# dsilvestro/LiteRate

Hardware: AMD Instinct MI355X
Metric: RJMCMC iters/sec x lineages (lineage-log-lik evals/s, summed over chains) (higher is better)
Workload: dtype f64

## Files before the change

include/literate_hip.h:

```cpp
#ifndef LITERATE_HIP_H
#define LITERATE_HIP_H

#include <stdint.h>

#ifdef __cplusplus
extern "C" {
#endif

#define LR_OK 0
#define LR_ERR_NULL (-1)
#define LR_ERR_SIZE (-2)
#define LR_ERR_MODEL (-3)
#define LR_ERR_WORKSPACE (-4)
#define LR_ERR_T0 (-5)
#define LR_ERR_STATE (-6)
#define LR_ERR_ORDER (-7)

#define LR_KMAX 32
#define LR_ROW 64
#define LR_MAX_BINS 4094

#define LR_MODEL_BD 0
#define LR_MODEL_ID 1
#define LR_MODEL_KEIDING 2
// ... 48 lines not shown
                   double* birth_rates, double* death_rates, void* stream);

int lr_binned_keiding(const double* birth_rates, const double* death_rates, const int64_t* n_spec,
                      const int64_t* n_exti, const double* DT, int32_t n_bins, int32_t n_chains,
                      double* out_birth, double* out_death, void* stream);

int lr_simulate_bd(const double* lam_steps, const double* mu_steps, int32_t n_steps, int32_t mode,
                   double l0, double m0, double K, double scale, int64_t n_start, int64_t capacity,
                   uint64_t seed, double* ts, double* te, int64_t* counters ,
                   int64_t* alive_trace, void* workspace, int64_t workspace_bytes, void* stream);

#define LR_SIMBATCH_GROUPS 512
#define LR_SIMBATCH_LDS_SLOTS 16384
int64_t lr_simulate_bd_batch_workspace_bytes(int32_t n_reps, int32_t n_bins, int32_t steps_per_bin, int64_t capacity);
int lr_simulate_bd_batch(const double* lam_bins , const double* mu_bins ,
                         int32_t n_reps, int32_t n_bins, int32_t steps_per_bin,
                         const int64_t* n_start , int64_t capacity, uint64_t seed,
                         int64_t* counts , int64_t* totals ,
                         void* workspace, int64_t workspace_bytes, void* stream);

#define LR_FORMAT_CRLF 1
int64_t lr_format_rows(const double* vals, const int64_t* row_start, int64_t n_rows, uint64_t int_cols, int32_t flags,
                       char* out, int64_t cap);

int64_t lr_rtt_summary_workspace_bytes(int32_t n_samples, int32_t n_chains, double start_age, double end_age,
                                       double burnin, int32_t pooled);
int lr_rtt_summary(const double* trace, int32_t n_samples, int32_t n_chains, double start_age, double end_age,
                   double burnin, int32_t pooled, double* rates, double* shift_freq, int64_t* k_counts,
                   void* workspace, int64_t workspace_bytes, void* stream);

#define LR_ESS_LDS_ROWS 16384
int64_t lr_ess_summary_workspace_bytes(int32_t n_samples, int32_t n_chains, int32_t row_width, const int32_t* cols,
                                       int32_t n_cols, double burnin, int32_t max_lag);
int lr_ess_summary(const double* rows, int32_t n_samples, int32_t n_chains, int32_t row_width, const int32_t* cols,
                   int32_t n_cols, double burnin, int32_t max_lag, double* chain_stats, int32_t* stop_lag,
                   double* col_stats, void* workspace, int64_t workspace_bytes, void* stream);

int64_t lr_col_summary_workspace_bytes(int32_t n_samples, int32_t n_chains, int32_t row_width, const int32_t* cols,
                                       int32_t n_cols, double burnin, int32_t pooled, int32_t cols_per_pass);
int lr_col_summary(const double* rows, int32_t n_samples, int32_t n_chains, int32_t row_width, const int32_t* cols,
                   int32_t n_cols, double burnin, int32_t pooled, double* out, void* workspace, int64_t workspace_bytes,
                   void* stream);
int64_t lr_curve_summary_workspace_bytes(int32_t n_samples, int32_t n_chains, int32_t row_width, int32_t arg_col,
                                         int32_t sampler, int32_t n_bins, double burnin, int32_t pooled,
                                         int32_t bins_per_pass);
int lr_curve_summary(const double* rows, int32_t n_samples, int32_t n_chains, int32_t row_width, int32_t arg_col,
                     int32_t sampler, int32_t m_birth, int32_t m_death, const double* aux, int32_t n_bins, double burnin,
                     int32_t pooled, double* out, void* workspace, int64_t workspace_bytes, void* stream);

typedef struct lr_mcmc_config {
    int64_t n_lineages;
    int32_t n_bins;
    int32_t n_chains;
    int32_t model;
    int32_t const_rates;
    int32_t const_death_rate;
    int32_t use_rate_HP;
    int32_t s_freq;
    int32_t n_trace_slots;
    double poisson_HP;
    double update_fraction;
    double t0;
    double start_time;
    double end_time;
    uint64_t seed;
    int64_t chain_offset;
    int32_t unit_resolution;
    int32_t engine_mode;
    double frac_birth;
    double frac_death;
    int32_t sampler;
    int32_t m_birth;
    int32_t m_death;
    int32_t team_request;
    double dd_present;
    double dd_init_death;
} lr_mcmc_config;

typedef struct lr_mcmc_layout {
    int64_t state_f64;
    int64_t state_i32;
    int64_t bin_consts;
    int64_t lineage_idx;
    int64_t args_blob;
    int64_t tables;
    int64_t partials;
    int64_t trace;
    int64_t total_bytes;
    int32_t table_stride;
    int32_t tiles;
    int32_t chains_per_block;
    int32_t trace_width;
    int32_t n_parts;
    int32_t pipelined;
    int32_t persistent;
    int32_t reserved1;
    int64_t status;
    int64_t xchg;
    int32_t team_blocks;
    int32_t table_mode;
    int64_t lineage_frac;
    int64_t pack_tmp;
    int32_t spec_chains_per_team;
    int32_t streaming;
    int32_t packed_scan;
    int32_t reserved3;
} lr_mcmc_layout;

#define LR_ROW_L 0
#define LR_ROW_M 1
#define LR_ROW_TL 2
#define LR_ROW_TM 3
#define LR_ROW_PL 4
#define LR_ROW_PM 5
#define LR_ROW_PTL 6
#define LR_ROW_PTM 7
#define LR_ROW_SCALARS 8
#define LR_STATE_ROWS 9
#define LR_S_LIKA 0
#define LR_S_PRIORA 1
#define LR_S_PRIORPOIA 2
#define LR_S_GRATE_L 3
#define LR_S_GRATE_M 4
#define LR_S_POI 5
#define LR_S_HASTING 6
#define LR_S_PRIOR_P 7
#define LR_S_PRIORPOI_P 8
#define LR_S_CONST_P 9
#define LR_S_CONST_A 10
#define LR_S_LIK_P 11
#define LR_S_LOG_G0 12
#define LR_S_LOG_G1 13
#define LR_S_LOG_POI 14
#define LR_S_LOG_U 15
#define LR_IROW_EL 0
#define LR_IROW_EM 1
#define LR_IROW_PEL 2
#define LR_IROW_PEM 3
#define LR_IROW_SCALARS 4
#define LR_ISTATE_ROWS 5
#define LR_I_KL 0
#define LR_I_KM 1
#define LR_I_PKL 2
#define LR_I_PKM 3
#define LR_I_GIBBS 4
#define LR_I_INVALID 5
#define LR_I_IT_LO 6
#define LR_I_IT_HI 7
#define LR_I_ACCEPTED 8
#define LR_I_MOVE 9
#define LR_I_NEXT_LO 10
#define LR_I_NEXT_HI 11
#define LR_I_SLOT 12

#define LR_TRACE_HEAD 13
#define LR_TRACE_W (LR_TRACE_HEAD + 2 * (2 * LR_KMAX - 1))

typedef struct lr_engine lr_engine;

int lr_mcmc_query_layout(const lr_mcmc_config* cfg , lr_mcmc_layout* out );
int lr_mcmc_create(const lr_mcmc_config* cfg , const double* ts, const double* te,
                   const double* br_length ,
                   void* workspace, int64_t workspace_bytes, lr_engine** out );
int lr_mcmc_init(lr_engine* e, const double* L, const double* M, const double* tL,
                 const double* tM, const int32_t* KL, const int32_t* KM, int32_t kmax, void* stream);
int lr_mcmc_steps(lr_engine* e, int64_t n_iters, void* stream);
int lr_mcmc_restore(lr_engine* e, void* stream);
int lr_mcmc_time_scan(lr_engine* e, int32_t reps, float* avg_ms , void* stream);
int lr_mcmc_time_steps(lr_engine* e, int64_t n_iters, float* total_ms , void* stream);
int lr_mcmc_status(lr_engine* e, int32_t* status , void* stream);
#define LR_WARN_KCAP 2
int lr_mcmc_warnings(lr_engine* e, int32_t* warnings , void* stream);
int lr_mcmc_describe(const lr_engine* e, char* buf , int32_t n);
int lr_mcmc_destroy(lr_engine* e);

#ifdef __cplusplus
}
#endif
#endif
```

literate_amd/_hip.py:

```python
import ctypes as C
import os

from .build import LIB

c_i32, c_i64, c_f64, c_vp = C.c_int32, C.c_int64, C.c_double, C.c_void_p

LR_ERR_NULL, LR_ERR_SIZE, LR_ERR_MODEL, LR_ERR_WORKSPACE, LR_ERR_T0, LR_ERR_STATE, LR_ERR_ORDER = -1, -2, -3, -4, -5, -6, -7
ERRORS = {-1: "LR_ERR_NULL", -2: "LR_ERR_SIZE", -3: "LR_ERR_MODEL", -4: "LR_ERR_WORKSPACE", -5: "LR_ERR_T0",
          -6: "LR_ERR_STATE", -7: "LR_ERR_ORDER (lineages must be sorted by birth time for the persistent engines)"}

LR_KMAX, LR_ROW, LR_MAX_BINS = 32, 64, 4094
LR_WARN_KCAP = 2
LR_STATE_ROWS, LR_ISTATE_ROWS = 9, 5
LR_TRACE_HEAD = 13
LR_TRACE_W = LR_TRACE_HEAD + 2 * (2 * LR_KMAX - 1)
LR_SIMBATCH_GROUPS, LR_SIMBATCH_LDS_SLOTS = 512, 16384
LR_ESS_LDS_ROWS = 16384
ROW_L, ROW_M, ROW_TL, ROW_TM, ROW_PL, ROW_PM, ROW_PTL, ROW_PTM, ROW_SCALARS = range(9)
(S_LIKA, S_PRIORA, S_PRIORPOIA, S_GRATE_L, S_GRATE_M, S_POI, S_HASTING, S_PRIOR_P, S_PRIORPOI_P, S_CONST_P,
 S_CONST_A, S_LIK_P, S_LOG_G0, S_LOG_G1, S_LOG_POI) = range(15)
IROW_EL, IROW_EM, IROW_PEL, IROW_PEM, IROW_SCALARS = range(5)
(I_KL, I_KM, I_PKL, I_PKM, I_GIBBS, I_INVALID, I_IT_LO, I_IT_HI, I_ACCEPTED, I_MOVE, I_NEXT_LO, I_NEXT_HI,
 I_SLOT) = range(13)


class McmcConfig(C.Structure):
    _fields_ = [("n_lineages", c_i64), ("n_bins", c_i32), ("n_chains", c_i32), ("model", c_i32),
                ("const_rates", c_i32), ("const_death_rate", c_i32), ("use_rate_HP", c_i32), ("s_freq", c_i32),
                ("n_trace_slots", c_i32), ("poisson_HP", c_f64), ("update_fraction", c_f64), ("t0", c_f64),
                ("start_time", c_f64), ("end_time", c_f64), ("seed", C.c_uint64), ("chain_offset", c_i64),
                ("unit_resolution", c_i32), ("engine_mode", c_i32), ("frac_birth", c_f64), ("frac_death", c_f64),
                ("sampler", c_i32), ("m_birth", c_i32), ("m_death", c_i32), ("team_request", c_i32),
                ("dd_present", c_f64), ("dd_init_death", c_f64)]


class McmcLayout(C.Structure):
    _fields_ = [("state_f64", c_i64), ("state_i32", c_i64), ("bin_consts", c_i64), ("lineage_idx", c_i64), ("args_blob", c_i64), ("tables", c_i64),
                ("partials", c_i64), ("trace", c_i64), ("total_bytes", c_i64), ("table_stride", c_i32),
                ("tiles", c_i32), ("chains_per_block", c_i32), ("trace_width", c_i32), ("n_parts", c_i32),
                ("pipelined", c_i32), ("persistent", c_i32), ("reserved1", c_i32), ("status", c_i64), ("xchg", c_i64),
                ("team_blocks", c_i32), ("table_mode", c_i32), ("lineage_frac", c_i64), ("pack_tmp", c_i64),
                ("spec_chains_per_team", c_i32), ("streaming", c_i32), ("packed_scan", c_i32), ("reserved3", c_i32)]


SIGNATURES = {
    "lr_version": (c_i32, []),
    "lr_bin_events_workspace_bytes": (c_i64, [c_i64, c_i32]),
    "lr_bin_events": (c_i32, [c_vp, c_vp, c_i64, c_vp, c_vp, c_i32, c_vp, c_vp, c_vp, c_vp, c_i64, c_vp]),
    "lr_bin_unit_events_workspace_bytes": (c_i64, [c_i64, c_i32]),
    "lr_bin_unit_events": (c_i32, [c_vp, c_vp, c_i64, c_f64, c_i32, c_vp, c_vp, c_vp, c_vp, c_i64, c_vp]),
    "lr_expand_rates": (c_i32, [c_vp, c_vp, c_vp, c_i32, c_i32, c_i32, c_i32, c_vp, c_vp]),
    "lr_bd_loglik_workspace_bytes": (c_i64, [c_i64, c_i32, c_i32, c_i32]),
    "lr_bd_loglik_plan": (c_i32, [c_i64, c_i32, c_i32, c_i32, C.POINTER(c_i32)]),
    "lr_bd_loglik_batch": (c_i32, [c_vp, c_vp, c_i64, c_f64, c_i32, c_vp, c_vp, c_i32, c_i32, c_vp, c_f64, c_vp,
                                   c_vp, c_i64, c_vp]),
    "lr_rj_propose_score": (c_i32, [c_vp, c_vp, c_vp, c_i32, c_i32, c_vp, c_vp, c_vp, c_f64, c_vp, c_vp, c_vp, c_vp,
                                    c_vp]),
    "lr_log_priors": (c_i32, [c_vp, c_vp, c_i32, c_i32, c_f64, c_vp, c_vp, c_vp, c_vp]),
    "lr_dd_rates": (c_i32, [c_vp, c_vp, c_i32, c_i32, c_i32, c_i32, c_vp, c_vp, c_vp, c_vp, c_vp]),
    "lr_ddv2_rates": (c_i32, [c_vp, c_vp, c_i32, c_i32, c_i32, c_i32, c_vp, c_vp, c_vp, c_vp, c_vp]),
    "lr_binned_keiding": (c_i32, [c_vp, c_vp, c_vp, c_vp, c_vp, c_i32, c_i32, c_vp, c_vp, c_vp]),
    "lr_simulate_bd": (c_i32, [c_vp, c_vp, c_i32, c_i32, c_f64, c_f64, c_f64, c_f64, c_i64, c_i64, C.c_uint64, c_vp, c_vp,
                             c_vp, c_vp, c_vp, c_i64, c_vp]),
    "lr_simulate_bd_batch_workspace_bytes": (c_i64, [c_i32, c_i32, c_i32, c_i64]),
    "lr_simulate_bd_batch": (c_i32, [c_vp, c_vp, c_i32, c_i32, c_i32, c_vp, c_i64, C.c_uint64, c_vp, c_vp, c_vp, c_i64,
                                   c_vp]),
    "lr_trend_rates": (c_i32, [c_vp, c_vp, c_i32, c_i32, c_i32, c_i32, c_vp, c_vp, c_vp]),
    "lr_format_rows": (c_i64, [c_vp, c_vp, c_i64, C.c_uint64, c_i32, c_vp, c_i64]),
    "lr_rtt_summary_workspace_bytes": (c_i64, [c_i32, c_i32, c_f64, c_f64, c_f64, c_i32]),
    "lr_rtt_summary": (c_i32, [c_vp, c_i32, c_i32, c_f64, c_f64, c_f64, c_i32, c_vp, c_vp, c_vp, c_vp, c_i64, c_vp]),
    "lr_ess_summary_workspace_bytes": (c_i64, [c_i32, c_i32, c_i32, c_vp, c_i32, c_f64, c_i32]),
    "lr_ess_summary": (c_i32, [c_vp, c_i32, c_i32, c_i32, c_vp, c_i32, c_f64, c_i32, c_vp, c_vp, c_vp, c_vp, c_i64, c_vp]),
    "lr_col_summary_workspace_bytes": (c_i64, [c_i32, c_i32, c_i32, c_vp, c_i32, c_f64, c_i32, c_i32]),
    "lr_col_summary": (c_i32, [c_vp, c_i32, c_i32, c_i32, c_vp, c_i32, c_f64, c_i32, c_vp, c_vp, c_i64, c_vp]),
    "lr_curve_summary_workspace_bytes": (c_i64, [c_i32, c_i32, c_i32, c_i32, c_i32, c_i32, c_f64, c_i32, c_i32]),
    "lr_curve_summary": (c_i32, [c_vp, c_i32, c_i32, c_i32, c_i32, c_i32, c_i32, c_i32, c_vp, c_i32, c_f64, c_i32, c_vp,
                                 c_vp, c_i64, c_vp]),
    "lr_mcmc_query_layout": (c_i32, [C.POINTER(McmcConfig), C.POINTER(McmcLayout)]),
    "lr_mcmc_create": (c_i32, [C.POINTER(McmcConfig), c_vp, c_vp, c_vp, c_vp, c_i64, C.POINTER(c_vp)]),
    "lr_mcmc_init": (c_i32, [c_vp, c_vp, c_vp, c_vp, c_vp, c_vp, c_vp, c_i32, c_vp]),
    "lr_mcmc_steps": (c_i32, [c_vp, c_i64, c_vp]),
    "lr_mcmc_time_scan": (c_i32, [c_vp, c_i32, C.POINTER(C.c_float), c_vp]),
    "lr_mcmc_time_steps": (c_i32, [c_vp, c_i64, C.POINTER(C.c_float), c_vp]),
    "lr_mcmc_restore": (c_i32, [c_vp, c_vp]),
    "lr_mcmc_describe": (c_i32, [c_vp, C.c_char_p, c_i32]),
    "lr_mcmc_status": (c_i32, [c_vp, C.POINTER(c_i32), c_vp]),
    "lr_mcmc_warnings": (c_i32, [c_vp, C.POINTER(c_i32), c_vp]),
    "lr_mcmc_destroy": (c_i32, [c_vp]),
    "lr_debug_draws": (c_i32, [C.c_uint64, c_i64, c_vp, c_vp, c_vp, c_vp, c_vp, c_i32, c_vp, c_vp]),
    "lr_debug_stream2": (c_i32, [c_vp, c_vp, c_i64, c_vp, c_vp]),
}

_lib = None


class HipLibraryError(RuntimeError):
    pass


def load():
    global _lib
    if _lib is not None:
        return _lib
    if not os.path.exists(LIB):
        raise HipLibraryError("libliterate_hip.so not found at %s - run `python -m literate_amd.build` "
                              "(there is no CPU fallback)" % LIB)
    lib = C.CDLL(LIB)
    for name, (res, args) in SIGNATURES.items():
        fn = getattr(lib, name)
        fn.restype, fn.argtypes = res, args
    _lib = lib
    return lib


def check(rc, what):
    if rc == 0:
        return
    if rc < 0:
        raise ValueError("%s: %s" % (what, ERRORS.get(rc, rc)))
    raise HipLibraryError("%s: hipError_t %d" % (what, rc))


def require_gpu():
    import torch
    if not torch.cuda.is_available():
        raise HipLibraryError("no ROCm GPU visible: literate_amd has no CPU path")
    return torch


def ptr(t):
    return None if t is None else c_vp(t.data_ptr())


def stream_ptr(device=None):
    import torch
    return c_vp(torch.cuda.current_stream(device).cuda_stream)


def launch(fn, device, *args):
    import torch
    with torch.cuda.device(device):
        return fn(*args, stream_ptr(device))
```

literate_amd/csrc/lr_engine.h:

```cpp
#pragma once
#include "lr_internal.h"
#include "lr_scan.h"
#include "lr_step.h"

#define LR_MAX_PARTS 4
struct lr_part {
    int base, count, hA;
    bool pipelined;
    hipStream_t stream;
    hipEvent_t done;
    hipGraphExec_t graph_exec;
    int graph_units;
};

struct lr_p4_shares {
    int delta[16];
    int n_slots;
    int help_trips;
};

struct lr_engine {
    lr_mcmc_config cfg;
    lr_mcmc_layout lay;
    lr_scan_plan plan;
    const double* ts;
    const double* te;
    const double* br_length;
    char* ws;
    bool initialised;
    int n_parts;
    lr_part part[LR_MAX_PARTS];
    bool persistent;
    long long n8;
    long long n8_alloc;
    lr_p4_shares p4;
    bool p4_help;
    bool packed_scan;
    bool streaming;
    hipEvent_t fork;
    hipEvent_t ev0, ev1;
};


#define LR_P4_MAX_GIVE 64
#define LR_IDX_SPARE ((LR_P4_MAX_GIVE + 2) * 1024)
#define LR_MAX_RUNS (1ll << 20)

static inline long long lr_groups_alloc(long long n_lineages) {
    const long long runs = n_lineages < LR_MAX_RUNS ? n_lineages : LR_MAX_RUNS;
    return (n_lineages + LR_SLOTS - 1) / LR_SLOTS + runs + LR_IDX_SPARE;
}

#define LR_P4_CARRY_BYTES 512

#define LR_H_WIDE 520

#ifndef LR_SPEC_THREADS
#define LR_SPEC_THREADS 768
#endif
#ifndef LR_SPEC_THREADS_SINGLE
#define LR_SPEC_THREADS_SINGLE 768
#endif
#ifndef LR_SPEC_SCAN_UNROLL
#define LR_SPEC_SCAN_UNROLL 1
#endif
#ifndef LR_SPEC_SCAN_PRIO
#define LR_SPEC_SCAN_PRIO 2
#endif
#define LR_TEAM_MAX 8
#define LR_SPEC_GRANULES 16
#define LR_SPEC_TIMEOUT_TICKS 200000000ull

static inline bool lr_p4_help_choice(const lr_engine* e) {
    const char* env = getenv("LR_P4_HELP");
    if (e->lay.persistent != 2 || e->plan.unit == LR_TAB_PAIRGEN || e->cfg.sampler != 0 || e->plan.H > 264) return false;
    return env ? atoi(env) != 0 : true;
}

static inline int lr_spec_mode(const lr_engine* e) {
    if (e->lay.spec_chains_per_team != 1) return 0;
    if (e->lay.team_blocks > 1) return 1;
    const double trips = (double)e->n8 / 64.0 / 8.0;
    const char* env = getenv("LR_SPEC_PLANES_BY_SCANNERS");
    const bool by_scanners = env ? atoi(env) != 0 : trips <= 3.0;
    return by_scanners ? 2 : 3;
}

#define LR_STEP_WAVES_PER_BLOCK (LR_SCAN_THREADS / LR_WAVE)
#define LR_STREAM_COPIES 64
#define LR_STREAM_MAX_CHAINS 16
struct lr_stream_sync {
    unsigned long long arrived;
    unsigned long long pad0[15];
    unsigned long long word[LR_STREAM_COPIES][LR_STREAM_MAX_CHAINS];
};
#define LR_STREAM_SYNC_BYTES (128 + LR_STREAM_COPIES * 128 + 128)
static_assert(sizeof(lr_stream_sync) + 128 == LR_STREAM_SYNC_BYTES && LR_STREAM_SYNC_BYTES % 256 == 0, "counter line + a line per copy");
bool lr_stream_eligible(const lr_mcmc_config* cfg, const lr_scan_plan& p);
void lr_stream_plan(const lr_mcmc_config* cfg, lr_scan_plan* p, int cus);
int lr_launch_stream(lr_engine* e, const lr_step_args& a, int64_t n_iters, bool query, hipStream_t stream);

bool lr_packscan_eligible(const lr_mcmc_config* cfg, const lr_scan_plan& p);
void lr_packscan_plan(const lr_mcmc_config* cfg, lr_scan_plan* p, int cus);
int lr_packscan_pairs(const lr_scan_plan& p, int n_chains);
int lr_launch_packscan(const lr_engine* e, int base, int count, hipStream_t stream);

lr_step_args lr_make_args(const lr_engine* e);
int lr_pack_lineages(lr_engine* e, hipStream_t stream);
long long lr_pack_tmp_bytes(long long n_lineages);
int lr_launch_spec(lr_engine* e, const lr_step_args& a, const lr_packed_lineages& pk, int64_t n_iters, hipStream_t stream);
```

literate_amd/csrc/lr_mcmc.hip:

```cpp
#include <cmath>
#include <cstdio>
#include <cstdlib>
#include <new>

#include "lr_chain.h"
#include "lr_dd.h"
#include "lr_engine.h"
#include "lr_internal.h"
#include "lr_scan.h"
#include "lr_step.h"

__global__ __launch_bounds__(LR_WAVE) void lr_rj_propose_score_kernel(
    const double* __restrict__ rates, const double* __restrict__ times, const int* __restrict__ K, int kmax,
    const int* __restrict__ move, const int* __restrict__ index, const double* __restrict__ draws, double mult_d,
    double* __restrict__ out_rates, double* __restrict__ out_times, int* __restrict__ out_K,
    double* __restrict__ out_score) {
    const int c = blockIdx.x, lane = threadIdx.x;
    int k = K[c];
    double R = (lane < k) ? rates[(size_t)c * kmax + lane] : 0.0;
    double T = (lane <= k) ? times[(size_t)c * (kmax + 1) + lane] : 0.0;
    const double* dr = draws + (size_t)c * 2 * kmax;
    const int mv = move[c];
    double score = 0.0;
    if (mv == 0) {
// ... 3 lines not shown
    } else if (mv == 1) {
        score = lr_wave_add_shift(R, T, k, index[c], dr[0], dr[1], lane);
    } else if (mv == 2) {
        score = lr_wave_remove_shift(R, T, k, index[c], lane);
    }
    if (lane < kmax) out_rates[(size_t)c * kmax + lane] = (lane < k) ? R : 0.0;
    if (lane <= kmax) out_times[(size_t)c * (kmax + 1) + lane] = (lane <= k) ? T : 0.0;
    if (lane == 0) out_K[c] = k, out_score[c] = score;
}

extern "C" int lr_rj_propose_score(const double* rates, const double* times, const int32_t* K, int32_t kmax,
                                   int32_t n_chains, const int32_t* move, const int32_t* index, const double* draws,
                                   double mult_d, double* out_rates, double* out_times, int32_t* out_K,
                                   double* out_score, void* stream_) {
    if (!rates || !times || !K || !move || !index || !draws || !out_rates || !out_times || !out_K || !out_score)
        return LR_ERR_NULL;
    if (kmax < 2 || kmax > LR_WAVE - 1 || n_chains < 1) return LR_ERR_SIZE;
    hipLaunchKernelGGL(lr_rj_propose_score_kernel, dim3(n_chains), dim3(LR_WAVE), 0, (hipStream_t)stream_, rates, times,
                       K, kmax, move, index, draws, mult_d, out_rates, out_times, out_K, out_score);
    return (int)hipGetLastError();
}

__global__ __launch_bounds__(LR_WAVE) void lr_log_priors_kernel(const double* __restrict__ rates,
                                                                const int* __restrict__ K, int kmax, double shape,
                                                                const double* __restrict__ gamma_rate,
                                                                const double* __restrict__ poi_rate,
                                                                double* __restrict__ out) {
    const int c = blockIdx.x, lane = threadIdx.x;
    const int k = K[c];
    const double R = (lane < k) ? rates[(size_t)c * kmax + lane] : 1.0;
    double p = lr_wave_prior_gamma(R, k, shape, gamma_rate[c], lane);
    if (poi_rate) p += lr_wave_poisson_prior(k, poi_rate[c], lane);
    if (lane == 0) out[c] = p;
}

extern "C" int lr_log_priors(const double* rates, const int32_t* K, int32_t kmax, int32_t n_chains, double shape,
                             const double* gamma_rate, const double* poi_rate, double* out, void* stream_) {
    if (!rates || !K || !gamma_rate || !out) return LR_ERR_NULL;
    if (kmax < 1 || kmax > LR_WAVE - 1 || n_chains < 1) return LR_ERR_SIZE;
    hipLaunchKernelGGL(lr_log_priors_kernel, dim3(n_chains), dim3(LR_WAVE), 0, (hipStream_t)stream_, rates, K, kmax,
                       shape, gamma_rate, poi_rate, out);
    return (int)hipGetLastError();
}

__global__ void lr_debug_draws_kernel(uint32_t seed, uint32_t chain, const long long* it, const int* purpose,
                                      const int* idx, const int* kind, const double* shape, int n, double* out) {
    const int i = blockIdx.x * blockDim.x + threadIdx.x;
    if (i >= n) return;
    lr_stream s{seed, chain};
    const uint64_t t = (uint64_t)it[i];
    double v;
    switch (kind[i]) {
        case 0: v = lr_pair(s, t, purpose[i], idx[i]).a; break;
        case 1: v = lr_pair(s, t, purpose[i], idx[i]).b; break;
        case 2: v = lr_normal(s, t, purpose[i], idx[i]); break;
        default: v = lr_gamma(s, t, purpose[i], idx[i], shape[i]); break;
    }
    out[i] = v;
}

extern "C" int lr_debug_draws(uint64_t seed, int64_t chain, const int64_t* it, const int32_t* purpose,
                              const int32_t* idx, const int32_t* kind, const double* shape, int32_t n, double* out,
                              void* stream_) {
    if (!it || !purpose || !idx || !kind || !shape || !out) return LR_ERR_NULL;
    hipLaunchKernelGGL(lr_debug_draws_kernel, dim3((n + 63) / 64), dim3(64), 0, (hipStream_t)stream_, (uint32_t)seed,
                       (uint32_t)chain, (const long long*)it, purpose, idx, kind, shape, n, out);
    return (int)hipGetLastError();
}

#define LR_STEP_WAVES (LR_SCAN_THREADS / LR_WAVE)

__global__ __launch_bounds__(LR_SCAN_THREADS) void lr_chain_step_kernel(lr_step_args a, int mode, int chain_base,
                                                                        int n_sub) {
    __shared__ lr_seg_scratch scratch[LR_STEP_WAVES];
    const int wave = threadIdx.x / LR_WAVE, lane = threadIdx.x & (LR_WAVE - 1);
    const int j = blockIdx.x * LR_STEP_WAVES + wave;
    if (j < n_sub) lr_chain_step_body<32>(a, mode, chain_base + j, lane, &scratch[wave]);
}

struct lr_fused_args {
    const double* ts;
    const double* te;
    long long n, chunk;
    double t0;
    int n_bins, tiles;
    int scan_base, scan_n;
    int step_base, step_n;
    int step_blocks;
};

template <int CB, int H, bool UNIT>
__global__ __launch_bounds__(LR_SCAN_THREADS) void lr_fused_iter_kernel(lr_step_args a, lr_fused_args f) {
    extern __shared__ double2 lds[];
    lr_seg_scratch* scratch = reinterpret_cast<lr_seg_scratch*>(lds);
    const int bid = blockIdx.x;
    if (bid < f.step_blocks) {
        const int wave = threadIdx.x / LR_WAVE, lane = threadIdx.x & (LR_WAVE - 1);
        const int j = bid * LR_STEP_WAVES + wave;
        if (j < f.step_n) lr_chain_step_body(a, 0, f.step_base + j, lane, &scratch[wave]);
        return;
    }
    int group, tile;
    if ((f.step_blocks & 7) == 0) {
        lr_xcd_remap(bid - f.step_blocks, f.tiles, (f.scan_n + CB - 1) / CB, &group, &tile);
    } else {
        const int sb = bid - f.step_blocks;
        tile = sb % f.tiles, group = sb / f.tiles;
    }
    const double2* tables = a.tables + (size_t)f.scan_base * a.tab_stride;
    const int tile_stride = lr_tile_stride(a.tiles);
    double* partials = const_cast<double*>(a.partials) + (size_t)f.scan_base * tile_stride;
    if (UNIT)
        lr_scan_unit_body<CB, H>(lds, tile, group * CB, f.ts, f.te, f.n, f.t0, f.n_bins, tables, f.scan_n, f.chunk,
                                 partials, tile_stride);
    else
        lr_scan_fast_body<CB, H>(lds, tile, group * CB, f.ts, f.te, f.n, f.t0, f.n_bins, tables, f.scan_n, f.chunk,
                                 partials, tile_stride);
}

#ifndef LR_PERSIST_THREADS
#define LR_PERSIST_THREADS 512
#endif
#ifndef LR_PERSIST_MINWAVES
#define LR_PERSIST_MINWAVES 4
#endif

template <int H, bool GENERAL>
__global__ __launch_bounds__(256) void lr_pairscan_kernel(lr_packed_lineages pk, long long n8, const double2* __restrict__ tables,
                                                          int n_chains, int n_bins, int tiles, double* __restrict__ partials) {
    constexpr int ENT = GENERAL ? 2 : 1;
    __shared__ double2 tab[LR_UNIT_PLANES * H];
    __shared__ double red[4][2];
    const int tid = threadIdx.x, lane = tid & (LR_WAVE - 1), wave = tid / LR_WAVE;
    const int tile = blockIdx.x, pair = blockIdx.y;
    const double2* src = tables + (size_t)pair * (2 * H * ENT);
    for (int i = tid; i < 2 * H * ENT; i += 256) tab[GENERAL ? lr_pairgen_lds_entry(i, H) : i] = src[i];
    __syncthreads();
    if (GENERAL) lr_pair_planes_block_general(tab, H, n_bins, tid, 256);
    else lr_pair_planes_block(tab, H, n_bins, tid, 256);
    __syncthreads();
    const long long per = (n8 + tiles - 1) / tiles;
    const long long g0 = min((long long)tile * per, n8), g1 = min(g0 + per, n8);
    double acc0 = 0.0, acc1 = 0.0;
    lr_persist_scan<H, GENERAL>(reinterpret_cast<const char*>(tab), pk, g0, g1 - g0, tid, 256, &acc0, &acc1);
    const double s0 = lr_wave_sum(acc0), s1 = lr_wave_sum(acc1);
    if (lane == 0) red[wave][0] = s0, red[wave][1] = s1;
    __syncthreads();
    if (tid < 2 && 2 * pair + tid < n_chains)
        partials[(size_t)(2 * pair + tid) * lr_tile_stride(tiles) + tile] = ((red[0][tid] + red[1][tid]) + red[2][tid]) + red[3][tid];
}

typedef __attribute__((address_space(3))) double lr_lds_f64;
typedef __attribute__((address_space(3))) int lr_lds_i32;
template <int PB, int ES, bool PRE = false, int SAMPLER = -1, bool HAND = false>
__device__ __forceinline__ void lr_persist_step_body(const __attribute__((address_space(3))) lr_step_args* a3, int c, int lane,
                                                     __attribute__((address_space(3))) lr_seg_scratch* scratch3,
                                                     lr_lds_f64* st_f64, lr_lds_i32* st_i32, double lik, lr_lds_f64* table3,
                                                     lr_lds_f64* br3 ,
                                                     const lr_draw_slot* draws = nullptr ,
                                                     lr_table_hand* hand = nullptr, int hand_epoch = 0) {
    constexpr int table_es = ES;
    const lr_step_args& a = *(const lr_step_args*)a3;
    const double* br_lds = (const double*)br3;
    LR_SSTAMP(0);
    lr_chain_regs st;
    lr_chain_load(st, (double*)st_f64, (int*)st_i32, lane);
    if (SAMPLER == 1 || (SAMPLER == -1 && a.cfg.sampler != 0))
        lr_dd_step_core<true>(st, a, 0, c, lane, lik, reinterpret_cast<double2*>((double*)table3), table_es, br_lds);
    else if (PRE) {
        lr_rj_draws pre;
        lr_draws_load(draws, pre, lane);
        lr_chain_step_core<true, PB, HAND>(st, a, 0, c, lane, (lr_seg_scratch*)scratch3, lik, reinterpret_cast<double2*>((double*)table3),
                                           table_es, br_lds, br_lds + LR_H_WIDE, &pre, hand, hand_epoch);
    } else
        lr_chain_step_core<true, PB>(st, a, 0, c, lane, (lr_seg_scratch*)scratch3, lik, reinterpret_cast<double2*>((double*)table3),
                                     table_es, br_lds, br_lds + LR_H_WIDE);
    if (HAND) lr_chain_store_handed(st, (double*)st_f64, (int*)st_i32, lane);
    else lr_chain_store(st, (double*)st_f64, (int*)st_i32, lane);
    LR_SSTAMP(8);
}

template <int NA>
__device__ __forceinline__ void lr_p4_leave_sums(double2 (*part)[LR_WAVE], int* arrived, double* out, int slot, int lane,
                                                 int& scans_done, double s0, double s1) {
    part[slot][lane] = make_double2(s0, s1);
    int prev = 0;
    if (lane == 0) prev = __hip_atomic_fetch_add(arrived, 1, __ATOMIC_RELAXED, __HIP_MEMORY_SCOPE_WORKGROUP);
    prev = __builtin_amdgcn_readfirstlane(prev);
    if (prev == NA * (scans_done + 1) - 1) {
        asm volatile("" ::: "memory");
        double a0 = 0.0, a1 = 0.0;
#pragma unroll
        for (int w = 0; w < NA; ++w) {
            const double2 v = part[w][lane];
            a0 += v.x, a1 += v.y;
        }
        a0 = lr_wave_sum(a0), a1 = lr_wave_sum(a1);
        if (lane == 0) out[0] = a0, out[1] = a1;
    }
    ++scans_done;
}

template <int PB, int ES>
__device__ __attribute__((noinline)) void lr_persist_step(const __attribute__((address_space(3))) lr_step_args* a3, int c, int lane,
                                                          __attribute__((address_space(3))) lr_seg_scratch* scratch3,
                                                          lr_lds_f64* st_f64, lr_lds_i32* st_i32, double lik, lr_lds_f64* table3,
                                                          lr_lds_f64* br3) {
    lr_persist_step_body<PB, ES>(a3, c, lane, scratch3, st_f64, st_i32, lik, table3, br3);
}

template <int PB, int ES, int NW, int SAMPLER, bool HELP>
__device__ __attribute__((noinline)) void lr_persist4_steppers(const __attribute__((address_space(3))) lr_step_args* a3, int c0,
                                                               int n_chains, int wave, int lane,
                                                               __attribute__((address_space(3))) lr_seg_scratch* scratch3,
                                                               lr_lds_f64* st_f64, lr_lds_i32* st_i32, lr_lds_f64* red,
                                                               lr_lds_f64* tab, int tab_doubles, lr_lds_f64* br3, long long n_iters,
                                                               const lr_draw_slot* draws ,
                                                               lr_table_hand* hands ) {
    static_assert(!HELP || (ES == 2 && SAMPLER == 0), "helper waves: RJ sampler at unit resolution");
    for (long long iter = 0; iter < n_iters; ++iter) {
#pragma unroll 1
        for (int ph = 0; ph < 2; ++ph) {
#ifdef LR_DIAG
            const unsigned long long dq0 = wall_clock64();
#endif
            const int c = c0 + 2 * ph + wave;
            if (c < n_chains) {
                double lik = 0.0;
#pragma unroll
                for (int w2 = 2; w2 < (ES == 2  ? 3 : NW); ++w2) lik += red[(ph * NW + w2) * 2 + wave];
                lr_persist_step_body<PB, ES, ES == 2  && SAMPLER == 0, SAMPLER, HELP>(
                    a3, c, lane, scratch3, st_f64 + (2 * ph + wave) * (LR_STATE_ROWS * LR_ROW),
                    st_i32 + (2 * ph + wave) * (LR_ISTATE_ROWS * LR_ROW), lik, tab + ph * tab_doubles + wave, br3,
                    draws + (2 * ph + wave), HELP ? hands + wave : nullptr, (int)((2 * iter + ph + 1) & 0x3fffffff));
            }
#ifdef LR_DIAG
            const unsigned long long dq1 = wall_clock64();
#endif
            __syncthreads();
#ifdef LR_DIAG
            if (lane == 0 && blockIdx.x < 64) {
                atomicAdd(&lr_diag_step[16384 + (blockIdx.x * 16 + wave) * 4 + 0], dq1 - dq0);
                atomicAdd(&lr_diag_step[16384 + (blockIdx.x * 16 + wave) * 4 + 1], wall_clock64() - dq1);
            }
#endif
        }
    }
}

template <int H, int T, int PB>
__device__ __attribute__((noinline)) void lr_persist2_steppers(const __attribute__((address_space(3))) lr_step_args* a3, int c, int wave,
                                                               int lane, __attribute__((address_space(3))) lr_seg_scratch* scratch3,
                                                               lr_lds_f64* st_f64, lr_lds_i32* st_i32, lr_lds_f64* red ,
                                                               lr_lds_f64* tab, lr_lds_f64* br3, const uint4* __restrict__ idx8,
                                                               long long n8w, long long n_iters, int prio_shift, int grp) {
    const int tid = wave * LR_WAVE + lane;
    for (long long iter = 0; iter < n_iters; ++iter) {
        if (prio_shift > 0) {
            if (((wall_clock64() >> prio_shift) + grp) & 1) __builtin_amdgcn_s_setprio(1);
            else __builtin_amdgcn_s_setprio(0);
        }
        double acc0 = 0.0, acc1 = 0.0;
        lr_scan_tail tail;
        lr_persist_scan_pair<H, 1, true>((const char*)(const double*)tab, idx8, n8w, tid, T, &acc0, &acc1, nullptr, &tail);
        const double s0 = lr_wave_sum(acc0), s1 = lr_wave_sum(acc1);
        if (lane == 0) red[wave * 2 + 0] = s0, red[wave * 2 + 1] = s1;
        lr_scan_drain(tail);
        __syncthreads();
        double lik = 0.0;
#pragma unroll
        for (int w2 = 0; w2 < T / LR_WAVE; ++w2) lik += red[w2 * 2 + wave];
        lr_persist_step_body<PB, 2>(a3, c, lane, scratch3, st_f64, st_i32, lik, tab + wave, br3);
        __syncthreads();
    }
}

template <int H, int T>
__global__ __launch_bounds__(T, LR_PERSIST_MINWAVES) void lr_persist_kernel(
    const lr_step_args* __restrict__ ap ,
    const uint4* __restrict__ idx8, long long n8, lr_p4_shares sh, long long n_iters, int prio_shift) {
    const lr_step_args& a = *ap;
    __shared__ double2 tab[LR_UNIT_PLANES * H];
    __shared__ double red[T / LR_WAVE][2];
    __shared__ lr_seg_scratch scratch[2];
    __shared__ double st_f64[2][LR_STATE_ROWS * LR_ROW];
    __shared__ int st_i32[2][LR_ISTATE_ROWS * LR_ROW];
    __shared__ lr_step_args a_lds;
    __shared__ double br_lds[2][LR_H_WIDE];
    const int tid = threadIdx.x, lane = tid & (LR_WAVE - 1), wave = tid / LR_WAVE;
    if (tid < (int)(sizeof(lr_step_args) / 4)) reinterpret_cast<int*>(&a_lds)[tid] = reinterpret_cast<const int*>(ap)[tid];
    for (int b = tid; b < LR_H_WIDE; b += blockDim.x) {
        const bool in = b < ap->cfg.n_bins;
        br_lds[0][b] = (in && ap->br_length) ? ap->br_length[b] : 0.0;
        br_lds[1][b] = in ? ap->log_br[b] : 0.0;
    }
    const int c0 = blockIdx.x * 2;
    const int c = c0 + wave;
    const bool stepper = (wave < 2) && (c < a.cfg.n_chains);
    double2* gpair = lr_chain_table(a, c0);
    if (stepper) {
        const double* S = a.state_f64 + (size_t)c * LR_STATE_ROWS * LR_ROW;
        const int* I = a.state_i32 + (size_t)c * LR_ISTATE_ROWS * LR_ROW;
        for (int r = 0; r < LR_STATE_ROWS; ++r) st_f64[wave][r * LR_ROW + lane] = S[r * LR_ROW + lane];
        for (int r = 0; r < LR_ISTATE_ROWS; ++r) st_i32[wave][r * LR_ROW + lane] = I[r * LR_ROW + lane];
    }
    for (int i = tid; i < 2 * H; i += T) tab[i] = gpair[i];
    __syncthreads();
    lr_pair_planes_block(tab, H, a.cfg.n_bins, tid, T);
    __syncthreads();
    const char* lbase = reinterpret_cast<const char*>(tab);
    const long long n8w = sh.delta[0] != 0 ? ((n8 + T - 1) / T + sh.delta[wave]) * T : n8;
    const int grp = (blockIdx.x >> 8) & 1;
#ifdef LR_DIAG
    unsigned long long d_t0 = 0, d_t1 = 0, d_t2 = 0, d_scan = 0, d_red = 0, d_step = 0;
#endif
#ifndef LR_DIAG
    if (stepper) {
        lr_persist2_steppers<H, T, (H <= 264 ? lr_bins_per_lane(H) : 0)>(
            (const __attribute__((address_space(3))) lr_step_args*)&a_lds, c, wave, lane,
            (__attribute__((address_space(3))) lr_seg_scratch*)&scratch[wave], (lr_lds_f64*)st_f64[wave], (lr_lds_i32*)st_i32[wave],
            (lr_lds_f64*)&red[0][0], (lr_lds_f64*)reinterpret_cast<double*>(tab), (lr_lds_f64*)&br_lds[0][0], idx8, n8w, n_iters,
            prio_shift, grp);
    } else
#endif
    for (long long iter = 0; iter < n_iters; ++iter) {
        if (prio_shift > 0) {
            if (((wall_clock64() >> prio_shift) + grp) & 1) __builtin_amdgcn_s_setprio(1);
            else __builtin_amdgcn_s_setprio(0);
        }
#ifdef LR_DIAG
        d_t0 = wall_clock64();
#endif
        double acc0 = 0.0, acc1 = 0.0;
        lr_scan_tail tail;
        lr_persist_scan_pair<H, 1, true>(lbase, idx8, n8w, tid, T, &acc0, &acc1, nullptr, &tail);
#ifdef LR_DIAG
        if (lane == 0 && blockIdx.x < 512) atomicAdd(&lr_diag_step[20000 + blockIdx.x * 8 + wave], wall_clock64() - d_t0);
#endif
#ifdef LR_DIAG
        d_t1 = wall_clock64();
#endif
        const double s0 = lr_wave_sum(acc0), s1 = lr_wave_sum(acc1);
        if (lane == 0) red[wave][0] = s0, red[wave][1] = s1;
        lr_scan_drain(tail);
        __syncthreads();
#ifdef LR_DIAG
        d_t2 = wall_clock64();
#endif
        if (stepper) {
            double lik = 0.0;
#pragma unroll
            for (int w2 = 0; w2 < T / LR_WAVE; ++w2) lik += red[w2][wave];
            lr_persist_step<(H <= 264 ? lr_bins_per_lane(H) : 0), 2>(
                (const __attribute__((address_space(3))) lr_step_args*)&a_lds, c, lane,
                (__attribute__((address_space(3))) lr_seg_scratch*)&scratch[wave], (lr_lds_f64*)st_f64[wave],
                (lr_lds_i32*)st_i32[wave], lik, (lr_lds_f64*)(reinterpret_cast<double*>(tab) + wave), (lr_lds_f64*)&br_lds[0][0]);
        }
        __syncthreads();
#ifdef LR_DIAG
        d_scan += d_t1 - d_t0, d_red += d_t2 - d_t1, d_step += wall_clock64() - d_t2;
#endif
    }
#ifdef LR_DIAG
    if (lane == 0 && blockIdx.x < 512) {
        unsigned long long* o = lr_diag_step + 4096 * 12 - 4096 + (blockIdx.x * 8 + wave) % 4096;
        (void)o;
    }
    if (tid == 0 && blockIdx.x < 340) {
        lr_diag_step[blockIdx.x * 12 + 9] = d_scan, lr_diag_step[blockIdx.x * 12 + 10] = d_red;
        lr_diag_step[blockIdx.x * 12 + 11] = d_step;
    }
    if (tid == 0 && blockIdx.x < 1024) lr_diag_step[2048 * 12 + blockIdx.x * 2 + 1] = wall_clock64();
#endif
    if (stepper) {
        double* S = a.state_f64 + (size_t)c * LR_STATE_ROWS * LR_ROW;
        int* I = a.state_i32 + (size_t)c * LR_ISTATE_ROWS * LR_ROW;
        for (int r = 0; r < LR_STATE_ROWS; ++r) S[r * LR_ROW + lane] = st_f64[wave][r * LR_ROW + lane];
        for (int r = 0; r < LR_ISTATE_ROWS; ++r) I[r * LR_ROW + lane] = st_i32[wave][r * LR_ROW + lane];
    }
    for (int i = tid; i < 2 * H; i += T) gpair[i] = tab[i];
}

#ifndef LR_P4_THREADS
#define LR_P4_THREADS 1024
#endif
#ifdef LR_DIAG
#define LR_PSTAMP(k) if (threadIdx.x == 0 && blockIdx.x < 64) lr_diag_step[28672 + blockIdx.x * 8 + (k)] = wall_clock64()
#else
#define LR_PSTAMP(k)
#endif

template <int H, bool GENERAL, bool PARAM ,
          bool HELP = false>
__global__ __launch_bounds__(LR_P4_THREADS, LR_P4_THREADS / 256) void lr_persist4_kernel(const lr_step_args* __restrict__ ap ,
                                                                       lr_packed_lineages pk, long long n8,
                                                                       lr_p4_shares sh, long long n_iters, char* carry_all) {
    static_assert(!HELP || (!GENERAL && !PARAM), "helper waves: RJ sampler at unit resolution");
    const lr_step_args& a = *ap;
    LR_PSTAMP(0);
    constexpr int NW = LR_P4_THREADS / LR_WAVE;
    constexpr int W0 = HELP ? 4 : 2;
    constexpr int NS = NW - W0;
    constexpr int LR_P4_SCANNERS = NS * LR_WAVE;
    constexpr int ENT = GENERAL ? 2 : 1;
    constexpr int ES = GENERAL ? 6 * H : 2;
    __shared__ double2 tab[2][LR_UNIT_PLANES * H];
    __shared__ double red[2][NW][2];
    constexpr bool LAST_SUMS = !GENERAL;
    __shared__ double2 part[LAST_SUMS ? NW - 2 : 1][LR_WAVE];
    __shared__ int arrived;
    __shared__ lr_table_hand hands[2];
    __shared__ lr_seg_scratch scratch[2];
    __shared__ double st_f64[4][LR_STATE_ROWS * LR_ROW];
    __shared__ int st_i32[4][LR_ISTATE_ROWS * LR_ROW];
    __shared__ lr_step_args a_lds;
    __shared__ double br_lds[2][LR_H_WIDE];
    __shared__ lr_draw_slot draws_s[4];
    lr_draw_slot* const draws = draws_s;
    const int tid = threadIdx.x, lane = tid & (LR_WAVE - 1), wave = tid / LR_WAVE;
    if (tid < (int)(sizeof(lr_step_args) / 4)) reinterpret_cast<int*>(&a_lds)[tid] = reinterpret_cast<const int*>(ap)[tid];
    for (int b = tid; b < LR_H_WIDE; b += blockDim.x) {
        const bool in = b < ap->cfg.n_bins;
        br_lds[0][b] = (in && ap->br_length) ? ap->br_length[b] : 0.0;
        br_lds[1][b] = in ? ap->log_br[b] : 0.0;
    }
    constexpr bool draw_ahead = !GENERAL && !PARAM;
    auto draw_duty = [&](int pr) {
        const int q = wave - W0, k = q & 1, ch = 2 * pr + k;
        if (!draw_ahead || q < 0 || q >= (HELP ? 2 : 4) || (int)(blockIdx.x * 4) + ch >= ap->cfg.n_chains) return;
        const int* I = st_i32[ch] + LR_IROW_SCALARS * LR_ROW;
        const unsigned long long it = ((unsigned long long)(unsigned int)I[LR_I_IT_HI] << 32 | (unsigned int)I[LR_I_IT_LO]) + 1ull;
        lr_draw_slot* slot = &draws[ch];
        if (HELP) lr_spec_draw_both(a_lds, (int)(blockIdx.x * 4) + ch, lane, it, slot);
        else lr_spec_draw_part(a_lds, (int)(blockIdx.x * 4) + ch, lane, it, slot, q >> 1);
    };
    auto help_duty = [&](int ph, int epoch) {
        const int k = wave - 2;
        const int ch = 2 * ph + k;
        if ((int)(blockIdx.x * 4) + ch >= ap->cfg.n_chains) return;
        lr_table_hand* hand = &hands[k];
#ifdef LR_DIAG
        const unsigned long long dh0 = wall_clock64();
#endif
        while (__hip_atomic_load(&hand->epoch, __ATOMIC_RELAXED, __HIP_MEMORY_SCOPE_WORKGROUP) != epoch) __builtin_amdgcn_s_sleep(1);
        asm volatile("" ::: "memory");
#ifdef LR_DIAG
        if (lane == 0 && blockIdx.x < 64) atomicAdd(&lr_diag_step[16384 + (blockIdx.x * 16 + wave) * 4 + 2], wall_clock64() - dh0);
#endif
        const lr_seg_scratch* sc = &scratch[k];
        const int eL = lane <= LR_KMAX ? sc->edge[0][lane] : 0, eM = lane <= LR_KMAX ? sc->edge[1][lane] : 0;
        double* tabd = reinterpret_cast<double*>(tab[ph]) + k;
        const double constP = lr_build_tables_segments<(H <= 264 ? lr_bins_per_lane(H) : 1), 2>(
            sc, eL, eM, hand->KL, hand->KM, br_lds[0], br_lds[1], a_lds.cfg.model, a_lds.cfg.n_bins, a_lds.n_cls, a_lds.H,
            reinterpret_cast<double2*>(tabd), lane, LR_TAB_UNIT, a_lds.cfg.frac_birth, a_lds.cfg.frac_death, ES, nullptr);
        LR_WAVE_LDS_ORDER();
        lr_pair_planes_wave(tabd, H, a_lds.cfg.n_bins, lane, 0);
        if (lane == 0) st_f64[ch][LR_ROW_SCALARS * LR_ROW + LR_S_CONST_P] = constP;
    };
    if (tid == 0) arrived = 0;
    if (tid < 2) hands[tid].epoch = 0;
    for (int i = tid; i < 2 * NW * 2; i += LR_P4_THREADS) (&red[0][0][0])[i] = 0.0;
    int scans_done = 0;
    constexpr int NA = NS + (HELP ? 2 : 0);
    auto leave_sums = [&](int pr, double s0, double s1) {
        if (LAST_SUMS) {
            lr_p4_leave_sums<NA>(part, &arrived, &red[pr][2][0], wave >= W0 ? wave - W0 : NS + wave - 2, lane, scans_done, s0, s1);
        } else {
            s0 = lr_wave_sum(s0), s1 = lr_wave_sum(s1);
            if (lane == 0) red[pr][wave][0] = s0, red[pr][wave][1] = s1;
        }
    };
    const int c0 = blockIdx.x * 4;
    const int C = a.cfg.n_chains;
    if (wave < 4 && c0 + wave < C) {
        const int c = c0 + wave;
        const double* S = a.state_f64 + (size_t)c * LR_STATE_ROWS * LR_ROW;
        const int* I = a.state_i32 + (size_t)c * LR_ISTATE_ROWS * LR_ROW;
        for (int r = 0; r < LR_STATE_ROWS; ++r) st_f64[wave][r * LR_ROW + lane] = S[r * LR_ROW + lane];
        for (int r = 0; r < LR_ISTATE_ROWS; ++r) st_i32[wave][r * LR_ROW + lane] = I[r * LR_ROW + lane];
    }
    double2* g0 = lr_chain_table(a, c0);
    double2* g1 = lr_chain_table(a, c0 + 2);
    for (int i = tid; i < 2 * H * ENT; i += LR_P4_THREADS) {
        const int e = GENERAL ? lr_pairgen_lds_entry(i, H) : i;
        tab[0][e] = g0[i], tab[1][e] = g1[i];
    }
    __syncthreads();
    LR_PSTAMP(1);
    if (GENERAL) {
        lr_pair_planes_block_general(tab[0], H, a.cfg.n_bins, tid, LR_P4_THREADS);
        lr_pair_planes_block_general(tab[1], H, a.cfg.n_bins, tid, LR_P4_THREADS);
    } else {
        lr_pair_planes_block(tab[0], H, a.cfg.n_bins, tid, LR_P4_THREADS);
        lr_pair_planes_block(tab[1], H, a.cfg.n_bins, tid, LR_P4_THREADS);
    }
    __syncthreads();
    LR_PSTAMP(2);
    const bool scanner = wave >= W0;
    const bool helper = HELP && (wave == 2 || wave == 3);
    const int sid = tid - W0 * LR_WAVE;
    const long long nh_ = HELP ? (long long)sh.help_trips * (2 * LR_WAVE) : 0;
    const int k_tot = (int)((n8 - nh_ + LR_P4_SCANNERS - 1) / LR_P4_SCANNERS);
    const int k_mine = k_tot + (scanner ? sh.delta[wave - W0] : 0);
    bool any_shift = false;
#pragma unroll
    for (int q = 0; q < NS; ++q) any_shift |= sh.delta[q] != 0;
    const long long nh = HELP ? (long long)sh.help_trips * (2 * LR_WAVE) : 0;
    const long long n8w = any_shift ? (long long)k_mine * LR_P4_SCANNERS : n8 - nh;
    auto help_scan = [&](int pr) {
        double s0 = 0.0, s1 = 0.0;
        if (nh > 0) lr_persist_scan<H, GENERAL, 1, false, false>(reinterpret_cast<const char*>(tab[pr]), pk, 0, nh, tid - 2 * LR_WAVE, 2 * LR_WAVE, &s0, &s1);
        leave_sums(pr, s0, s1);
    };
    static_assert(2 * NW * 8 + 4 <= LR_P4_CARRY_BYTES, "");
    char* carry = carry_all ? carry_all + (size_t)blockIdx.x * LR_P4_CARRY_BYTES : nullptr;
    const bool carried = carry && *reinterpret_cast<const int*>(carry + 2 * NW * 8) == 1;
    auto prologue_draws = [&]() { draw_duty(0); };
    if (carried) {
        if (tid < 2 * NW) (&red[0][0][0])[tid] = reinterpret_cast<const double*>(carry)[tid];
        if (scanner) prologue_draws();
    } else if (scanner) {
        double s0 = 0.0, s1 = 0.0;
        lr_scan_tail tail;
        lr_persist_scan<H, GENERAL, 1, false, true>(reinterpret_cast<const char*>(tab[0]), pk, nh, n8w, sid, LR_P4_SCANNERS, &s0, &s1, nullptr, &tail);
        leave_sums(0, s0, s1);
        lr_scan_drain(tail);
        prologue_draws();
    }
    if (helper && !carried) help_scan(0);
    __syncthreads();
    LR_PSTAMP(3);
    if (helper) {
        for (long long iter = 0; iter < n_iters; ++iter) {
#pragma unroll 1
            for (int ph = 0; ph < 2; ++ph) {
#ifdef LR_DIAG
                const unsigned long long dq0 = wall_clock64();
#endif
                help_scan(1 - ph);
                help_duty(ph, (int)((2 * iter + ph + 1) & 0x3fffffff));
#ifdef LR_DIAG
                const unsigned long long dq1 = wall_clock64();
#endif
                __syncthreads();
#ifdef LR_DIAG
                if (lane == 0 && blockIdx.x < 64) {
                    atomicAdd(&lr_diag_step[16384 + (blockIdx.x * 16 + wave) * 4 + 0], dq1 - dq0);
                    atomicAdd(&lr_diag_step[16384 + (blockIdx.x * 16 + wave) * 4 + 1], wall_clock64() - dq1);
                }
#endif
            }
        }
    } else if (!scanner)
        lr_persist4_steppers<(H <= 264 ? lr_bins_per_lane(H) : 0), ES, NW, PARAM ? 1 : 0, HELP>(
            (const __attribute__((address_space(3))) lr_step_args*)&a_lds, c0, C, wave, lane,
            (__attribute__((address_space(3))) lr_seg_scratch*)&scratch[wave], (lr_lds_f64*)&st_f64[0][0], (lr_lds_i32*)&st_i32[0][0],
            (lr_lds_f64*)&red[0][0][0], (lr_lds_f64*)reinterpret_cast<double*>(tab[0]), 2 * LR_UNIT_PLANES * H,
            (lr_lds_f64*)&br_lds[0][0], n_iters, &draws[0], &hands[0]);
    else
    for (long long iter = 0; iter < n_iters; ++iter) {
#pragma unroll
        for (int ph = 0; ph < 2; ++ph) {
#ifdef LR_DIAG
            const unsigned long long dq0 = wall_clock64();
#endif
            {
                double s0 = 0.0, s1 = 0.0;
                lr_scan_tail tail;
                lr_persist_scan<H, GENERAL, 1, false, true>(reinterpret_cast<const char*>(tab[1 - ph]), pk, nh, n8w, sid, LR_P4_SCANNERS, &s0, &s1, nullptr, &tail);
                leave_sums(1 - ph, s0, s1);
                lr_scan_drain(tail);
                draw_duty(1 - ph);
            }
#ifdef LR_DIAG
            const unsigned long long dq1 = wall_clock64();
#endif
            __syncthreads();
#ifdef LR_DIAG
            if (lane == 0 && blockIdx.x < 64) {
                atomicAdd(&lr_diag_step[16384 + (blockIdx.x * 16 + wave) * 4 + 0], dq1 - dq0);
                atomicAdd(&lr_diag_step[16384 + (blockIdx.x * 16 + wave) * 4 + 1], wall_clock64() - dq1);
            }
#endif
        }
    }
    LR_PSTAMP(4);
    if (wave < 4 && c0 + wave < C) {
        const int c = c0 + wave;
        double* S = a.state_f64 + (size_t)c * LR_STATE_ROWS * LR_ROW;
        int* I = a.state_i32 + (size_t)c * LR_ISTATE_ROWS * LR_ROW;
        for (int r = 0; r < LR_STATE_ROWS; ++r) S[r * LR_ROW + lane] = st_f64[wave][r * LR_ROW + lane];
        for (int r = 0; r < LR_ISTATE_ROWS; ++r) I[r * LR_ROW + lane] = st_i32[wave][r * LR_ROW + lane];
    }
    for (int i = tid; i < 2 * H * ENT; i += LR_P4_THREADS) {
        const int e = GENERAL ? lr_pairgen_lds_entry(i, H) : i;
        g0[i] = tab[0][e], g1[i] = tab[1][e];
    }
    if (carry) {
        if (tid < 2 * NW) reinterpret_cast<double*>(carry)[tid] = (&red[0][0][0])[tid];
        if (tid == 0) *reinterpret_cast<int*>(carry + 2 * NW * 8) = 1;
    }
    LR_PSTAMP(5);
}

__global__ void lr_store_args_kernel(lr_step_args a, lr_step_args* dst) {
    if (threadIdx.x == 0 && blockIdx.x == 0) *dst = a;
}

__global__ void lr_log_br_kernel(const double* __restrict__ br, int n_bins, double* __restrict__ out) {
    const int b = blockIdx.x * blockDim.x + threadIdx.x;
    if (b < n_bins) out[b] = (br && br[b] > 0.0) ? lr_log(br[b]) : 0.0;
}

__global__ __launch_bounds__(LR_WAVE) void lr_chain_init_kernel(lr_step_args a, const double* L0, const double* M0,
                                                                const double* tL0, const double* tM0,
                                                                const int* KL0, const int* KM0, int kmax) {
    __shared__ lr_seg_scratch scratch;
    const lr_mcmc_config& cfg = a.cfg;
    const int c = blockIdx.x, lane = threadIdx.x, n_bins = cfg.n_bins;
    double* S = a.state_f64 + (size_t)c * LR_STATE_ROWS * LR_ROW;
    int* I = a.state_i32 + (size_t)c * LR_ISTATE_ROWS * LR_ROW;
    const lr_stream rng{(uint32_t)cfg.seed, (uint32_t)(cfg.chain_offset + c)};
    if (cfg.sampler != 0) {
        const bool trend = cfg.sampler == 2;
        const int npar = trend ? LR_TR_NPAR : LR_DD_NPAR;
        double A = 0.0;
        if (L0) {
            if (lane < npar) A = L0[(size_t)c * kmax + lane];
        } else if (trend) {
            const double init[LR_TR_NPAR] = {.1, .1, 0.0, 0.0, 1.0, 1.0};
            if (lane < npar) A = init[lane];
        } else {
            const double x0 = cfg.dd_present - (cfg.t0 + cfg.dd_present) / 2.0;
            const double init[LR_DD_NPAR] = {0.5, 1.5, x0, 10.0, 20000.0, cfg.dd_init_death, 1.0, 1.0};
            if (lane < npar) A = init[lane];
        }
        if (trend) {
            const lr_trend_params tp = lr_trend_unpack(A);
            const double* aux = a.br_length;
            lr_rates_build_tables_wave([&](int b, double* br, double* dr) { lr_trend_bin_rates(tp, aux[b], cfg.m_birth, cfg.m_death, br, dr); },
                                       n_bins, a.H, lr_chain_table(a, c), lane, a.unit, cfg.frac_birth, cfg.frac_death, lr_tab_es(a.unit, a.H));
        } else {
            const lr_dd_params pp = lr_dd_unpack(A);
            lr_dd_build_tables_wave(pp, a.br_length, cfg.m_birth, cfg.m_death, n_bins, a.H, lr_chain_table(a, c), lane,
                                    a.unit, cfg.frac_birth, cfg.frac_death, lr_tab_es(a.unit, a.H));
        }
        for (int r = 0; r < LR_STATE_ROWS; ++r) S[r * LR_ROW + lane] = 0.0;
        for (int r = 0; r < LR_ISTATE_ROWS; ++r) I[r * LR_ROW + lane] = 0;
        S[LR_ROW_L * LR_ROW + lane] = A, S[LR_ROW_PL * LR_ROW + lane] = A;
        int io = 0;
        if (lane == LR_I_KL || lane == LR_I_PKL || lane == LR_I_KM || lane == LR_I_PKM) io = npar;
        I[LR_IROW_SCALARS * LR_ROW + lane] = io;
        return;
    }
    double L = 0.0, M = 0.0, tL = 0.0, tM = 0.0;
    int KL = 1, KM = 1;
    if (L0) {
        KL = KL0[c], KM = KM0[c];
        if (lane < KL) L = L0[(size_t)c * kmax + lane];
        if (lane < KM) M = M0[(size_t)c * kmax + lane];
        if (lane <= KL) tL = tL0[(size_t)c * (kmax + 1) + lane];
        if (lane <= KM) tM = tM0[(size_t)c * (kmax + 1) + lane];
    } else {
        const double l0 = lr_gamma(rng, 0, LR_P_INIT, 0, 2.0) * 2.0;
        const double m0 = lr_gamma(rng, 0, LR_P_INIT, 64, 2.0) * 2.0;
        if (lane == 0) L = l0, M = m0, tL = tM = cfg.start_time;
        if (lane == 1) tL = tM = cfg.end_time;
    }
    const int eL = lr_wave_edges(tL, 1), eM = lr_wave_edges(tM, 1);
    double logL, logM;
    lr_stage_segments(&scratch, L, M, eL, eM, KL, KM, lane, &logL, &logM);
    const double constA = lr_build_tables_segments(&scratch, eL, eM, KL, KM, a.br_length, a.log_br, cfg.model, n_bins,
                                                   a.n_cls, a.H, lr_chain_table(a, c), lane,
                                                   a.unit, cfg.frac_birth, cfg.frac_death, lr_tab_es(a.unit, a.H));
    S[LR_ROW_L * LR_ROW + lane] = L, S[LR_ROW_M * LR_ROW + lane] = M;
    S[LR_ROW_TL * LR_ROW + lane] = tL, S[LR_ROW_TM * LR_ROW + lane] = tM;
    S[LR_ROW_PL * LR_ROW + lane] = L, S[LR_ROW_PM * LR_ROW + lane] = M;
    S[LR_ROW_PTL * LR_ROW + lane] = tL, S[LR_ROW_PTM * LR_ROW + lane] = tM;
    I[LR_IROW_EL * LR_ROW + lane] = eL, I[LR_IROW_EM * LR_ROW + lane] = eM;
    I[LR_IROW_PEL * LR_ROW + lane] = eL, I[LR_IROW_PEM * LR_ROW + lane] = eM;
    const double poi0 = (cfg.poisson_HP == 0.0) ? 1.0 : cfg.poisson_HP;
    double so = 0.0;
    if (lane == LR_S_GRATE_L || lane == LR_S_GRATE_M) so = 1.0;
    if (lane == LR_S_POI) so = poi0;
    if (lane == LR_S_LOG_POI) so = lr_log(poi0);
    if (lane == LR_S_CONST_A || lane == LR_S_CONST_P) so = constA;
    S[LR_ROW_SCALARS * LR_ROW + lane] = so;
    int io = 0;
    if (lane == LR_I_KL || lane == LR_I_PKL) io = KL;
    if (lane == LR_I_KM || lane == LR_I_PKM) io = KM;
    I[LR_IROW_SCALARS * LR_ROW + lane] = io;
}

static int lr_env_int(const char* name, int dflt) {
    const char* v = getenv(name);
    return v ? atoi(v) : dflt;
}
static int lr_pipeline_env() {
    static int env = lr_env_int("LR_PIPELINE", 1);
    return env;
}

static bool lr_packscan_planned(const lr_mcmc_config* cfg, const lr_scan_plan& p) {
    if (!lr_packscan_eligible(cfg, p)) return false;
    const bool general = p.unit == LR_TAB_PAIRGEN;
    const double evals = (double)cfg->n_lineages * (double)cfg->n_chains;
    return cfg->engine_mode == 7 || cfg->n_chains < (general ? 17 : 32) || evals >= (general ? 1.5e8 : 3.0e8);
}

static int lr_packed_mode(const lr_mcmc_config* cfg, const lr_scan_plan& p) {
    if (!lr_packscan_planned(cfg, p)) return 0;
    const char* env = getenv("LR_PACKED_PARTS");
    if (env && (atoi(env) == 1 || atoi(env) == 2)) return atoi(env);
    const double evals = (double)cfg->n_lineages * (double)cfg->n_chains;
    return evals >= (p.unit == LR_TAB_PAIRGEN ? 1.75e8 : 3.5e8) ? 2 : 1;
}

static int lr_partition(int n_chains, int cb, bool fused_ok, int base[LR_MAX_PARTS + 1], int hA[LR_MAX_PARTS],
                        bool pipelined[LR_MAX_PARTS], int packed = 0) {
    static const int want_parts = lr_env_int("LR_PARTS", 2);
    int parts = want_parts < 1 ? 1 : (want_parts > LR_MAX_PARTS ? LR_MAX_PARTS : want_parts);
    if (packed) fused_ok = false;
    if (packed == 1) parts = 1;
    const int groups = (n_chains + cb - 1) / cb;
    const bool pipe = lr_pipeline_env() && fused_ok;
    while (parts > 1 && groups < parts * (pipe ? 2 : 1)) --parts;
    base[0] = 0;
    for (int p = 0; p < parts; ++p) {
        const int g = groups / parts + (p < groups % parts ? 1 : 0);
        base[p + 1] = base[p] + g * cb < n_chains ? base[p] + g * cb : n_chains;
    }
    base[parts] = n_chains;
    for (int p = 0; p < parts; ++p) {
        const int count = base[p + 1] - base[p];
        pipelined[p] = pipe && count >= 2 * cb;
        hA[p] = pipelined[p] ? ((count / 2 + cb - 1) / cb) * cb : count;
    }
    return parts;
}

static int lr_persist_variant(const lr_mcmc_config* cfg, const lr_scan_plan& p, int* team_k, int* team_cpb);
static int lr_device_cus();
static int lr_plan_engine(const lr_mcmc_config* cfg, lr_scan_plan* p) {
    int rc = lr_plan_scan(cfg->n_lineages, cfg->n_chains, cfg->n_bins, cfg->model, cfg->unit_resolution, p,
                          (!cfg->unit_resolution && cfg->n_chains > 8 && cfg->n_chains <= 16 && lr_env_int("LR_ENGINE_WIDE", 1)) ? 1 : 0);
    if (rc) return rc;
    if (cfg->model == LR_MODEL_KEIDING_DEAD && cfg->n_bins <= 258) {
        static const int fast_H[] = {40, 72, 136, 264, LR_H_WIDE};
        lr_scan_plan q = *p;
        q.n_cls = 1, q.fast = 1, q.H = 0;
        for (int h : fast_H)
            if (2 * (cfg->n_bins + 2) <= h) {
                q.H = h;
// ... 149 lines not shown
    if (env == 0 || cfg->engine_mode == 1 || cfg->engine_mode == 6 || cfg->engine_mode == 7) return false;
    if (!p.unit || cfg->n_bins + 2 > LR_H_WIDE || p.cb < 2) return false;
    const bool general = p.unit == LR_TAB_PAIRGEN;
    if (cfg->n_lineages >= (1ll << 31) - 1 || lr_groups_alloc(cfg->n_lineages) * 16 >= (1ll << 32)) return false;
    if (p.H != 40 && p.H != 72 && p.H != 136 && p.H != 264 && p.H != LR_H_WIDE) return false;
    if (env == 1 || cfg->engine_mode >= 2) return true;
    const double n = (double)cfg->n_lineages, c = (double)cfg->n_chains;
    double t_persist = lr_model_four_chain(cfg, general);
    if (!general) t_persist = fmin(t_persist, lr_model_two_chain(cfg));
    int k = 0;
    const double t_spec = (p.H > (general ? 136 : 264)) ? 1e30 : lr_spec_model(cfg, &k, general);
    if (k > 0 && t_spec < t_persist) t_persist = t_spec;
    double t_launch = n * c / (general ? 3e12 : 7e12) * 1e6 + 15.5 + c / 1024.0;
    if (lr_packscan_planned(cfg, p)) t_launch = fmin(t_launch, 11.5 + 5.0 * c / 1024.0 + n * c / (general ? 1.5e13 : 3.1e13) * 1e6);
    return t_persist <= t_launch;
}

static int lr_persist_variant(const lr_mcmc_config* cfg, const lr_scan_plan& p, int* team_k, int* team_cpb = nullptr) {
    if (team_k) *team_k = 0;
    if (team_cpb) *team_cpb = 0;
    if (!lr_persist_eligible(cfg, p)) return 0;
    static const int p4_env = lr_env_int("LR_PERSIST4", -1);
    static const int spec_env = lr_env_int("LR_SPEC", -1);
    const bool general = p.unit == LR_TAB_PAIRGEN;
    int k = 0, cpb = 2;
    const double t_spec = (p.H > (general ? 136 : 264)) ? 1e30 : lr_spec_model(cfg, &k, general, &cpb);
    if (k > 0 && t_spec < 1e29 && cfg->engine_mode != 3 && cfg->engine_mode != 4 && spec_env != 0) {
        const double t_wide = general ? 1e30 : fmax(4.1, 4.41 + 0.236 * (double)((cfg->n_lineages + LR_GRP - 1) / LR_GRP) / 1024.0);
        if (cfg->engine_mode == 5 || spec_env == 1 || t_spec <= t_wide) {
            if (team_k) *team_k = k;
            if (team_cpb) *team_cpb = cpb;
            return 3;
        }
    }
    if (cfg->engine_mode == 5) return 0;
    if (general) return (p.cb >= 4 && cfg->engine_mode != 4) ? 2 : 0;
    if (p.cb < 4) return 1;
    if (cfg->engine_mode == 3) return 2;
    if (cfg->engine_mode == 4) return 1;
    if (p4_env >= 0) return p4_env ? 2 : 1;
    return lr_model_four_chain(cfg, false) < lr_model_two_chain(cfg) ? 2 : 1;
}

static int lr_check_cfg(const lr_mcmc_config* cfg) {
    if (!cfg) return LR_ERR_NULL;
    if (cfg->n_lineages < 1 || cfg->n_chains < 1 || cfg->s_freq < 1 || cfg->n_trace_slots < 0) return LR_ERR_SIZE;
    if (cfg->n_bins < 1 || cfg->n_bins > LR_MAX_BINS) return LR_ERR_SIZE;
    if (cfg->model < 0 || cfg->model > 3) return LR_ERR_MODEL;
    if (cfg->t0 != floor(cfg->t0)) return LR_ERR_T0;
    if (!(cfg->end_time > cfg->start_time)) return LR_ERR_SIZE;
    if (cfg->sampler < 0 || cfg->sampler > 2) return LR_ERR_MODEL;
    {
        const int k_req = cfg->team_request & 0xff, cpb_req = (cfg->team_request >> 8) & 0xff;
        if (cfg->team_request < 0 || cfg->team_request > 0xffff) return LR_ERR_SIZE;
        if (k_req != 0 && k_req != 1 && k_req != 2 && k_req != 4 && k_req != 8) return LR_ERR_SIZE;
        if (cpb_req > 2) return LR_ERR_SIZE;
    }
    if (cfg->sampler != 0) {
        if (cfg->model != LR_MODEL_KEIDING) return LR_ERR_MODEL;
        if (cfg->n_bins > LR_DD_MAXP * LR_WAVE) return LR_ERR_SIZE;
    }
    if (cfg->sampler == 1) {
        if (cfg->m_birth < 0 || cfg->m_birth > 2 || cfg->m_death < -2 || cfg->m_death > 2) return LR_ERR_MODEL;
        if (!(cfg->dd_present > cfg->t0)) return LR_ERR_SIZE;
    }
    return LR_OK;
}

extern "C" int lr_mcmc_query_layout(const lr_mcmc_config* cfg, lr_mcmc_layout* out) {
    int rc = lr_check_cfg(cfg);
    if (rc) return rc;
    if (!out) return LR_ERR_NULL;
    lr_scan_plan p;
    rc = lr_plan_engine(cfg, &p);
    if (rc) return rc;
    const long long C = cfg->n_chains;
    long long o = 0;
    out->state_f64 = o, o += lr_align_up64(C * LR_STATE_ROWS * LR_ROW * 8, 256);
    out->state_i32 = o, o += lr_align_up64(C * LR_ISTATE_ROWS * LR_ROW * 4, 256);
    out->bin_consts = o, o += lr_align_up64((long long)(cfg->n_bins + 2) * 8, 256);
    const long long n_alloc = lr_groups_alloc(cfg->n_lineages);
    out->lineage_idx = o, o += lr_align_up64(n_alloc * 16, 256);
    out->lineage_frac = o;
    if (p.unit == LR_TAB_PAIRGEN) o += lr_align_up64(n_alloc * 16 * LR_FRAC_ARRAYS, 256);
    out->pack_tmp = o, o += lr_align_up64(lr_pack_tmp_bytes(cfg->n_lineages), 256);
    out->args_blob = o, o += 1024;
    out->tables = o, o += lr_align_up64((long long)lr_align_up64(C, p.cb < 2 ? 2 : p.cb) * p.tab_stride * 16, 256);
    out->partials = o, o += lr_align_up64((long long)lr_tile_stride(p.tiles) * C * 8, 256);
    out->trace = o, o += lr_align_up64((long long)cfg->n_trace_slots * C * LR_TRACE_W * 8, 256);
    int team_k = 0, team_cpb = 0;
    out->persistent = lr_persist_variant(cfg, p, &team_k, &team_cpb);
    out->spec_chains_per_team = team_cpb;
    {
        int base[LR_MAX_PARTS + 1], hA[LR_MAX_PARTS];
        bool pipelined[LR_MAX_PARTS];
        const bool packed = lr_packscan_planned(cfg, p);
        const int parts = lr_partition(cfg->n_chains, p.cb, lr_fused_supported(p), base, hA, pipelined, lr_packed_mode(cfg, p));
        out->packed_scan = (out->persistent == 0 && packed) ? 1 : 0;
        out->streaming = (out->persistent == 0 && !out->packed_scan && parts == 1 && !pipelined[0] && lr_stream_eligible(cfg, p)) ? 1 : 0;
        out->reserved3 = 0;
    }
    if (p.unit == LR_TAB_PAIRGEN && out->persistent == 0 && !lr_packscan_planned(cfg, p)) return LR_ERR_STATE;
    out->team_blocks = team_k;
    out->table_mode = p.unit;
    out->status = o, o += 256;
    out->xchg = o, o += (team_k > 1) ? lr_align_up64(2ll * C * LR_TEAM_MAX * LR_SPEC_GRANULES * 8, 256)
                                     : (out->persistent == 2 ? lr_align_up64((C + 3) / 4 * LR_P4_CARRY_BYTES, 256)
                                        : (out->streaming ? LR_STREAM_SYNC_BYTES + lr_align_up64((long long)lr_align_up64(C, p.cb < 2 ? 2 : p.cb) * p.tab_stride * 16, 256) : 0));
    out->total_bytes = o;
    out->table_stride = p.tab_stride;
    out->tiles = p.tiles;
    out->chains_per_block = p.cb;
    out->trace_width = LR_TRACE_W;
    {
        int base[LR_MAX_PARTS + 1], hA[LR_MAX_PARTS];
        bool pipelined[LR_MAX_PARTS];
        out->n_parts = lr_partition(cfg->n_chains, p.cb, lr_fused_supported(p), base, hA, pipelined, lr_packed_mode(cfg, p));
        out->pipelined = pipelined[0] ? 1 : 0;
    }
    {
        static const int wide_env = lr_env_int("LR_PERSIST_WIDE", -1);
        const bool wide = wide_env >= 0 ? wide_env != 0 : ((cfg->n_chains + 1) / 2 <= 256 && cfg->n_lineages >= 20000);
        out->reserved1 = out->persistent == 3 ? (team_cpb == 1 ? LR_SPEC_THREADS_SINGLE : LR_SPEC_THREADS) : (out->persistent == 2 ? 1024 : (out->persistent == 1 ? (wide ? 1024 : 512) : 0));
    }
    return LR_OK;
}

extern "C" int lr_mcmc_create(const lr_mcmc_config* cfg, const double* ts, const double* te, const double* br_length,
                              void* workspace, int64_t workspace_bytes, lr_engine** out) {
    if (!ts || !te || !workspace || !out) return LR_ERR_NULL;
    lr_mcmc_layout lay;
    int rc = lr_mcmc_query_layout(cfg, &lay);
    if (rc) return rc;
    if ((cfg->model == LR_MODEL_BD || cfg->model == LR_MODEL_ID || cfg->sampler != 0) && !br_length) return LR_ERR_MODEL;
    if (lay.total_bytes > workspace_bytes) return LR_ERR_WORKSPACE;
    lr_engine* e = new (std::nothrow) lr_engine();
    if (!e) return (int)hipErrorOutOfMemory;
    e->cfg = *cfg;
    e->lay = lay;
    lr_plan_engine(cfg, &e->plan);
    e->ts = ts, e->te = te, e->br_length = br_length;
    e->ws = (char*)workspace;
    e->initialised = false;
    int base[LR_MAX_PARTS + 1], hA[LR_MAX_PARTS];
    bool pipelined[LR_MAX_PARTS];
    e->n_parts = lr_partition(cfg->n_chains, e->plan.cb, lr_fused_supported(e->plan), base, hA, pipelined,
                              lay.packed_scan ? lr_packed_mode(cfg, e->plan) : 0);
    e->persistent = lay.persistent != 0;
    e->n8 = 0;
    e->n8_alloc = lr_groups_alloc(cfg->n_lineages);
    for (int j = 0; j < 16; ++j) e->p4.delta[j] = 0;
    e->p4.n_slots = 8;
    e->p4_help = lr_p4_help_choice(e);
    e->streaming = false;
    e->packed_scan = lay.packed_scan != 0;
    e->fork = nullptr;
    e->ev0 = e->ev1 = nullptr;
    for (int p = 0; p < e->n_parts; ++p) {
        lr_part& q = e->part[p];
        q.base = base[p], q.count = base[p + 1] - base[p], q.hA = hA[p], q.pipelined = pipelined[p];
        q.stream = nullptr, q.done = nullptr, q.graph_exec = nullptr, q.graph_units = 0;
    }
    {
        hipError_t he = hipEventCreate(&e->ev0);
        if (he == hipSuccess) he = hipEventCreate(&e->ev1);
        if (he != hipSuccess) {
            lr_mcmc_destroy(e);
            return (int)he;
        }
    }
    if (e->n_parts > 1) {
        hipError_t he = hipEventCreateWithFlags(&e->fork, hipEventDisableTiming);
        for (int p = 0; p < e->n_parts && he == hipSuccess; ++p) {
            he = hipStreamCreateWithFlags(&e->part[p].stream, hipStreamNonBlocking);
            if (he == hipSuccess) he = hipEventCreateWithFlags(&e->part[p].done, hipEventDisableTiming);
        }
        if (he != hipSuccess) {
            lr_mcmc_destroy(e);
            return (int)he;
        }
    }
    if (lay.streaming) {
        const int rcq = lr_launch_stream(e, lr_make_args(e), 0, true, nullptr);
        if (rcq != LR_OK && rcq != LR_ERR_STATE) {
            lr_mcmc_destroy(e);
            return rcq;
        }
        e->streaming = rcq == LR_OK;
    }
    *out = e;
    return LR_OK;
}

lr_step_args lr_make_args(const lr_engine* e) {
    lr_step_args a;
    a.cfg = e->cfg;
    a.state_f64 = (double*)(e->ws + e->lay.state_f64);
    a.state_i32 = (int*)(e->ws + e->lay.state_i32);
    a.log_br = (const double*)(e->ws + e->lay.bin_consts);
    a.dd_consts = a.log_br + e->cfg.n_bins;
    a.log_T = log(e->cfg.end_time - e->cfg.start_time);
    a.mult_l = 2.0 * log(LR_MULT_D);
    a.tables = (double2*)(e->ws + e->lay.tables);
    a.partials = (const double*)(e->ws + e->lay.partials);
    a.trace = (double*)(e->ws + e->lay.trace);
    a.br_length = e->br_length;
    a.tab_stride = e->plan.tab_stride;
    a.n_cls = e->plan.n_cls;
    a.tiles = e->plan.tiles;
    a.H = e->plan.H;
    a.unit = e->plan.unit;
    a.cb = e->plan.cb;
    a.warn = (unsigned int*)(e->ws + e->lay.status) + 1;
    return a;
}

template <int H>
static int lr_launch_pairscan(const lr_engine* e, hipStream_t stream) {
    lr_packed_lineages pk;
    pk.idx8 = (const uint4*)(e->ws + e->lay.lineage_idx), pk.frac = (const uint4*)(e->ws + e->lay.lineage_frac);
    pk.fstride = e->n8_alloc;
    const dim3 grid(e->plan.tiles, (e->cfg.n_chains + 1) / 2);
    if (e->plan.unit == LR_TAB_PAIRGEN)
        hipLaunchKernelGGL((lr_pairscan_kernel<H, true>), grid, dim3(256), 0, stream, pk, e->n8,
                           (const double2*)(e->ws + e->lay.tables), e->cfg.n_chains, e->cfg.n_bins, e->plan.tiles, (double*)(e->ws + e->lay.partials));
    else
        hipLaunchKernelGGL((lr_pairscan_kernel<H, false>), grid, dim3(256), 0, stream, pk, e->n8,
                           (const double2*)(e->ws + e->lay.tables), e->cfg.n_chains, e->cfg.n_bins, e->plan.tiles, (double*)(e->ws + e->lay.partials));
    return (int)hipGetLastError();
}

static int lr_enqueue_scan_range(const lr_engine* e, int base, int count, hipStream_t stream) {
    if (e->packed_scan) return lr_launch_packscan(e, base, count, stream);
    if (e->plan.unit == LR_TAB_PAIRGEN || (e->persistent && (e->cfg.model == LR_MODEL_KEIDING_DEAD || e->plan.H == LR_H_WIDE))) {
        if (base != 0 || count != e->cfg.n_chains) return LR_ERR_STATE;
        switch (e->plan.H) {
            case 40: return lr_launch_pairscan<40>(e, stream);
            case 72: return lr_launch_pairscan<72>(e, stream);
            case 136: return lr_launch_pairscan<136>(e, stream);
            case 264: return lr_launch_pairscan<264>(e, stream);
            default: return lr_launch_pairscan<LR_H_WIDE>(e, stream);
        }
    }
    return lr_launch_scan(e->plan, e->ts, e->te, e->cfg.n_lineages, e->cfg.t0, e->cfg.n_bins, e->cfg.end_time,
                          (const double2*)(e->ws + e->lay.tables) + (size_t)base * e->plan.tab_stride, count,
                          (double*)(e->ws + e->lay.partials) + (size_t)base * lr_tile_stride(e->plan.tiles), lr_tile_stride(e->plan.tiles), stream);
}
static int lr_enqueue_scan(const lr_engine* e, hipStream_t stream) {
    return lr_enqueue_scan_range(e, 0, e->cfg.n_chains, stream);
}
static int lr_enqueue_step_range(const lr_engine* e, const lr_step_args& a, int mode, int base, int count,
                                 hipStream_t stream) {
    hipLaunchKernelGGL(lr_chain_step_kernel, dim3((count + LR_STEP_WAVES - 1) / LR_STEP_WAVES), dim3(LR_SCAN_THREADS),
                       0, stream, a, mode, base, count);
    return (int)hipGetLastError();
}

__global__ void lr_dd_consts_kernel(const double* __restrict__ DT, int n_bins, double* __restrict__ out) {
    const int lane = threadIdx.x;
    double m = -INFINITY;
    for (int b = lane; b < n_bins; b += LR_WAVE) m = fmax(m, DT[b]);
    m = -lr_wave_min(-m);
    if (lane == 0) out[0] = m, out[1] = lr_log(m);
}

static void lr_prepare_constants(const lr_engine* e, const lr_step_args& a, hipStream_t stream, bool restored) {
    if (restored) {
        (void)hipMemsetAsync(e->ws + e->lay.status, 0, 4, stream);
        (void)hipMemsetAsync(e->ws + e->lay.status + 8, 0, 248, stream);
    } else {
        (void)hipMemsetAsync(e->ws + e->lay.status, 0, 256, stream);
    }
    if (e->lay.persistent == 2) (void)hipMemsetAsync(e->ws + e->lay.xchg, 0, (size_t)((e->cfg.n_chains + 3) / 4) * LR_P4_CARRY_BYTES, stream);
    hipLaunchKernelGGL(lr_log_br_kernel, dim3((e->cfg.n_bins + 127) / 128), dim3(128), 0, stream, e->br_length,
                       e->cfg.n_bins, (double*)(e->ws + e->lay.bin_consts));
    if (e->cfg.sampler == 1)
        hipLaunchKernelGGL(lr_dd_consts_kernel, dim3(1), dim3(LR_WAVE), 0, stream, e->br_length, e->cfg.n_bins,
                           (double*)(e->ws + e->lay.bin_consts) + e->cfg.n_bins);
    if (e->persistent) {
        static_assert(sizeof(lr_step_args) <= 1024, "args blob too small");
        hipLaunchKernelGGL(lr_store_args_kernel, dim3(1), dim3(64), 0, stream, a, (lr_step_args*)(e->ws + e->lay.args_blob));
    }
}

static int lr_pack_for_scan(lr_engine* e, hipStream_t stream) {
    if (!e->lay.packed_scan) return LR_OK;
    const int rc = lr_pack_lineages(e, stream);
    e->packed_scan = rc == LR_OK;
    return (rc != LR_OK && (e->plan.unit == LR_TAB_PAIRGEN || e->cfg.model == LR_MODEL_KEIDING_DEAD || e->plan.H == LR_H_WIDE)) ? rc : LR_OK;
}

extern "C" int lr_mcmc_restore(lr_engine* e, void* stream_) {
    if (!e) return LR_ERR_NULL;
    hipStream_t stream = (hipStream_t)stream_;
    const lr_step_args a = lr_make_args(e);
    lr_prepare_constants(e, a, stream, true);
    int rc = (int)hipGetLastError();
    if (rc) return rc;
    if (e->persistent) rc = lr_pack_lineages(e, stream);
    if (rc) return rc;
    rc = lr_pack_for_scan(e, stream);
    if (rc) return rc;
    e->initialised = true;
    return LR_OK;
}

// ... 9 lines not shown
    if (e->persistent) {
        const int rcp = lr_pack_lineages(e, stream);
        if (rcp) return rcp;
    }
    {
        const int rcp = lr_pack_for_scan(e, stream);
        if (rcp) return rcp;
    }
    hipLaunchKernelGGL(lr_chain_init_kernel, dim3(e->cfg.n_chains), dim3(LR_WAVE), 0, stream, a, L, M, tL, tM, KL, KM,
                       kmax);
    int rc = (int)hipGetLastError();
    if (rc) return rc;
    rc = lr_enqueue_scan(e, stream);
    if (rc) return rc;
    rc = lr_enqueue_step_range(e, a, 1, 0, e->cfg.n_chains, stream);
    if (rc) return rc;
    e->initialised = true;
    return LR_OK;
}

static int lr_graph_iters() {
    static int v = -1;
    if (v < 0) {
        const char* e = getenv("LR_GRAPH_ITERS");
        v = e ? atoi(e) : 32;
        if (v < 0) v = 0;
        if (v > 4096) v = 4096;
    }
    return v;
}

template <int CB, int H, bool UNIT>
static int lr_launch_fused(const lr_engine* e, const lr_step_args& a, const lr_fused_args& f, hipStream_t stream) {
    const int groups = (f.scan_n + CB - 1) / CB;
    const int blocks = f.step_blocks + groups * f.tiles;
    const size_t lds_bytes = e->plan.lds_bytes > (int)(LR_STEP_WAVES * sizeof(lr_seg_scratch)) ? (size_t)e->plan.lds_bytes : LR_STEP_WAVES * sizeof(lr_seg_scratch);
    hipLaunchKernelGGL((lr_fused_iter_kernel<CB, H, UNIT>), dim3(blocks), dim3(LR_SCAN_THREADS), lds_bytes,
                       stream, a, f);
    return (int)hipGetLastError();
}

template <int H>
static int lr_launch_fused_h(const lr_engine* e, const lr_step_args& a, const lr_fused_args& f, hipStream_t stream) {
    if (e->plan.unit) {
        switch (e->plan.cb) {
            case 16: return lr_launch_fused<16, H, true>(e, a, f, stream);
            case 8: return lr_launch_fused<8, H, true>(e, a, f, stream);
            default: return LR_ERR_SIZE;
        }
    }
    switch (e->plan.cb) {
        case 8: return lr_launch_fused<8, H, false>(e, a, f, stream);
        case 4: return lr_launch_fused<4, H, false>(e, a, f, stream);
        default: return LR_ERR_SIZE;
    }
}

static int lr_enqueue_fused(const lr_engine* e, const lr_step_args& a, int scan_base, int scan_n, int step_base,
                            int step_n, hipStream_t stream) {
    lr_fused_args f;
    f.ts = e->ts, f.te = e->te, f.n = e->cfg.n_lineages, f.chunk = e->plan.chunk, f.t0 = e->cfg.t0;
    f.n_bins = e->cfg.n_bins, f.tiles = e->plan.tiles;
    f.scan_base = scan_base, f.scan_n = scan_n, f.step_base = step_base, f.step_n = step_n;
    f.step_blocks = (step_n + LR_STEP_WAVES - 1) / LR_STEP_WAVES;
    switch (e->plan.H) {
        case 40: return lr_launch_fused_h<40>(e, a, f, stream);
        case 72: return lr_launch_fused_h<72>(e, a, f, stream);
        case 136: return lr_launch_fused_h<136>(e, a, f, stream);
        case 264: return lr_launch_fused_h<264>(e, a, f, stream);
        default: return LR_ERR_SIZE;
    }
}

static int lr_enqueue_unit(const lr_engine* e, const lr_step_args& a, const lr_part& q, hipStream_t stream) {
    if (!q.pipelined) {
        int rc = lr_enqueue_scan_range(e, q.base, q.count, stream);
        if (rc) return rc;
        return lr_enqueue_step_range(e, a, 0, q.base, q.count, stream);
    }
    int rc = lr_enqueue_fused(e, a, q.base + q.hA, q.count - q.hA, q.base, q.hA, stream);
    if (rc) return rc;
    return lr_enqueue_fused(e, a, q.base, q.hA, q.base + q.hA, q.count - q.hA, stream);
}

static int lr_run_units(lr_engine* e, const lr_step_args& a, lr_part& q, int64_t units, hipStream_t stream) {
    int64_t done = 0;
    const int G = lr_graph_iters();
    if (G > 0 && units >= G) {
        if (!q.graph_exec) {
            hipStream_t cs = nullptr;
            hipGraph_t graph = nullptr;
            hipError_t he = hipStreamCreateWithFlags(&cs, hipStreamNonBlocking);
            if (he != hipSuccess) return (int)he;
            int rc = LR_OK;
            he = hipStreamBeginCapture(cs, hipStreamCaptureModeThreadLocal);
            if (he == hipSuccess) {
                for (int i = 0; i < G && rc == LR_OK; ++i) rc = lr_enqueue_unit(e, a, q, cs);
                he = hipStreamEndCapture(cs, &graph);
            }
            if (he == hipSuccess && rc == LR_OK) he = hipGraphInstantiate(&q.graph_exec, graph, nullptr, nullptr, 0);
            if (graph) (void)hipGraphDestroy(graph);
            (void)hipStreamDestroy(cs);
            if (rc) return rc;
            if (he != hipSuccess) return (int)he;
            q.graph_units = G;
        }
        while (units - done >= q.graph_units) {
            hipError_t he = hipGraphLaunch(q.graph_exec, stream);
            if (he != hipSuccess) return (int)he;
            done += q.graph_units;
        }
    }
    for (; done < units; ++done) {
        const int rc = lr_enqueue_unit(e, a, q, stream);
        if (rc) return rc;
    }
    return LR_OK;
}

static int lr_run_part(lr_engine* e, const lr_step_args& a, lr_part& q, int64_t n_iters, hipStream_t stream) {
    if (!q.pipelined) return lr_run_units(e, a, q, n_iters, stream);
    int rc = lr_enqueue_fused(e, a, q.base, q.hA, q.base, 0, stream);
    if (rc) return rc;
    rc = lr_run_units(e, a, q, n_iters - 1, stream);
    if (rc) return rc;
    rc = lr_enqueue_fused(e, a, q.base + q.hA, q.count - q.hA, q.base, q.hA, stream);
    if (rc) return rc;
    return lr_enqueue_step_range(e, a, 0, q.base + q.hA, q.count - q.hA, stream);
}

extern "C" int lr_mcmc_steps(lr_engine* e, int64_t n_iters, void* stream_) {
    if (!e) return LR_ERR_NULL;
    if (!e->initialised) return LR_ERR_STATE;
    if (n_iters < 0) return LR_ERR_SIZE;
    if (n_iters == 0) return LR_OK;
    hipStream_t stream = (hipStream_t)stream_;
    const lr_step_args a = lr_make_args(e);
    if (e->persistent) {
        const uint4* idx8 = (const uint4*)(e->ws + e->lay.lineage_idx);
        const bool general = e->plan.unit == LR_TAB_PAIRGEN;
        lr_packed_lineages pk;
        pk.idx8 = idx8, pk.frac = general ? (const uint4*)(e->ws + e->lay.lineage_frac) : nullptr, pk.fstride = e->n8_alloc;
        if (e->n8 <= 0) return LR_ERR_STATE;
        const lr_step_args* ap = (const lr_step_args*)(e->ws + e->lay.args_blob);
        const int blocks = (e->cfg.n_chains + 1) / 2;
        const bool p4 = e->lay.persistent == 2;
        const bool param = e->cfg.sampler != 0;
        static const int prio = lr_env_int("LR_PERSIST_PRIO", 12);
        const bool wide = e->lay.reserved1 == 1024;
        if (e->lay.persistent == 3) return lr_launch_spec(e, a, pk, n_iters, stream);
        for (int64_t done = 0; done < n_iters;) {
            const int64_t n = (n_iters - done > 4096) ? 4096 : n_iters - done;
        static const int carry_env = lr_env_int("LR_P4_CARRY", 1);
        char* p4_carry = (p4 && carry_env) ? e->ws + e->lay.xchg : nullptr;
#define LR_P_LAUNCH(HH)                                                                                                       \
    if (p4) {                                                                                                                 \
        const dim3 g4((e->cfg.n_chains + 3) / 4), b4(LR_P4_THREADS);                                                          \
        if (general && param) hipLaunchKernelGGL((lr_persist4_kernel<HH, true, true>), g4, b4, 0, stream, ap, pk, e->n8, e->p4, (long long)n, p4_carry);   \
        else if (general) hipLaunchKernelGGL((lr_persist4_kernel<HH, true, false>), g4, b4, 0, stream, ap, pk, e->n8, e->p4, (long long)n, p4_carry);      \
        else if (param) hipLaunchKernelGGL((lr_persist4_kernel<HH, false, true>), g4, b4, 0, stream, ap, pk, e->n8, e->p4, (long long)n, p4_carry);        \
        else if (e->p4_help)                                                 \
            hipLaunchKernelGGL((lr_persist4_kernel<(HH <= 264 ? HH : 264), false, false, true>), g4, b4, 0, stream, ap, pk, e->n8, e->p4, (long long)n, p4_carry); \
        else hipLaunchKernelGGL((lr_persist4_kernel<HH, false, false>), g4, b4, 0, stream, ap, pk, e->n8, e->p4, (long long)n, p4_carry);                  \
    } else if (wide) {                                                                                                        \
        hipLaunchKernelGGL((lr_persist_kernel<HH, 1024>), dim3(blocks), dim3(1024), 0, stream, ap, idx8, e->n8, e->p4, (long long)n, 0); \
    } else {                                                                                                                  \
        hipLaunchKernelGGL((lr_persist_kernel<HH, 512>), dim3(blocks), dim3(512), 0, stream, ap, idx8, e->n8, e->p4, (long long)n, prio); \
    }
            switch (e->plan.H) {
                case 40: LR_P_LAUNCH(40); break;
                case 72: LR_P_LAUNCH(72); break;
                case 136: LR_P_LAUNCH(136); break;
                case 264: LR_P_LAUNCH(264); break;
                default: LR_P_LAUNCH(LR_H_WIDE); break;
            }
#undef LR_P_LAUNCH
            const int rc = (int)hipGetLastError();
            if (rc) return rc;
            done += n;
        }
        return LR_OK;
    }
    if (e->streaming) return lr_launch_stream(e, a, n_iters, false, stream);
    if (e->n_parts == 1) return lr_run_part(e, a, e->part[0], n_iters, stream);
    hipError_t he = hipEventRecord(e->fork, stream);
    if (he != hipSuccess) return (int)he;
    for (int p = 0; p < e->n_parts; ++p) {
        lr_part& q = e->part[p];
        he = hipStreamWaitEvent(q.stream, e->fork, 0);
        if (he != hipSuccess) return (int)he;
        const int rc = lr_run_part(e, a, q, n_iters, q.stream);
        if (rc) return rc;
        he = hipEventRecord(q.done, q.stream);
        if (he != hipSuccess) return (int)he;
        he = hipStreamWaitEvent(stream, q.done, 0);
        if (he != hipSuccess) return (int)he;
    }
    return LR_OK;
}

extern "C" int lr_mcmc_time_steps(lr_engine* e, int64_t n_iters, float* total_ms, void* stream_) {
    if (!e || !total_ms) return LR_ERR_NULL;
    hipStream_t stream = (hipStream_t)stream_;
    int rc = (int)hipEventRecord(e->ev0, stream);
    if (rc == LR_OK) rc = lr_mcmc_steps(e, n_iters, stream_);
    if (rc == LR_OK) rc = (int)hipEventRecord(e->ev1, stream);
    if (rc == LR_OK) rc = (int)hipEventSynchronize(e->ev1);
    float ms = 0.f;
    if (rc == LR_OK) rc = (int)hipEventElapsedTime(&ms, e->ev0, e->ev1);
    *total_ms = ms;
    return rc;
}

extern "C" int lr_mcmc_time_scan(lr_engine* e, int32_t reps, float* avg_ms, void* stream_) {
    if (!e || !avg_ms) return LR_ERR_NULL;
    if (!e->initialised) return LR_ERR_STATE;
    if (reps < 1) return LR_ERR_SIZE;
    hipStream_t stream = (hipStream_t)stream_;
    int rc = lr_enqueue_scan(e, stream);
    if (rc == LR_OK) rc = (int)hipEventRecord(e->ev0, stream);
    for (int i = 0; i < reps && rc == LR_OK; ++i) rc = lr_enqueue_scan(e, stream);
    if (rc == LR_OK) rc = (int)hipEventRecord(e->ev1, stream);
    if (rc == LR_OK) rc = (int)hipEventSynchronize(e->ev1);
    float ms = 0.f;
    if (rc == LR_OK) rc = (int)hipEventElapsedTime(&ms, e->ev0, e->ev1);
    *avg_ms = ms / reps;
    return rc;
}

extern "C" int lr_mcmc_status(lr_engine* e, int32_t* status, void* stream_) {
    if (!e || !status) return LR_ERR_NULL;
    unsigned int v = 0;
    hipError_t he = hipMemcpyAsync(&v, e->ws + e->lay.status, sizeof(v), hipMemcpyDeviceToHost, (hipStream_t)stream_);
    if (he == hipSuccess) he = hipStreamSynchronize((hipStream_t)stream_);
    *status = (int32_t)v;
    return (int)he;
}

extern "C" int lr_mcmc_warnings(lr_engine* e, int32_t* warnings, void* stream_) {
    if (!e || !warnings) return LR_ERR_NULL;
    unsigned int v = 0;
    hipError_t he = hipMemcpyAsync(&v, e->ws + e->lay.status + 4, sizeof(v), hipMemcpyDeviceToHost, (hipStream_t)stream_);
    if (he == hipSuccess) he = hipStreamSynchronize((hipStream_t)stream_);
    *warnings = (int32_t)v;
    return (int)he;
}

extern "C" int lr_mcmc_describe(const lr_engine* e, char* buf, int32_t n) {
    if (!e || !buf) return LR_ERR_NULL;
    if (n < 64) return LR_ERR_SIZE;
    if (e->persistent) {
        const char* gen = e->plan.unit == LR_TAB_PAIRGEN ? "true" : "false";
        if (e->lay.persistent == 3)
            snprintf(buf, (size_t)n, "lr_spec_kernel<%d, %d, %s, %s, %d>", e->plan.H, e->lay.reserved1, e->cfg.sampler == 0 ? "true" : "false", gen,
                     lr_spec_mode(e));
        else if (e->lay.persistent == 2)
            snprintf(buf, (size_t)n, "lr_persist4_kernel<%d, %s, %s, %s>", e->plan.H, gen, e->cfg.sampler != 0 ? "true" : "false",
                     e->p4_help ? "true" : "false");
        else snprintf(buf, (size_t)n, "lr_persist_kernel<%d, %d>", e->plan.H, e->lay.reserved1);
    } else if (e->packed_scan) {
        snprintf(buf, (size_t)n, "lr_packscan_kernel<%d, %d, %s>", lr_packscan_pairs(e->plan, e->cfg.n_chains), e->plan.H,
                 e->plan.unit == LR_TAB_PAIRGEN ? "true" : "false");
    } else if (e->streaming) {
        snprintf(buf, (size_t)n, "lr_stream_kernel<%d, %d, %s>", e->plan.cb, e->plan.H, e->plan.unit ? "true" : "false");
    } else if (e->part[0].pipelined) {
        snprintf(buf, (size_t)n, "lr_fused_iter_kernel<%d, %d, %s>", e->plan.cb, e->plan.H, e->plan.unit ? "true" : "false");
    } else if (e->plan.fast && !e->plan.unit && e->plan.cb == 16) {
        snprintf(buf, (size_t)n, "lr_scan_wide_kernel<%d>", e->plan.H);
    } else if (e->plan.fast) {
        snprintf(buf, (size_t)n, "%s<%d, %d>", e->plan.unit ? "lr_scan_unit_kernel" : "lr_scan_fast_kernel", e->plan.cb, e->plan.H);
    } else {
        snprintf(buf, (size_t)n, "lr_scan_kernel<%d>", e->plan.cb);
    }
    return LR_OK;
}

extern "C" int lr_mcmc_destroy(lr_engine* e) {
    if (!e) return LR_ERR_NULL;
    for (int p = 0; p < e->n_parts; ++p) {
        lr_part& q = e->part[p];
        if (q.graph_exec) (void)hipGraphExecDestroy(q.graph_exec);
        if (q.done) (void)hipEventDestroy(q.done);
        if (q.stream) (void)hipStreamDestroy(q.stream);
    }
    if (e->fork) (void)hipEventDestroy(e->fork);
    if (e->ev0) (void)hipEventDestroy(e->ev0);
    if (e->ev1) (void)hipEventDestroy(e->ev1);
    delete e;
    return LR_OK;
}

#ifdef LR_DIAG
extern "C" int lr_diag_dump_step(unsigned long long* host_out, int n_words) {
    return (int)hipMemcpyFromSymbol(host_out, HIP_SYMBOL(lr_diag_step), (size_t)n_words * 8);
}
extern "C" int lr_diag_dump_seg(unsigned long long* host_out, int n_words, int reset) {
    int rc = (int)hipMemcpyFromSymbol(host_out, HIP_SYMBOL(lr_diag_seg), (size_t)n_words * 8);
    if (reset) {
        static unsigned long long zeros[64 * 16];
        rc = (int)hipMemcpyToSymbol(HIP_SYMBOL(lr_diag_seg), zeros, sizeof(zeros));
    }
    return rc;
}
#endif
```

literate_amd/csrc/lr_pack.hip:

```cpp
#include <cmath>
#include <cstdio>
#include <cstdlib>
#include <cstring>

#include <rocprim/rocprim.hpp>

#include "lr_engine.h"

static int lr_env_int_pack(const char* name, int dflt) {
    const char* v = getenv(name);
    return v ? atoi(v) : dflt;
}

__device__ __forceinline__ int lr_birth_index(double s, double t0, int n_bins) {
    return min(max(__double2int_rz(floor(s) - t0), -1), n_bins) + 1;
}
__device__ __forceinline__ int lr_death_index(double e, double t0, int n_bins) {
    return min(max(__double2int_rz(ceil(e) - t0), 0), n_bins + 1);
}

__global__ void lr_pack_runs_kernel(const double* __restrict__ ts, long long n, double t0, int n_bins,
                                    int* __restrict__ start_cand) {
    const long long i = (long long)blockIdx.x * blockDim.x + threadIdx.x;
    if (i >= n) return;
    const int a = lr_birth_index(ts[i], t0, n_bins);
    const int ap = i > 0 ? lr_birth_index(ts[i - 1], t0, n_bins) : -1;
    start_cand[i] = (a != ap) ? (int)i : 0;
}

__device__ __forceinline__ long long lr_share_permute(long long g, int k_tot, const lr_p4_shares& sh) {
    const int stride = sh.n_slots * 64;
    const int slot = (int)(g % stride) / 64, trip = (int)(g / stride), lane = (int)(g % 64);
    if (sh.delta[slot] < 0 && trip >= k_tot + sh.delta[slot]) {
        int r = trip - (k_tot + sh.delta[slot]);
        for (int q = 0; q < slot; ++q) r += sh.delta[q] < 0 ? -sh.delta[q] : 0;
        int to = 0;
        for (; to < sh.n_slots; ++to) {
            const int extra = sh.delta[to] > 0 ? sh.delta[to] : 0;
            if (r < extra) break;
            r -= extra;
        }
        g = (long long)(k_tot + r) * stride + to * 64 + lane;
    }
    return g;
}

__device__ __forceinline__ int lr_pack_death_entry(const double* __restrict__ ts, const double* __restrict__ te, long long i,
                                                   double t0, int n_bins, int extant_block, double end_time, bool* extant) {
    const double e = te[i];
    *extant = extant_block && e >= end_time;
    return *extant ? n_bins + 2 + lr_birth_index(ts[i], t0, n_bins) : lr_death_index(e, t0, n_bins);
}
__device__ __forceinline__ bool lr_pack_pairable(const double* __restrict__ ts, const double* __restrict__ te, long long i,
                                                 const int* __restrict__ run_start, double t0, int n_bins, int extant_block,
                                                 double end_time, int dmax) {
    if (i == 0 || run_start[i] == (int)i) return false;
    bool x0, x1;
    const int d0 = lr_pack_death_entry(ts, te, i - 1, t0, n_bins, extant_block, end_time, &x0);
    const int d1 = lr_pack_death_entry(ts, te, i, t0, n_bins, extant_block, end_time, &x1);
    return !x0 && !x1 && d1 >= d0 && d1 - d0 <= dmax;
}
__global__ void lr_pack_stretch_kernel(const double* __restrict__ ts, const double* __restrict__ te, long long n, double t0,
                                       int n_bins, const int* __restrict__ run_start, int extant_block, double end_time,
                                       int dmax, int* __restrict__ cand) {
    const long long i = (long long)blockIdx.x * blockDim.x + threadIdx.x;
    if (i >= n) return;
    cand[i] = lr_pack_pairable(ts, te, i, run_start, t0, n_bins, extant_block, end_time, dmax) ? 0 : (int)i;
}
__global__ void lr_pack_heads_kernel(const int* __restrict__ stretch_start, long long n, int* __restrict__ head) {
    const long long i = (long long)blockIdx.x * blockDim.x + threadIdx.x;
    if (i >= n) return;
    head[i] = (((int)i - stretch_start[i]) & 1) ? 0 : 1;
}
__global__ void lr_pack_slot_flags_kernel(const int* __restrict__ run_start, const int* __restrict__ stretch_start,
                                          const int* __restrict__ head_incl, long long n, int* __restrict__ flag) {
    const long long i = (long long)blockIdx.x * blockDim.x + threadIdx.x;
    if (i >= n) return;
    const bool head = !(((int)i - stretch_start[i]) & 1);
    const int slot = head_incl[i] - head_incl[run_start[i]];
    flag[i] = (head && slot % LR_SLOTS == 0) ? 1 : 0;
}
__global__ void lr_pack_slots_kernel(const double* __restrict__ ts, const double* __restrict__ te, long long n, double t0,
                                     int n_bins, int H, const int* __restrict__ run_start, const int* __restrict__ stretch_start,
                                     const int* __restrict__ head_incl, const int* __restrict__ group_incl, int permute,
                                     int k_tot, long long share_base, lr_p4_shares sh, unsigned short* __restrict__ out, int extant_block,
                                     double end_time, unsigned int* __restrict__ frac, long long fstride) {
    const long long i = (long long)blockIdx.x * blockDim.x + threadIdx.x;
    if (i >= n) return;
    if (((int)i - stretch_start[i]) & 1) return;
    const int rs = run_start[i];
    const int slot_in_run = head_incl[i] - head_incl[rs];
    const int slot = slot_in_run % LR_SLOTS;
    long long g = group_incl[i] - 1;
    if (permute && g >= share_base) g = share_base + lr_share_permute(g - share_base, k_tot, sh);
    unsigned short* grp = out + g * 8;
    bool x0;
    const int d0 = lr_pack_death_entry(ts, te, i, t0, n_bins, extant_block, end_time, &x0);
    const bool pair = i + 1 < n && stretch_start[i + 1] == stretch_start[i];
    int entry = H + d0;
    if (pair) {
        bool x1;
        const int d1 = lr_pack_death_entry(ts, te, i + 1, t0, n_bins, extant_block, end_time, &x1);
        entry = (2 + (d1 - d0)) * H + d0;
    }
    grp[1 + slot] = (unsigned short)(entry << 4);
    auto fix = [](double f) { return fmin(rint(f * 4294967296.0), 4294967295.0); };
    if (frac) {
        const double s0 = ts[i], e0 = te[i];
        double fe = x0 ? fix(s0 - floor(s0)) : fix(ceil(e0) - e0);
        if (pair) {
            const double e1 = te[i + 1];
            fe = fmin(rint((fe + fix(ceil(e1) - e1)) * 0.5), 4294967295.0);
        }
        frac[((size_t)(slot >> 2) * fstride + g) * 4 + (slot & 3)] = (unsigned int)fe;
    }
    if (slot == 0) {
        const int a = lr_birth_index(ts[i], t0, n_bins);
        int cnt = 0, slots = 0;
        long long k = i;
        while (slots < LR_SLOTS && k < n && run_start[k] == rs) {
            const bool pr = k + 1 < n && stretch_start[k + 1] == stretch_start[k];
            cnt += pr ? 2 : 1, k += pr ? 2 : 1, ++slots;
        }
        grp[0] = (unsigned short)((a << 4) | cnt);
        for (int q = slots; q < LR_SLOTS; ++q) grp[1 + q] = (unsigned short)(H << 4);
        if (frac) {
            double sum = 0.0;
            for (long long m = i; m < k; ++m) {
                const double sm = ts[m];
                sum += fix(sm - floor(sm));
            }
            unsigned int* q = frac + ((size_t)2 * fstride + g) * 4;
            q[0] = (unsigned int)__double2loint(sum), q[1] = (unsigned int)__double2hiint(sum);
        }
    }
}

struct lr_max_op {
    __host__ __device__ int operator()(int a, int b) const { return a > b ? a : b; }
};

static size_t lr_scan_tmp_bytes(long long n) {
    size_t b1 = 0, b2 = 0;
    (void)rocprim::inclusive_scan(nullptr, b1, (const int*)nullptr, (int*)nullptr, (size_t)n, lr_max_op());
    (void)rocprim::inclusive_scan(nullptr, b2, (const int*)nullptr, (int*)nullptr, (size_t)n, rocprim::plus<int>());
    return (b1 > b2 ? b1 : b2) + 256;
}

long long lr_pack_tmp_bytes(long long n) {
    return (long long)(4 * lr_align_up64(n * 4, 256) + (long long)lr_scan_tmp_bytes(n) + 256);
}

static void lr_set_shares(lr_engine* e) {
    static const char* env = getenv("LR_P4_SHARES");
    static const int env2 = lr_env_int_pack("LR_P2_SHARE", 0);
    for (int j = 0; j < 16; ++j) e->p4.delta[j] = 0;
    e->p4.help_trips = 0;
    e->p4_help = lr_p4_help_choice(e);
    if (e->lay.persistent == 2 && e->p4_help) {
        static const int env_t = lr_env_int_pack("LR_P4_HELP_TRIPS", -1);
        const double t = ((double)e->n8 + 512.0) / 896.0;
        int h = (int)lrint(t - 3.5);
        h = h < 0 ? 0 : (h > 5 ? 5 : h);
        e->p4.help_trips = env_t >= 0 ? env_t : h;
        if (e->p4.help_trips < 0) e->p4.help_trips = 0;
        if ((long long)e->p4.help_trips * 128 > e->n8) e->p4.help_trips = 0;
    }
    if (e->lay.persistent == 0 || e->lay.persistent == 3) {
        e->p4.n_slots = 8;
    } else if (e->lay.persistent == 2) {
        e->p4.n_slots = e->p4_help ? 12 : 14;
        int base[7] = {0, 0, 0, 0, 0, 0, 0};
        if (env && e->p4.n_slots == 14) sscanf(env, "%d,%d,%d,%d,%d,%d,%d", &base[0], &base[1], &base[2], &base[3], &base[4], &base[5], &base[6]);
        const long long behind = e->p4_help ? (long long)e->p4.help_trips * 128 : 0;
        const int per = e->p4.n_slots * 64;
        const int k_tot = (int)((e->n8 - behind + per - 1) / per);
        int sum = 0;
        for (int j = 0; j < 7; ++j) {
            int d = (k_tot >= 6) ? (int)lrint((double)base[j] * k_tot / 14.0) : 0;
            if (d < -(k_tot - 1)) d = -(k_tot - 1);
            if (d > LR_P4_MAX_GIVE) d = LR_P4_MAX_GIVE;
            e->p4.delta[2 * j] = e->p4.delta[2 * j + 1] = d;
            sum += d;
        }
        for (int guard = 0; sum != 0 && guard < 64; ++guard) {
            int pick = 0;
            for (int j = 1; j < 7; ++j)
                if (sum > 0 ? e->p4.delta[2 * j] > e->p4.delta[2 * pick] : e->p4.delta[2 * j] < e->p4.delta[2 * pick]) pick = j;
            const int step = sum > 0 ? -1 : 1;
            e->p4.delta[2 * pick] += step, e->p4.delta[2 * pick + 1] += step;
            sum += step;
        }
        if (sum != 0) for (int j = 0; j < 14; ++j) e->p4.delta[j] = 0;
    } else {
        const bool wide2 = e->lay.reserved1 == 1024;
        e->p4.n_slots = wide2 ? 16 : 8;
        const int k_tot = (int)((e->n8 + e->p4.n_slots * 64 - 1) / (e->p4.n_slots * 64));
        int d = (k_tot >= 12) ? (int)lrint((double)env2 * k_tot / 24.0) : 0;
        if (d > LR_P4_MAX_GIVE) d = LR_P4_MAX_GIVE;
        if (e->p4.n_slots == 8)
            for (int j = 0; j < 4; ++j) e->p4.delta[j] = d, e->p4.delta[4 + j] = -d;
        if (e->p4.n_slots == 16 && k_tot >= 6) {
            static const char* envw = getenv("LR_P2W_SHARES");
            int a = 5, b = 2;
            if (envw) sscanf(envw, "%d,%d", &a, &b);
            int da = (int)lrint((double)a * k_tot / 12.0), db = (int)lrint((double)b * k_tot / 12.0);
            if (da > LR_P4_MAX_GIVE) da = LR_P4_MAX_GIVE;
            if (db > LR_P4_MAX_GIVE) db = LR_P4_MAX_GIVE;
            if (da > k_tot - 1) da = k_tot - 1;
            if (db > k_tot - 1) db = k_tot - 1;
            for (int j = 0; j < 4; ++j) e->p4.delta[j] = da, e->p4.delta[4 + j] = db, e->p4.delta[8 + j] = -db, e->p4.delta[12 + j] = -da;
        }
    }
    const long long stride = (long long)e->p4.n_slots * 64;
    const long long k_tot = (e->n8 + stride - 1) / stride;
    int dmax = 0;
    for (int j = 0; j < 16; ++j) dmax = e->p4.delta[j] > dmax ? e->p4.delta[j] : dmax;
    if ((k_tot + dmax + 1) * stride + (e->p4_help ? (long long)e->p4.help_trips * 128 : 0) > e->n8_alloc)
        for (int j = 0; j < 16; ++j) e->p4.delta[j] = 0;
}

int lr_pack_lineages(lr_engine* e, hipStream_t stream) {
    const long long n = e->cfg.n_lineages;
    if (n >= (1ll << 31)) return LR_ERR_SIZE;
    const bool general = e->plan.unit == LR_TAB_PAIRGEN;
    const int extant_block = e->cfg.model == LR_MODEL_KEIDING_DEAD ? 1 : 0;
    char* tmp = e->ws + e->lay.pack_tmp;
    const long long arr = lr_align_up64(n * 4, 256);
    int* run_start = (int*)tmp;
    int* group_incl = (int*)(tmp + arr);
    int* stretch_start = (int*)(tmp + 2 * arr);
    int* head_incl = (int*)(tmp + 3 * arr);
    char* scan_tmp = tmp + 4 * arr;
    size_t scan_bytes = lr_scan_tmp_bytes(n);
    const dim3 grid((unsigned)((n + 255) / 256)), blk(256);
    hipLaunchKernelGGL(lr_pack_runs_kernel, grid, blk, 0, stream, e->ts, n, e->cfg.t0, e->cfg.n_bins, group_incl);
    hipError_t he = rocprim::inclusive_scan(scan_tmp, scan_bytes, (const int*)group_incl, run_start, (size_t)n, lr_max_op(), stream);
    if (he != hipSuccess) return (int)he;
    {
        hipLaunchKernelGGL(lr_pack_stretch_kernel, grid, blk, 0, stream, e->ts, e->te, n, e->cfg.t0, e->cfg.n_bins,
                           (const int*)run_start, extant_block, e->cfg.end_time, general ? 0 : LR_PAIR_DMAX, group_incl);
        scan_bytes = lr_scan_tmp_bytes(n);
        he = rocprim::inclusive_scan(scan_tmp, scan_bytes, (const int*)group_incl, stretch_start, (size_t)n, lr_max_op(), stream);
        if (he != hipSuccess) return (int)he;
        hipLaunchKernelGGL(lr_pack_heads_kernel, grid, blk, 0, stream, (const int*)stretch_start, n, group_incl);
        scan_bytes = lr_scan_tmp_bytes(n);
        he = rocprim::inclusive_scan(scan_tmp, scan_bytes, (const int*)group_incl, head_incl, (size_t)n, rocprim::plus<int>(), stream);
        if (he != hipSuccess) return (int)he;
        hipLaunchKernelGGL(lr_pack_slot_flags_kernel, grid, blk, 0, stream, (const int*)run_start, (const int*)stretch_start,
                           (const int*)head_incl, n, group_incl);
    }
    scan_bytes = lr_scan_tmp_bytes(n);
    he = rocprim::inclusive_scan(scan_tmp, scan_bytes, (const int*)group_incl, group_incl, (size_t)n, rocprim::plus<int>(), stream);
    if (he != hipSuccess) return (int)he;
    int n_groups = 0;
    he = hipMemcpyAsync(&n_groups, group_incl + (n - 1), sizeof(int), hipMemcpyDeviceToHost, stream);
    if (he == hipSuccess) he = hipStreamSynchronize(stream);
    if (he != hipSuccess) return (int)he;
    if (n_groups < 1 || (long long)n_groups + LR_IDX_SPARE > e->n8_alloc) return LR_ERR_ORDER;
    e->n8 = n_groups;
    lr_set_shares(e);
    he = hipMemsetAsync(e->ws + e->lay.lineage_idx, 0, (size_t)e->n8_alloc * 16, stream);
    if (he == hipSuccess && general) he = hipMemsetAsync(e->ws + e->lay.lineage_frac, 0, (size_t)e->n8_alloc * 16 * LR_FRAC_ARRAYS, stream);
    if (he != hipSuccess) return (int)he;
    bool any = false;
    for (int j = 0; j < 16; ++j) any |= e->p4.delta[j] != 0;
    const long long share_base = (e->lay.persistent == 2 && e->p4_help) ? (long long)e->p4.help_trips * 128 : 0;
    const int k_tot = (int)((e->n8 - share_base + e->p4.n_slots * 64 - 1) / (e->p4.n_slots * 64));
    hipLaunchKernelGGL(lr_pack_slots_kernel, grid, blk, 0, stream, e->ts, e->te, n, e->cfg.t0, e->cfg.n_bins, e->plan.H,
                       (const int*)run_start, (const int*)stretch_start, (const int*)head_incl, (const int*)group_incl,
                       any ? 1 : 0, k_tot, share_base, e->p4, (unsigned short*)(e->ws + e->lay.lineage_idx), extant_block, e->cfg.end_time,
                       general ? (unsigned int*)(e->ws + e->lay.lineage_frac) : nullptr, (long long)e->n8_alloc);
    return (int)hipGetLastError();
}
```

literate_amd/csrc/lr_step.h:

```cpp
#pragma once
#include "lr_chain.h"
#include "lr_dd.h"
#include "lr_internal.h"
#include "lr_scan.h"

struct lr_step_args {
    lr_mcmc_config cfg;
    double* state_f64;
    int* state_i32;
    const double* log_br;
    double2* tables;
    const double* partials;
    double* trace;
    const double* br_length;
    double log_T;
    double mult_l;
    const double* dd_consts;
    int tab_stride, n_cls, tiles, H, unit, cb;
    unsigned int* warn;
};

__device__ __forceinline__ double2* lr_chain_table(const lr_step_args& a, int c) {
    if (!a.unit) return a.tables + (size_t)c * a.tab_stride;
    if (a.unit == LR_TAB_PAIRGEN)
// ... 368 lines not shown
        case 11: h = s.g1; break;
        case 12: h = s.poi; break;
    }
    if (lane < LR_TRACE_HEAD) row[lane] = h;
    const double nan = __longlong_as_double(0x7ff8000000000000LL);
    double* rl = row + LR_TRACE_HEAD;
    double* rm = rl + (2 * LR_KMAX - 1);
    if (lane < LR_KMAX) rl[lane] = lane < s.KL ? s.L : nan, rm[lane] = lane < s.KM ? s.M : nan;
    if (lane >= 1 && lane < LR_KMAX) {
        rl[LR_KMAX + lane - 1] = lane < s.KL ? s.tL : nan;
        rm[LR_KMAX + lane - 1] = lane < s.KM ? s.tM : nan;
    }
}

struct lr_rj_draws {
    double log_u;
    double r_a, r_b, q_a, q_b, q2_a, q2_b;
    double beta;
    double x, m, da;
};

__device__ __forceinline__ void lr_make_rj_draws(const lr_step_args& a, int c, int lane, uint64_t it, lr_rj_draws& d) {
    const lr_mcmc_config& cfg = a.cfg;
    const lr_stream rng{(uint32_t)cfg.seed, (uint32_t)(cfg.chain_offset + c)};
    const uint32_t purpose = (lane == 0) ? LR_P_ACCEPT : (lane == 1 ? LR_P_MOVE : LR_P_RJ);
    const lr_u2 ud = lr_pair(rng, it, purpose, lane == 3 ? 1u : 0u);
    const double lu = lr_log(lane == 0 ? ud.a : 1.0);
    d.log_u = lr_bcast(lu, 0);
    d.r_a = lr_bcast(ud.a, 1), d.r_b = lr_bcast(ud.b, 1);
    d.q_a = lr_bcast(ud.a, 2), d.q_b = lr_bcast(ud.b, 2);
    d.q2_a = lr_bcast(ud.a, 3), d.q2_b = lr_bcast(ud.b, 3);
    d.x = 0.0, d.m = 1.0, d.da = 1.0, d.beta = 0.0;
    if (d.r_a < 0.8) {
        const lr_u2 u = lr_pair(rng, it, LR_P_MULT, lane);
        d.da = u.a;
        d.x = a.mult_l * (u.b - .5);
        d.m = exp(d.x);
    } else if (d.r_a < 0.999 && cfg.const_rates == 0 && d.q_b > 0.5) {
        double ga, gb;
        lr_wave_gamma2(rng, it, LR_P_BETA_A, LR_SHAPE_BETA_RJ, LR_P_BETA_B, LR_SHAPE_BETA_RJ, lane, &ga, &gb);
        d.beta = ga / (ga + gb);
    }
}

struct lr_draw_slot {
    double sc[8];
    double x[LR_ROW], m[LR_ROW], da[LR_ROW];
};

__device__ __forceinline__ void lr_draws_store(lr_draw_slot* q, const lr_rj_draws& d, int lane) {
    double so = d.log_u;
    so = (lane == 1) ? d.r_a : so;
    so = (lane == 2) ? d.r_b : so;
    so = (lane == 3) ? d.q_a : so;
    so = (lane == 4) ? d.q_b : so;
    so = (lane == 5) ? d.q2_a : so;
    so = (lane == 6) ? d.q2_b : so;
    so = (lane == 7) ? d.beta : so;
    if (lane < 8) q->sc[lane] = so;
    q->x[lane] = d.x, q->m[lane] = d.m, q->da[lane] = d.da;
}

__device__ __forceinline__ void lr_draws_load(const lr_draw_slot* q, lr_rj_draws& d, int lane) {
    const double v = q->sc[lane & 7];
    d.log_u = lr_bcast(v, 0), d.r_a = lr_bcast(v, 1), d.r_b = lr_bcast(v, 2), d.q_a = lr_bcast(v, 3);
    d.q_b = lr_bcast(v, 4), d.q2_a = lr_bcast(v, 5), d.q2_b = lr_bcast(v, 6), d.beta = lr_bcast(v, 7);
    d.x = q->x[lane], d.m = q->m[lane], d.da = q->da[lane];
}

__device__ __forceinline__ void lr_spec_draw(const lr_step_args& a, int c, int lane, unsigned long long it,
                                             lr_draw_slot* out) {
    lr_rj_draws d;
    lr_make_rj_draws(a, c, lane, it, d);
    lr_draws_store(out, d, lane);
}

__device__ __forceinline__ void lr_spec_draw_part(const lr_step_args& a, int c, int lane, unsigned long long it,
                                                  lr_draw_slot* out, int part) {
    const lr_mcmc_config& cfg = a.cfg;
    const lr_stream rng{(uint32_t)cfg.seed, (uint32_t)(cfg.chain_offset + c)};
    if (part) {
        const lr_u2 u = lr_pair(rng, it, LR_P_MULT, lane);
        const double x = a.mult_l * (u.b - .5);
        out->x[lane] = x, out->m[lane] = exp(x), out->da[lane] = u.a;
    } else {
        const uint32_t purpose = (lane == 0) ? LR_P_ACCEPT : (lane == 1 ? LR_P_MOVE : LR_P_RJ);
        const lr_u2 ud = lr_pair(rng, it, purpose, lane == 3 ? 1u : 0u);
        const double lu = lr_log(lane == 0 ? ud.a : 1.0);
        const double r_a = lr_bcast(ud.a, 1), q_b = lr_bcast(ud.b, 2);
        double beta = 0.0;
        if (!(r_a < 0.8) && r_a < 0.999 && cfg.const_rates == 0 && q_b > 0.5) {
            double ga, gb;
            lr_wave_gamma2(rng, it, LR_P_BETA_A, LR_SHAPE_BETA_RJ, LR_P_BETA_B, LR_SHAPE_BETA_RJ, lane, &ga, &gb);
            beta = ga / (ga + gb);
        }
        double so = lu;
        so = (lane == 1) ? r_a : so;
        so = (lane == 2) ? lr_bcast(ud.b, 1) : so;
        so = (lane == 3) ? lr_bcast(ud.a, 2) : so;
        so = (lane == 4) ? q_b : so;
        so = (lane == 5) ? lr_bcast(ud.a, 3) : so;
        so = (lane == 6) ? lr_bcast(ud.b, 3) : so;
        so = (lane == 7) ? beta : so;
        if (lane < 8) out->sc[lane] = so;
    }
}

#define LR_UD_LANE 32
static_assert(LR_KMAX <= LR_UD_LANE && LR_UD_LANE + 4 <= LR_WAVE, "one lane per rate below the wave-uniform draws");

__device__ __forceinline__ double lr_wave_multiplier_pre(double& R, int K, bool ff, double x, double m, int lane) {
    const bool active = (lane < K) && ff;
    if (active) R = R * m;
    return lr_wave_sum(active ? x : 0.0);
}

__device__ __forceinline__ void lr_spec_draw_both(const lr_step_args& a, int c, int lane, unsigned long long it, lr_draw_slot* out) {
    const lr_mcmc_config& cfg = a.cfg;
    const lr_stream rng{(uint32_t)cfg.seed, (uint32_t)(cfg.chain_offset + c)};
    const int ul = lane - LR_UD_LANE;
    const uint32_t purpose = (ul < 0) ? LR_P_MULT : ((ul == 0) ? LR_P_ACCEPT : (ul == 1 ? LR_P_MOVE : LR_P_RJ));
    const lr_u2 u = lr_pair(rng, it, purpose, ul < 0 ? (uint32_t)lane : (ul == 3 ? 1u : 0u));
    const double x = a.mult_l * (u.b - .5);
    out->x[lane] = x, out->m[lane] = exp(x), out->da[lane] = u.a;
    const double lu = lr_log(ul == 0 ? u.a : 1.0);
    const double r_a = lr_bcast(u.a, LR_UD_LANE + 1), q_b = lr_bcast(u.b, LR_UD_LANE + 2);
    double beta = 0.0;
    if (!(r_a < 0.8) && r_a < 0.999 && cfg.const_rates == 0 && q_b > 0.5) {
        double ga, gb;
        lr_wave_gamma2(rng, it, LR_P_BETA_A, LR_SHAPE_BETA_RJ, LR_P_BETA_B, LR_SHAPE_BETA_RJ, lane, &ga, &gb);
        beta = ga / (ga + gb);
    }
    double so = lr_bcast(lu, LR_UD_LANE);
    so = (lane == 1) ? r_a : so;
    so = (lane == 2) ? lr_bcast(u.b, LR_UD_LANE + 1) : so;
    so = (lane == 3) ? lr_bcast(u.a, LR_UD_LANE + 2) : so;
    so = (lane == 4) ? q_b : so;
    so = (lane == 5) ? lr_bcast(u.a, LR_UD_LANE + 3) : so;
    so = (lane == 6) ? lr_bcast(u.b, LR_UD_LANE + 3) : so;
    so = (lane == 7) ? beta : so;
    if (lane < 8) out->sc[lane] = so;
}

struct lr_table_hand {
    int epoch;
    int KL, KM;
    int reuse;
    int noop;
    int out_idx, base_idx;
    int pad_;
    double par[8];
};

template <bool LDS_CONSTS = false, int PB = 0, int CS = 2, bool PAIR_PLANES = true, bool HAND = false>
__device__ __forceinline__ void lr_propose_rj(const lr_step_args& a, int c, int lane, lr_seg_scratch* scratch_p,
                                              uint64_t it, lr_rj_state& s, lr_rj_prop& p, double2* table,
                                              int table_es, const lr_rj_draws* pre = nullptr,
                                              const double* br_lds = nullptr, const double* logbr_lds = nullptr,
                                              const double* base_col = nullptr, int col_doubles = 0, double base_const = 0.0,
                                              lr_table_hand* hand = nullptr, int hand_epoch = 0) {
    static_assert(CS == 2 || (PB > 0 && !PAIR_PLANES), "a column of its own: one-pass builder, no pair planes");
    static_assert(!HAND || PB > 0, "a helper wave runs the one-pass builder");
    lr_seg_scratch& scratch = *scratch_p;
    const lr_mcmc_config& cfg = a.cfg;
    const int n_bins = cfg.n_bins;
    const lr_stream rng{(uint32_t)cfg.seed, (uint32_t)(cfg.chain_offset + c)};
    const double L = s.L, M = s.M, tL = s.tL, tM = s.tM;
    const int eL = s.eL, eM = s.eM, KL = s.KL, KM = s.KM;
    double g0 = s.g0, g1 = s.g1, poi = s.poi, lg0 = s.lg0, lg1 = s.lg1, lpoi = s.lpoi;
    const double priorPoiA = s.priorPoi;

    lr_u2 ud{0.0, 0.0};
    if (!pre) {
        const int ul = lane - LR_UD_LANE;
        const uint32_t purpose = (ul < 0) ? LR_P_MULT : ((ul == 0) ? LR_P_ACCEPT : (ul == 1 ? LR_P_MOVE : LR_P_RJ));
        ud = lr_pair(rng, it, purpose, ul < 0 ? (uint32_t)lane : (ul == 3 ? 1u : 0u));
    }
    const double u_next = pre ? 1.0 : lr_bcast(ud.a, LR_UD_LANE);
    LR_SSTAMP(2);

    double pL = L, pM = M, ptL = tL, ptM = tM;
    int peL = eL, peM = eM, PKL = KL, PKM = KM;
    double hasting = 0.0, priorPoi = 0.0;
    int gibbs = 0, invalid = 0, move_kind;
    const double sample_shift_mu = cfg.const_death_rate ? 0.0 : 0.5;
    const double b_freq = cfg.const_death_rate ? 0.7 : 0.4, d_freq = 0.8;
    const double fL = cfg.update_fraction, fM = cfg.const_death_rate ? 1.0 : cfg.update_fraction;
    const lr_u2 r = pre ? lr_u2{pre->r_a, pre->r_b} : lr_u2{lr_bcast(ud.a, LR_UD_LANE + 1), lr_bcast(ud.b, LR_UD_LANE + 1)};
    if (r.a < b_freq) {
        if (r.b < .5 || KL == 1) {
            if (pre) {
                hasting = lr_wave_multiplier_pre(pL, KL, pre->da < fL, pre->x, pre->m, lane);
            } else {
                hasting = lr_wave_multiplier(pL, KL, ud.a < fL, ud.b, a.mult_l, lane);
            }
            move_kind = 0;
        } else {
            peL = lr_wave_edges(tL, 0);
            move_kind = 1;
        }
    } else if (r.a < d_freq) {
        if (r.b < .5 || KM == 1) {
            if (pre) {
                hasting = lr_wave_multiplier_pre(pM, KM, pre->da < fM, pre->x, pre->m, lane);
            } else {
                hasting = lr_wave_multiplier(pM, KM, ud.a < fM, ud.b, a.mult_l, lane);
            }
            move_kind = 2;
        } else {
            peM = lr_wave_edges(tM, 0);
            move_kind = 3;
        }
    } else if (r.a < 0.999 && cfg.const_rates == 0) {
        move_kind = 4;
        const lr_u2 q = pre ? lr_u2{pre->q_a, pre->q_b} : lr_u2{lr_bcast(ud.a, LR_UD_LANE + 2), lr_bcast(ud.b, LR_UD_LANE + 2)};
        const bool sideL = q.a > sample_shift_mu;
        double R = sideL ? L : M, T = sideL ? tL : tM;
        int K = sideL ? KL : KM;
        double score = 0.0;
        const lr_u2 q2 = pre ? lr_u2{pre->q2_a, pre->q2_b} : lr_u2{lr_bcast(ud.a, LR_UD_LANE + 3), lr_bcast(ud.b, LR_UD_LANE + 3)};
        if (q.b > 0.5) {
            if (K >= LR_KMAX) {
                invalid = LR_INVALID_KCAP;
            } else {
                const int ind = min((int)(q2.a * K), K - 1);
                const double delta = q2.b * (lr_bcast(T, ind + 1) - lr_bcast(T, ind));
                double beta;
                if (pre) {
                    beta = pre->beta;
                } else {
                    double ga, gb;
                    lr_wave_gamma2(rng, it, LR_P_BETA_A, LR_SHAPE_BETA_RJ, LR_P_BETA_B, LR_SHAPE_BETA_RJ, lane, &ga, &gb);
                    beta = ga / (ga + gb);
                }
                score = lr_wave_add_shift(R, T, K, ind, delta, beta, lane);
            }
        } else if (K > 1) {
            const int idx = 1 + min((int)(q2.a * (K - 1)), K - 2);
            score = lr_wave_remove_shift(R, T, K, idx, lane);
        }
        hasting = score;
        const int E = lr_wave_edges(T, 0);
        if (sideL) pL = R, ptL = T, PKL = K, peL = E;
        else pM = R, ptM = T, PKM = K, peM = E;
        priorPoi = lr_poisson_prior(PKL, poi, lpoi) + lr_poisson_prior(PKM, poi, lpoi);
    } else {
        move_kind = 5;
        double gl = 0.0, gm = 0.0, gp = 0.0, dummy;
        if (cfg.use_rate_HP)
            lr_wave_gamma2(rng, it, LR_P_GIBBS_L, LR_HP_GAMMA_SHAPE + LR_GAMMA_SHAPE * KL, LR_P_GIBBS_M,
                           LR_HP_GAMMA_SHAPE + LR_GAMMA_SHAPE * KM, lane, &gl, &gm);
        if (cfg.poisson_HP == 0.0)
            lr_wave_gamma2(rng, it, LR_P_GIBBS_POI, LR_RJHP_SHAPE + KL + KM, LR_P_GIBBS_POI, LR_RJHP_SHAPE + KL + KM, lane,
                           &gp, &dummy);
        if (cfg.poisson_HP == 0.0) poi = gp * (1. / (LR_RJHP_RATE + 2));
        if (cfg.use_rate_HP) {
            const double sL = lr_wave_sum(lane < KL ? L : 0.0), sM = lr_wave_sum(lane < KM ? M : 0.0);
            g0 = gl * (1. / (LR_HP_GAMMA_RATE + sL));
            g1 = gm * (1. / (LR_HP_GAMMA_RATE + sM));
        }
        const double lx = lr_log(lane == 0 ? g0 : (lane == 1 ? g1 : (lane == 2 ? poi : 1.0)));
        lg0 = lr_bcast(lx, 0), lg1 = lr_bcast(lx, 1), lpoi = lr_bcast(lx, 2);
        gibbs = 1;
    }

    LR_SSTAMP(3);
    double logpL, logpM, log_u_next;
    lr_stage_segments(&scratch, pL, pM, peL, peM, PKL, PKM, lane, &logpL, &logpM, u_next, &log_u_next);
    if (pre) log_u_next = pre->log_u;

    lr_seg_cache sg{s.sgL, s.sgM, false};
    bool edges_same = false;
    if ((pre && s.sg_valid) || base_col) edges_same = PKL == KL && PKM == KM && __ballot(lane <= LR_KMAX && (peL != eL || peM != eM)) == 0ull;
    if (pre && s.sg_valid) sg.reuse = edges_same;
    const bool same_table = base_col && edges_same && (move_kind == 1 || move_kind == 3 || move_kind == 5);
    if (HAND) {
        if (lane == 0) hand->KL = PKL, hand->KM = PKM, hand->reuse = sg.reuse ? 1 : 0, hand->noop = same_table ? 1 : 0;
        LR_WAVE_LDS_ORDER();
        if (lane == 0) __hip_atomic_store(&hand->epoch, hand_epoch, __ATOMIC_RELAXED, __HIP_MEMORY_SCOPE_WORKGROUP);
    }

    LR_SSTAMP(4);
    double priorP = -INFINITY;
    {
        const double nL = lr_dpp_zero<0x130 , 0xf, 0xf>(ptL);
        const double nM = lr_dpp_zero<0x130, 0xf, 0xf>(ptM);
        const double dmin = fmin(lane < PKL ? fabs(nL - ptL) : 1e300, lane < PKM ? fabs(nM - ptM) : 1e300);
        if (__ballot(dmin <= LR_MIN_ALLOWED_T)) invalid |= LR_INVALID_GUARD;
    }
    if (!invalid) {
        const double vL = (lane < PKL) ? (logpL + lg0) - pL * g0 + lg0 : 0.0;
        const double vM = (lane < PKM) ? (logpM + lg1) - pM * g1 + lg1 : 0.0;
        priorP = lr_wave_sum(vL + vM);
        priorP += -a.log_T * (PKL - 1 + PKM - 1);
        if (priorPoi != 0.0) priorP += priorPoi;
        else priorP += priorPoiA, priorPoi = priorPoiA;
    }

    LR_SSTAMP(5);
    double constP = 0.0;
    p.table_by_helper = 0;
    if (same_table) {
        double* col = reinterpret_cast<double*>(table);
        for (int i = lane; i < col_doubles; i += LR_WAVE) col[CS * i] = base_col[CS * i];
        constP = base_const;
    } else if (HAND) {
        p.table_by_helper = 1;
    } else {
        constP = lr_build_tables_segments<PB, CS>(&scratch, peL, peM, PKL, PKM, LDS_CONSTS ? br_lds : a.br_length,
                                                  LDS_CONSTS ? logbr_lds : a.log_br, cfg.model,
                                                  n_bins, a.n_cls, a.H, table, lane,
                                                  lr_tab_mode<LDS_CONSTS>(a, table_es), cfg.frac_birth, cfg.frac_death,
                                                  table_es, pre ? &sg : nullptr);
        s.sgL = sg.packL, s.sgM = sg.packM, s.sg_valid = (pre && sg.packL != -1) ? 1 : 0;
    }
    if (LDS_CONSTS && PAIR_PLANES && !HAND && !same_table) {
        LR_WAVE_LDS_ORDER();
        if (lr_tab_mode<LDS_CONSTS>(a, table_es) == LR_TAB_UNIT) lr_pair_planes_wave(reinterpret_cast<double*>(table), a.H, n_bins, lane, 0);
        else lr_pair_planes_wave_general(reinterpret_cast<double*>(table), a.H, n_bins, lane, 0);
    }
    LR_SSTAMP(6);
    s.L = pL, s.M = pM, s.tL = ptL, s.tM = ptM, s.eL = peL, s.eM = peM, s.KL = PKL, s.KM = PKM;
    s.g0 = g0, s.g1 = g1, s.poi = poi, s.lg0 = lg0, s.lg1 = lg1, s.lpoi = lpoi, s.priorPoi = priorPoi;
    p.hasting = hasting, p.prior = priorP, p.constP = constP, p.log_u = log_u_next;
    p.gibbs = gibbs, p.invalid = invalid, p.move = move_kind;
}

template <bool LDS_CONSTS = false, int PB = 0, bool HAND = false>
__device__ __forceinline__ void lr_chain_step_core(lr_chain_regs& st, const lr_step_args& a, int mode, int c, int lane,
                                                   lr_seg_scratch* scratch_p, double lik_sum, double2* table,
                                                   int table_es = 2, const double* br_lds = nullptr,
                                                   const double* logbr_lds = nullptr, const lr_rj_draws* pre = nullptr,
                                                   lr_table_hand* hand = nullptr, int hand_epoch = 0) {
    const lr_mcmc_config& cfg = a.cfg;
    const double sc = st.sc;
    const int isc = st.isc;
    double lik_p = lr_bcast(sc, LR_S_LIK_P);
    double likA = lr_bcast(sc, LR_S_LIKA), priorA = lr_bcast(sc, LR_S_PRIORA);
    double constA = lr_bcast(sc, LR_S_CONST_A);
    lr_rj_state s;
    s.L = st.L, s.M = st.M, s.tL = st.tL, s.tM = st.tM, s.eL = st.eL, s.eM = st.eM;
    s.KL = lr_bcast_i(isc, LR_I_KL), s.KM = lr_bcast_i(isc, LR_I_KM);
    s.g0 = lr_bcast(sc, LR_S_GRATE_L), s.g1 = lr_bcast(sc, LR_S_GRATE_M), s.poi = lr_bcast(sc, LR_S_POI);
    s.lg0 = lr_bcast(sc, LR_S_LOG_G0), s.lg1 = lr_bcast(sc, LR_S_LOG_G1), s.lpoi = lr_bcast(sc, LR_S_LOG_POI);
    s.priorPoi = lr_bcast(sc, LR_S_PRIORPOIA);
    s.sgL = s.sgM = 0, s.sg_valid = 0;
    uint64_t it = (uint64_t)(uint32_t)lr_bcast_i(isc, LR_I_IT_LO) | ((uint64_t)(uint32_t)lr_bcast_i(isc, LR_I_IT_HI) << 32);
    int n_acc = lr_bcast_i(isc, LR_I_ACCEPTED);
    uint64_t next_sample = (uint64_t)(uint32_t)lr_bcast_i(isc, LR_I_NEXT_LO) | ((uint64_t)(uint32_t)lr_bcast_i(isc, LR_I_NEXT_HI) << 32);
    int trace_slot = lr_bcast_i(isc, LR_I_SLOT);
    LR_SSTAMP(1);

    if (mode == 1) {
        likA = lik_sum + constA;
        priorA = lr_wave_prior_gamma(s.L, s.KL, LR_GAMMA_SHAPE, 2.0, lane) + lr_wave_prior_gamma(s.M, s.KM, LR_GAMMA_SHAPE, 2.0, lane);
        priorA += -a.log_T * (s.KL - 1 + s.KM - 1);
        s.priorPoi = lr_poisson_prior(s.KL, s.poi, s.lpoi) + lr_poisson_prior(s.KM, s.poi, s.lpoi);
        priorA += s.priorPoi;
    } else {
        const int gibbs = lr_bcast_i(isc, LR_I_GIBBS), invalid = lr_bcast_i(isc, LR_I_INVALID);
        const double priorP = lr_bcast(sc, LR_S_PRIOR_P), constP = lr_bcast(sc, LR_S_CONST_P);
        double lik;
        const bool ok = lr_mh_accept(gibbs, invalid, lik_sum, constP, likA, priorP, priorA, lr_bcast(sc, LR_S_HASTING),
                                     lr_bcast(sc, LR_S_LOG_U), &lik) && mode != 2;
        lik_p = invalid ? -INFINITY : lik;
        lr_warn_kcap(a.warn, invalid, lane);
        if (ok) {
            s.L = st.pL, s.M = st.pM, s.tL = st.ptL, s.tM = st.ptM, s.eL = st.peL, s.eM = st.peM;
            s.KL = lr_bcast_i(isc, LR_I_PKL), s.KM = lr_bcast_i(isc, LR_I_PKM);
            likA = lik, priorA = priorP, s.priorPoi = lr_bcast(sc, LR_S_PRIORPOI_P), constA = constP;
            n_acc += 1;
        }
        if (it == next_sample) {
            const int slot = trace_slot;
            trace_slot += 1;
            next_sample += (uint64_t)cfg.s_freq;
            if (slot < cfg.n_trace_slots) lr_write_trace_row(a, c, lane, slot, it, likA, priorA, s);
        }
        it += 1;
    }
    const double priorPoiA = s.priorPoi;
    st.L = s.L, st.M = s.M, st.tL = s.tL, st.tM = s.tM, st.eL = s.eL, st.eM = s.eM;
    const int KL = s.KL, KM = s.KM;

    lr_rj_prop p;
    if (HAND) lr_propose_rj<LDS_CONSTS, (PB > 0 ? PB : 1), 2, true, HAND>(a, c, lane, scratch_p, it, s, p, table, table_es, pre, br_lds, logbr_lds, nullptr, 0, 0.0, hand, hand_epoch);
    else lr_propose_rj<LDS_CONSTS, PB>(a, c, lane, scratch_p, it, s, p, table, table_es, pre, br_lds, logbr_lds);

    st.pL = s.L, st.pM = s.M, st.ptL = s.tL, st.ptM = s.tM, st.peL = s.eL, st.peM = s.eM;
    {
        double so = 0.0;
        so = (lane == LR_S_LIKA) ? likA : so;
        so = (lane == LR_S_PRIORA) ? priorA : so;
        so = (lane == LR_S_PRIORPOIA) ? priorPoiA : so;
        so = (lane == LR_S_GRATE_L) ? s.g0 : so;
        so = (lane == LR_S_GRATE_M) ? s.g1 : so;
        so = (lane == LR_S_POI) ? s.poi : so;
        so = (lane == LR_S_HASTING) ? p.hasting : so;
        so = (lane == LR_S_PRIOR_P) ? p.prior : so;
        so = (lane == LR_S_PRIORPOI_P) ? s.priorPoi : so;
        so = (lane == LR_S_CONST_P) ? p.constP : so;
        so = (lane == LR_S_CONST_A) ? constA : so;
        so = (lane == LR_S_LIK_P) ? lik_p : so;
        so = (lane == LR_S_LOG_G0) ? s.lg0 : so;
        so = (lane == LR_S_LOG_G1) ? s.lg1 : so;
        so = (lane == LR_S_LOG_POI) ? s.lpoi : so;
        so = (lane == LR_S_LOG_U) ? p.log_u : so;
        st.sc = so;
        int io = 0;
        io = (lane == LR_I_KL) ? KL : io;
        io = (lane == LR_I_KM) ? KM : io;
        io = (lane == LR_I_PKL) ? s.KL : io;
        io = (lane == LR_I_PKM) ? s.KM : io;
        io = (lane == LR_I_GIBBS) ? p.gibbs : io;
        io = (lane == LR_I_INVALID) ? p.invalid : io;
        io = (lane == LR_I_IT_LO) ? (int)(uint32_t)it : io;
        io = (lane == LR_I_IT_HI) ? (int)(uint32_t)(it >> 32) : io;
        io = (lane == LR_I_ACCEPTED) ? n_acc : io;
        io = (lane == LR_I_MOVE) ? p.move : io;
        io = (lane == LR_I_NEXT_LO) ? (int)(uint32_t)next_sample : io;
        io = (lane == LR_I_NEXT_HI) ? (int)(uint32_t)(next_sample >> 32) : io;
        io = (lane == LR_I_SLOT) ? trace_slot : io;
        st.isc = io;
    }
    LR_SSTAMP(7);

}


struct lr_dd_prop {
    double hasting, prior, log_u;
    int move;
};
struct lr_dd_draws {
    double log_u, rr_a, rr_b, slide_u, z1;
    double da, x, m;
};
__device__ __forceinline__ void lr_make_dd_draws(const lr_step_args& a, int c, int lane, uint64_t it, lr_dd_draws& d) {
    const lr_mcmc_config& cfg = a.cfg;
    const bool trend = cfg.sampler == 2;
    const lr_stream rng{(uint32_t)cfg.seed, (uint32_t)(cfg.chain_offset + c)};
    const uint32_t purpose = trend ? (lane == 0 ? LR_P_TR_ACCEPT : LR_P_TR_MOVE)
                                   : (lane == 0 ? LR_P_DD_ACCEPT : (lane == 1 ? LR_P_DD_MOVE : LR_P_DD_SLIDE));
    const lr_u2 ud = lr_pair(rng, it, purpose, 0u);
    const double lu = lr_log(lane == 0 ? ud.a : 1.0);
    d.log_u = lr_bcast(lu, 0);
    d.rr_a = lr_bcast(ud.a, 1), d.rr_b = lr_bcast(ud.b, 1), d.slide_u = lr_bcast(ud.a, 2);
    d.z1 = 0.0, d.da = 1.0, d.x = 0.0, d.m = 1.0;
    if (trend) {
        const lr_u2 u = lr_pair(rng, it, LR_P_TR_MULT, lane);
        d.da = u.a;
        if (d.rr_a < .33) {
            d.x = lr_normal(rng, it, LR_P_TR_NORM, lane);
        } else {
            d.x = a.mult_l * (u.b - .5);
            d.m = exp(d.x);
        }
    } else if (d.rr_b < 0.1 && (cfg.m_birth == 2 || cfg.m_death == 2)) {
        if (cfg.m_death == -1) d.z1 = lr_normal(rng, it, LR_P_DD_SLIDE, 1);
    } else {
        const lr_u2 u = lr_pair(rng, it, LR_P_DD_MULT, lane);
        d.da = u.a;
        d.x = a.mult_l * (u.b - .5);
        d.m = exp(d.x);
    }
}

template <bool LDS_CONSTS, bool PAIR_PLANES, int CS>
__device__ __forceinline__ void lr_param_tables(const lr_step_args& a, double P, const double* aux, double2* table, int mode,
                                                int table_es, int lane) {
    const lr_mcmc_config& cfg = a.cfg;
    if (cfg.sampler == 2) {
        const lr_trend_params tp = lr_trend_unpack(P);
        lr_rates_build_tables_wave<CS>([&](int b, double* br, double* dr) { lr_trend_bin_rates(tp, aux[b], cfg.m_birth, cfg.m_death, br, dr); },
                                       cfg.n_bins, a.H, table, lane, mode, cfg.frac_birth, cfg.frac_death, table_es);
    } else {
        const lr_dd_params pp = lr_dd_unpack(P);
        lr_dd_build_tables_wave<CS>(pp, aux, cfg.m_birth, cfg.m_death, cfg.n_bins, a.H, table, lane, mode, cfg.frac_birth, cfg.frac_death,
                                    table_es);
    }
    if (LDS_CONSTS && PAIR_PLANES) {
        LR_WAVE_LDS_ORDER();
        if (mode == LR_TAB_UNIT) lr_pair_planes_wave(reinterpret_cast<double*>(table), a.H, cfg.n_bins, lane, 0);
        else lr_pair_planes_wave_general(reinterpret_cast<double*>(table), a.H, cfg.n_bins, lane, 0);
    }
}

template <bool LDS_CONSTS = false, bool PAIR_PLANES = true, int CS = 2, bool HAND = false>
__device__ __forceinline__ double lr_propose_dd(const lr_step_args& a, int c, int lane, uint64_t it, double A,
                                                lr_dd_prop& p, double2* table, int table_es,
                                                const double* aux_lds = nullptr, const lr_dd_draws* pre = nullptr,
                                                lr_table_hand* hand = nullptr, int hand_epoch = 0) {
    static_assert(CS == 2 || !PAIR_PLANES, "a column of its own carries no pair planes");
    const lr_mcmc_config& cfg = a.cfg;
    const bool trend = cfg.sampler == 2;
    const int npar = trend ? LR_TR_NPAR : LR_DD_NPAR;
    const lr_stream rng{(uint32_t)cfg.seed, (uint32_t)(cfg.chain_offset + c)};
    const double origin = cfg.t0, present = cfg.dd_present;
    const double k0 = a.dd_consts[0], log_k0 = a.dd_consts[1];
    const double* aux = LDS_CONSTS ? aux_lds : a.br_length;
    const uint32_t purpose = trend ? (lane == 0 ? LR_P_TR_ACCEPT : LR_P_TR_MOVE)
                                   : (lane == 0 ? LR_P_DD_ACCEPT : (lane == 1 ? LR_P_DD_MOVE : LR_P_DD_SLIDE));
    lr_u2 ud{0.0, 0.0};
    if (!pre) ud = lr_pair(rng, it, purpose, 0u);
    p.log_u = pre ? pre->log_u : lr_bcast(lr_log(lane == 0 ? ud.a : 1.0), 0);
    double P = A, hasting = 0.0;
    int move_kind;
    if (trend) {
        const double rr = pre ? pre->rr_a : lr_bcast(ud.a, 1);
        double f_mult, f_norm;
        lr_trend_update_freq(cfg.m_birth, cfg.m_death, lane, &f_mult, &f_norm);
        lr_u2 d{0.0, 0.0};
        if (!pre) d = lr_pair(rng, it, LR_P_TR_MULT, lane);
        const double da = pre ? pre->da : d.a;
        if (rr < .33) {
            const double z = pre ? pre->x : lr_normal(rng, it, LR_P_TR_NORM, lane);
            if (lane < npar && da < f_norm) P = A + z * .001;
            move_kind = 1;
        } else {
            hasting = pre ? lr_wave_multiplier_pre(P, npar, da < f_mult, pre->x, pre->m, lane)
                          : lr_wave_multiplier(P, npar, da < f_mult, d.b, a.mult_l, lane);
            move_kind = 0;
        }
    } else {
        const lr_u2 rr = pre ? lr_u2{pre->rr_a, pre->rr_b} : lr_u2{lr_bcast(ud.a, 1), lr_bcast(ud.b, 1)};
        if (rr.b < 0.1 && (cfg.m_birth == 2 || cfg.m_death == 2)) {
            double ii = lr_bcast(A, 2) + ((pre ? pre->slide_u : lr_bcast(ud.a, 2)) - .5) * 1.5;
            if (ii > present) ii = present - (ii - present);
            ii = fabs(ii);
            if (lane == 2) P = ii;
            if (cfg.m_death == -1) {
                const double z = pre ? pre->z1 : lr_normal(rng, it, LR_P_DD_SLIDE, 1);
                if (lane == 1) P = A + z * 0.2;
            }
            move_kind = 1;
        } else {
            const double f = lr_dd_update_freq(cfg.m_birth, cfg.m_death, lane);
            if (pre) {
                hasting = lr_wave_multiplier_pre(P, npar, pre->da < f, pre->x, pre->m, lane);
            } else {
                const lr_u2 d = lr_pair(rng, it, LR_P_DD_MULT, lane);
                hasting = lr_wave_multiplier(P, npar, d.a < f, d.b, a.mult_l, lane);
            }
            move_kind = 0;
        }
    }
    if (HAND) {
        if (lane < 8) hand->par[lane] = P;
        LR_WAVE_LDS_ORDER();
        if (lane == 0) __hip_atomic_store(&hand->epoch, hand_epoch, __ATOMIC_RELAXED, __HIP_MEMORY_SCOPE_WORKGROUP);
        p.prior = trend ? lr_trend_prior(P, lane) : lr_dd_prior(P, origin, present, k0, log_k0, lane);
    } else {
        if (trend) p.prior = lr_trend_prior(P, lane);
        else p.prior = lr_dd_prior(P, origin, present, k0, log_k0, lane);
        lr_param_tables<LDS_CONSTS, PAIR_PLANES, CS>(a, P, aux, table, lr_tab_mode<LDS_CONSTS>(a, table_es), table_es, lane);
    }
    p.hasting = hasting, p.move = move_kind;
    return P;
}

__device__ __forceinline__ bool lr_dd_accept(double lik, double likA, double priorP, double priorA, double hasting,
                                             double log_u, uint64_t it) {
    return ((lik - likA) + (priorP - priorA) + hasting > log_u) || it == 0;
}

__device__ __forceinline__ void lr_dd_write_trace_row(const lr_step_args& a, int c, int lane, int slot, uint64_t it,
                                                      double likA, double priorA, double A) {
    const int npar = a.cfg.sampler == 2 ? LR_TR_NPAR : LR_DD_NPAR;
    double* row = a.trace + ((size_t)slot * a.cfg.n_chains + c) * LR_TRACE_W;
    double h = __longlong_as_double(0x7ff8000000000000LL);
    if (lane == 0) h = (double)it;
    if (lane == 1) h = likA + priorA;
    if (lane == 2) h = likA;
    if (lane == 3) h = priorA;
    const double Aj = __shfl(A, (lane - 4) & (LR_WAVE - 1));
// ... 110 lines not shown
```

literate_amd/engine.py:

```python
import ctypes as C
import hashlib
import os
from collections import namedtuple

import numpy as np

from . import _hip, ops


class ChainEngine:
    def __init__(self, ts, te, n_chains, model=0, seed=1, const_rates=0, const_death_rate=0, use_rate_HP=1,
                 poisson_HP=0.0, update_fraction=0.75, s_freq=1000, n_trace_slots=0, chain_offset=0,
                 device=None, stats=None, sort_lineages=True, unit_resolution=None, engine="auto", dd=None, team=0,
                 chains_per_team=0):
        torch = _hip.require_gpu()
        self.lib = _hip.load()
        self.device = torch.device(device or "cuda")
        ts_d = ops._dev(ts, torch.float64, self.device)
        te_d = ops._dev(te, torch.float64, self.device)
        if sort_lineages:
            o1 = torch.sort(te_d, stable=True).indices
            o2 = torch.sort(torch.floor(ts_d[o1]), stable=True).indices
            order = o1[o2]
            ts_d, te_d = ts_d[order].contiguous(), te_d[order].contiguous()
# ... 26 lines not shown
            engine_mode={"auto": 0, "launch": 1, "persistent": 2, "persistent4": 3, "persistent2": 4, "spec": 5, "stream": 6, "packed": 7}[engine],
            frac_birth=fs0 if self.unit_resolution else 0.0, frac_death=fe0 if self.unit_resolution else 0.0,
            sampler=0 if dd is None else (2 if dd.get("kind") == "trend" else 1),
            m_birth=0 if dd is None else int(dd["m_birth"]), m_death=0 if dd is None else int(dd["m_death"]),
            team_request=(int(team) or (1 if os.environ.get("LR_SHARED_DEVICE", "0") == "1" else 0)) | (int(chains_per_team) << 8),
            dd_present=0.0 if dd is None else float(dd.get("present", 0.0)),
            dd_init_death=0.0 if dd is None else float(dd.get("init_death", 0.1)))
        self.dd = dd
        self.layout = _hip.McmcLayout()
        with torch.cuda.device(self.device):
            _hip.check(self.lib.lr_mcmc_query_layout(C.byref(self.cfg), C.byref(self.layout)), "lr_mcmc_query_layout")
        self.workspace = torch.zeros(self.layout.total_bytes, dtype=torch.uint8, device=self.device)
        handle = C.c_void_p()
        br_ptr = _hip.ptr(self.br_length) if (model in (0, 1) or dd is not None) else None
        with torch.cuda.device(self.device):
            _hip.check(self.lib.lr_mcmc_create(C.byref(self.cfg), _hip.ptr(self.ts), _hip.ptr(self.te), br_ptr,
                                               _hip.ptr(self.workspace), self.workspace.numel(), C.byref(handle)),
                       "lr_mcmc_create")
        self.handle = handle
        self.n_chains = int(n_chains)
        self.iterations = 0
        self._hash = None
        self._plan_args = dict(model=model, const_rates=const_rates, const_death_rate=const_death_rate, use_rate_HP=use_rate_HP,
                               poisson_HP=poisson_HP, update_fraction=update_fraction, unit_resolution=self.unit_resolution, dd=dd,
                               stats=(self.t0, self.n_bins, self.br_length))
        self.plan_report = None
        if engine == "auto" and os.environ.get("LR_PLAN_CHECK", "0") == "1" and not ChainEngine._in_plan_check:
            self.plan_report = self.plan_check()

    _in_plan_check = False

    def plan_check(self, n_iters=200, tolerance=0.10):
        import warnings
        torch = _hip.require_gpu()
        ChainEngine._in_plan_check = True
        times = {}
        try:
            for name in ("auto", "persistent4", "persistent2", "spec", "packed", "launch"):
                try:
                    e = ChainEngine(self.ts, self.te, self.n_chains, seed=int(self.cfg.seed), s_freq=1 << 30, n_trace_slots=2,
                                    chain_offset=int(self.cfg.chain_offset), device=self.device, sort_lineages=False,
                                    engine=name, **self._plan_args)
                except (ValueError, _hip.HipLibraryError):
                    times[name] = None
                    continue
                try:
                    e.init()
                    e.steps(n_iters)
                    torch.cuda.synchronize(self.device)
                    times[name] = e.timed_steps(n_iters) / n_iters * 1e3
                    if name == "auto":
                        auto_kernel = e.kernel_name()
                finally:
                    e.close()
        finally:
            ChainEngine._in_plan_check = False
        valid = {k: v for k, v in times.items() if v is not None and k != "auto"}
        best = min(valid, key=valid.get)
        ok = times["auto"] <= (1.0 + tolerance) * valid[best]
        if not ok:
            warnings.warn("LR_PLAN_CHECK: the planner chose %s (%.2f us per iteration) but engine=%r runs this configuration "
                          "in %.2f us on this device: pass engine=%r, and refit the planner's model (csrc/lr_mcmc.hip)"
                          % (auto_kernel, times["auto"], best, valid[best], best), RuntimeWarning)
        return dict(auto=auto_kernel, us_per_iter=times, best=best, ok=bool(ok))

    @property
    def _data_hash(self):
        if self._hash is None:
            h = hashlib.sha1(self.ts.cpu().numpy().tobytes())
            h.update(self.te.cpu().numpy().tobytes())
            self._hash = h.hexdigest()
        return self._hash

    def _view(self, off, dtype, shape):
        torch = _hip.require_gpu()
        n = int(np.prod(shape))
        item = torch.empty((), dtype=dtype).element_size()
        return self.workspace[off:off + n * item].view(dtype).view(*shape)

    @property
    def state_f64(self):
        import torch
        return self._view(self.layout.state_f64, torch.float64, (self.n_chains, _hip.LR_STATE_ROWS, _hip.LR_ROW))

    @property
    def state_i32(self):
        import torch
        return self._view(self.layout.state_i32, torch.int32, (self.n_chains, _hip.LR_ISTATE_ROWS, _hip.LR_ROW))

    @property
    def trace(self):
        import torch
        return self._view(self.layout.trace, torch.float64,
                          (self.cfg.n_trace_slots, self.n_chains, _hip.LR_TRACE_W))

    def init(self, L=None, M=None, tL=None, tM=None):
        import torch
        if L is None:
            rc = _hip.launch(self.lib.lr_mcmc_init, self.device, self.handle, None, None, None, None, None, None, 0)
        elif self.dd is not None:
            npar = 6 if self.dd.get("kind") == "trend" else 8
            args = np.zeros((self.n_chains, _hip.LR_KMAX))
            args[:, :npar] = np.asarray(L, dtype=float).reshape(self.n_chains, npar)
            self._init_keep = [ops._dev(args, torch.float64, self.device)]
            rc = _hip.launch(self.lib.lr_mcmc_init, self.device, self.handle, _hip.ptr(self._init_keep[0]), None, None, None,
                             None, None, _hip.LR_KMAX)
        else:
            kmax = _hip.LR_KMAX
            Ls = np.zeros((self.n_chains, kmax)); Ms = np.zeros((self.n_chains, kmax))
            tLs = np.zeros((self.n_chains, kmax + 1)); tMs = np.zeros((self.n_chains, kmax + 1))
            KL = np.zeros(self.n_chains, dtype=np.int32); KM = np.zeros(self.n_chains, dtype=np.int32)
            for c in range(self.n_chains):
                l, m = np.atleast_1d(L[c]), np.atleast_1d(M[c])
                KL[c], KM[c] = len(l), len(m)
                Ls[c, :len(l)], Ms[c, :len(m)] = l, m
                tLs[c, :len(l) + 1], tMs[c, :len(m) + 1] = tL[c], tM[c]
            dev = [ops._dev(x, torch.float64, self.device) for x in (Ls, Ms, tLs, tMs)]
            dk = [ops._dev(x, torch.int32, self.device) for x in (KL, KM)]
            self._init_keep = dev + dk
            rc = _hip.launch(self.lib.lr_mcmc_init, self.device, self.handle, *[_hip.ptr(x) for x in dev + dk], kmax)
        _hip.check(rc, "lr_mcmc_init")
        self.iterations = 0

    def _launch(self, fn, *args):
        import torch
        idx = self.device.index
        if idx is None or torch.cuda.current_device() == idx:
            return fn(*args, C.c_void_p(torch.cuda.current_stream().cuda_stream))
        return _hip.launch(fn, self.device, *args)

    def steps(self, n):
        _hip.check(self._launch(self.lib.lr_mcmc_steps, self.handle, int(n)), "lr_mcmc_steps")
        self.iterations += int(n)

    def time_scan(self, reps=20):
        ms = C.c_float(0.0)
        _hip.check(_hip.launch(self.lib.lr_mcmc_time_scan, self.device, self.handle, int(reps), C.byref(ms)),
                   "lr_mcmc_time_scan")
        return float(ms.value)

    def check_status(self):
        st = C.c_int32(0)
        _hip.check(_hip.launch(self.lib.lr_mcmc_status, self.device, self.handle, C.byref(st)), "lr_mcmc_status")
        if st.value != 0:
            raise _hip.HipLibraryError("engine status %d: a wait between blocks timed out (the kernel's blocks were not all "
                                       "resident: is the GPU shared? LR_SHARED_DEVICE=1 runs without teams, LR_STREAM=0 "
                                       "without the resident streaming kernel), the run is void" % st.value)

    def warnings(self):
        w = C.c_int32(0)
        _hip.check(_hip.launch(self.lib.lr_mcmc_warnings, self.device, self.handle, C.byref(w)), "lr_mcmc_warnings")
        return int(w.value)

    def warning_text(self):
        w = self.warnings()
        if w & _hip.LR_WARN_KCAP:
            return ("WARNING: an add-shift move was proposed from a state with %d rates and rejected: the device holds at "
                    "most %d rates per process (the reference has no cap, LiteRateForward.py:29-47); the posterior of "
                    "the number of shifts is truncated there" % (_hip.LR_KMAX, _hip.LR_KMAX))
        return ""

    def kernel_name(self):
        buf = C.create_string_buffer(128)
        _hip.check(self.lib.lr_mcmc_describe(self.handle, buf, 128), "lr_mcmc_describe")
        return buf.value.decode()

    def timed_steps(self, n):
        ms = C.c_float(0.0)
        _hip.check(self._launch(self.lib.lr_mcmc_time_steps, self.handle, int(n), C.byref(ms)), "lr_mcmc_time_steps")
        self.iterations += int(n)
        return float(ms.value)

    def prepared_timed_steps(self, n):
        import torch
        ms = C.c_float(0.0)
        fn, handle, n_c, ms_ref = self.lib.lr_mcmc_time_steps, self.handle, C.c_int64(int(n)), C.byref(ms)
        with torch.cuda.device(self.device):
            stream = C.c_void_p(torch.cuda.current_stream(self.device).cuda_stream)

        def call():
            rc = fn(handle, n_c, ms_ref, stream)
            if rc:
                _hip.check(rc, "lr_mcmc_time_steps")
            self.iterations += int(n)
            return float(ms.value)
        return call

    _CFG_KEYS = ("n_lineages", "n_bins", "n_chains", "model", "const_rates", "const_death_rate", "use_rate_HP",
                 "s_freq", "n_trace_slots", "poisson_HP", "update_fraction", "t0", "start_time", "end_time", "seed",
                 "chain_offset", "unit_resolution", "frac_birth", "frac_death", "sampler", "m_birth", "m_death",
                 "dd_present", "dd_init_death", "engine_mode")

    def _signature(self):
        sig = {k: repr(getattr(self.cfg, k)) for k in self._CFG_KEYS}
        sig.update({"layout_" + f: repr(getattr(self.layout, f)) for f, _ in self.layout._fields_})
        sig["data_sha1"] = self._data_hash
        sig["format"] = "2: state in .npz (head, tail), trace rows in .npz.trace"
        return sig

    def _trace_span(self):
        return int(self.layout.trace), int(self.layout.status)

    def checkpoint_begin(self):
        import torch
        t0, t1 = self._trace_span()
        with torch.cuda.device(self.device):
            head, tail = self.workspace[:t0].clone(), self.workspace[t1:].clone()
            ev = torch.cuda.Event()
            ev.record()
        return dict(head=head, tail=tail, ev=ev, iterations=int(self.iterations), samples=int(self.samples_done()))

    def checkpoint_write(self, ticket, path):
        import torch
        path = str(path)
        if not path.endswith(".npz"):
            path += ".npz"
        side = getattr(self, "_ckpt_stream", None)
        if side is None:
            side = self._ckpt_stream = torch.cuda.Stream(device=self.device)
        row_bytes = self.n_chains * _hip.LR_TRACE_W * 8
        s1 = ticket["samples"]
        sidecar = path + ".trace"
        saved = getattr(self, "_ckpt_saved", {}).get(path, 0)
        if saved > s1 or not os.path.exists(sidecar) or os.path.getsize(sidecar) < saved * row_bytes:
            saved = 0
        with torch.cuda.device(self.device), torch.cuda.stream(side):
            side.wait_event(ticket["ev"])
            head, tail = ticket["head"].cpu().numpy(), ticket["tail"].cpu().numpy()
            new_rows = self.trace[saved:s1].cpu().numpy() if s1 > saved else None
        side.synchronize()
        sig = self._signature()
        tmp = path + ".tmp.npz"
        np.savez(tmp, head=head, tail=tail, iterations=np.int64(ticket["iterations"]), n_trace_rows=np.int64(s1),
                 sig_keys=np.array(list(sig.keys())), sig_vals=np.array(list(sig.values())))
        if saved > 0:
            with open(sidecar, "r+b") as f:
                f.seek(saved * row_bytes)
                f.truncate()
                if new_rows is not None:
                    f.write(new_rows.tobytes())
                f.flush()
                os.fsync(f.fileno())
        else:
            with open(sidecar + ".tmp", "wb") as f:
                if new_rows is not None:
                    f.write(new_rows.tobytes())
                f.flush()
                os.fsync(f.fileno())
            os.replace(sidecar + ".tmp", sidecar)
        os.replace(tmp, path)
        if not hasattr(self, "_ckpt_saved"):
            self._ckpt_saved = {}
        self._ckpt_saved[path] = s1

    def save(self, path):
        ticket = self.checkpoint_begin()
        self.check_status()
        self.checkpoint_write(ticket, path)

    def load(self, path):
        import torch
        path = str(path)
        with np.load(path) as z:
            saved = dict(zip([str(k) for k in z["sig_keys"]], [str(v) for v in z["sig_vals"]]))
            mine = self._signature()
            bad = [k for k in mine if k not in saved or mine[k] != saved[k]]
            if bad or len(saved) != len(mine):
                raise ValueError("checkpoint was written by a different configuration: " + ", ".join(bad))
            t0, t1 = self._trace_span()
            head, tail = torch.from_numpy(z["head"]), torch.from_numpy(z["tail"])
            if head.numel() != t0 or tail.numel() != self.workspace.numel() - t1:
                raise ValueError("checkpoint workspace size differs")
            n_rows = int(z["n_trace_rows"])
            row_bytes = self.n_chains * _hip.LR_TRACE_W * 8
            if n_rows > 0:
                sidecar = path + ".trace"
                if not os.path.exists(sidecar) or os.path.getsize(sidecar) < n_rows * row_bytes:
                    raise ValueError("checkpoint trace file %s is missing or shorter than the %d rows the checkpoint holds" % (sidecar, n_rows))
                rows = np.fromfile(sidecar, dtype=np.uint8, count=n_rows * row_bytes)
                self.workspace[t0:t0 + n_rows * row_bytes].copy_(torch.from_numpy(rows).to(self.device))
            self.workspace[:t0].copy_(head.to(self.device))
            self.workspace[t1:].copy_(tail.to(self.device))
            self.iterations = int(z["iterations"])
        self._ckpt_saved = {path: n_rows}
        _hip.check(_hip.launch(self.lib.lr_mcmc_restore, self.device, self.handle), "lr_mcmc_restore")

    def close(self):
        if getattr(self, "handle", None) is not None:
            self.lib.lr_mcmc_destroy(self.handle)
            self.handle = None

    def __del__(self):
        try:
            self.close()
        except Exception:
            pass

    def snapshot(self):
        self.check_status()
        return self.snapshot_from(self.state_f64.cpu().numpy(), self.state_i32.cpu().numpy())

    def snapshot_from(self, S, I):
        KL, KM = I[:, _hip.IROW_SCALARS, _hip.I_KL], I[:, _hip.IROW_SCALARS, _hip.I_KM]
        sc = S[:, _hip.ROW_SCALARS]
        n = S.shape[0]
        return dict(
# ... 110 lines not shown
```

Measured before the change: 16160 billion.

## Skip lineage scans for invalid or no-op RJ proposals in helper persistent kernel

In the helper-wave persistent kernel, a stepper whose proposal is invalid or leaves the rate-shift edges unchanged from an accepted origin state now decides it locally, reusing the carried likelihood, and proposes again without waiting for a full lineage scan. Phases are driven by per-chain done/need status bytes in LDS, so scanners and helpers only scan when some chain needs a fresh table, and the loop ends when every chain reaches its iteration target. The intent is to remove lineage scans whose result is already known. In exchange it adds control-flow complexity, a new origin state field, uneven per-chain progress inside a launch, and new counters and an environment toggle (on by default).

```diff
diff --git a/include/literate_hip.h b/include/literate_hip.h
--- a/include/literate_hip.h
+++ b/include/literate_hip.h
@@ -224,6 +224,7 @@
 #define LR_I_NEXT_LO 10
 #define LR_I_NEXT_HI 11
 #define LR_I_SLOT 12
+#define LR_I_ORIGIN 13
 
 #define LR_TRACE_HEAD 13
 #define LR_TRACE_W (LR_TRACE_HEAD + 2 * (2 * LR_KMAX - 1))
@@ -243,6 +244,11 @@
 int lr_mcmc_status(lr_engine* e, int32_t* status , void* stream);
 #define LR_WARN_KCAP 2
 int lr_mcmc_warnings(lr_engine* e, int32_t* warnings , void* stream);
+#define LR_COUNTER_PHASES 0
+#define LR_COUNTER_SHORTCUTS 1
+#define LR_COUNTER_SCANS 2
+#define LR_COUNTERS_OFFSET 16
+int lr_mcmc_counters(lr_engine* e, int64_t* counters , void* stream);
 int lr_mcmc_describe(const lr_engine* e, char* buf , int32_t n);
 int lr_mcmc_destroy(lr_engine* e);
 
diff --git a/literate_amd/_hip.py b/literate_amd/_hip.py
--- a/literate_amd/_hip.py
+++ b/literate_amd/_hip.py
@@ -21,7 +21,7 @@
  S_CONST_A, S_LIK_P, S_LOG_G0, S_LOG_G1, S_LOG_POI) = range(15)
 IROW_EL, IROW_EM, IROW_PEL, IROW_PEM, IROW_SCALARS = range(5)
 (I_KL, I_KM, I_PKL, I_PKM, I_GIBBS, I_INVALID, I_IT_LO, I_IT_HI, I_ACCEPTED, I_MOVE, I_NEXT_LO, I_NEXT_HI,
- I_SLOT) = range(13)
+ I_SLOT, I_ORIGIN) = range(14)
 
 
 class McmcConfig(C.Structure):
@@ -86,6 +86,7 @@
     "lr_mcmc_describe": (c_i32, [c_vp, C.c_char_p, c_i32]),
     "lr_mcmc_status": (c_i32, [c_vp, C.POINTER(c_i32), c_vp]),
     "lr_mcmc_warnings": (c_i32, [c_vp, C.POINTER(c_i32), c_vp]),
+    "lr_mcmc_counters": (c_i32, [c_vp, C.POINTER(c_i64), c_vp]),
     "lr_mcmc_destroy": (c_i32, [c_vp]),
     "lr_debug_draws": (c_i32, [C.c_uint64, c_i64, c_vp, c_vp, c_vp, c_vp, c_vp, c_i32, c_vp, c_vp]),
     "lr_debug_stream2": (c_i32, [c_vp, c_vp, c_i64, c_vp, c_vp]),
diff --git a/literate_amd/csrc/lr_engine.h b/literate_amd/csrc/lr_engine.h
--- a/literate_amd/csrc/lr_engine.h
+++ b/literate_amd/csrc/lr_engine.h
@@ -35,6 +35,7 @@
     long long n8_alloc;
     lr_p4_shares p4;
     bool p4_help;
+    bool p4_shortcut;
     bool packed_scan;
     bool streaming;
     hipEvent_t fork;
@@ -77,6 +78,11 @@
     return env ? atoi(env) != 0 : true;
 }
 
+static inline bool lr_p4_shortcut_choice() {
+    const char* env = getenv("LR_P4_SHORTCUT");
+    return env ? atoi(env) != 0 : true;
+}
+
 static inline int lr_spec_mode(const lr_engine* e) {
     if (e->lay.spec_chains_per_team != 1) return 0;
     if (e->lay.team_blocks > 1) return 1;
diff --git a/literate_amd/csrc/lr_mcmc.hip b/literate_amd/csrc/lr_mcmc.hip
--- a/literate_amd/csrc/lr_mcmc.hip
+++ b/literate_amd/csrc/lr_mcmc.hip
@@ -179,13 +179,14 @@
 
 typedef __attribute__((address_space(3))) double lr_lds_f64;
 typedef __attribute__((address_space(3))) int lr_lds_i32;
-template <int PB, int ES, bool PRE = false, int SAMPLER = -1, bool HAND = false>
+template <int PB, int ES, bool PRE = false, int SAMPLER = -1, bool HAND = false, bool SKIP = false>
 __device__ __forceinline__ void lr_persist_step_body(const __attribute__((address_space(3))) lr_step_args* a3, int c, int lane,
                                                      __attribute__((address_space(3))) lr_seg_scratch* scratch3,
                                                      lr_lds_f64* st_f64, lr_lds_i32* st_i32, double lik, lr_lds_f64* table3,
                                                      lr_lds_f64* br3 ,
                                                      const lr_draw_slot* draws = nullptr ,
-                                                     lr_table_hand* hand = nullptr, int hand_epoch = 0) {
+                                                     lr_table_hand* hand = nullptr, int hand_epoch = 0,
+                                                     lr_skip_ctl* ctl = nullptr) {
     constexpr int table_es = ES;
     const lr_step_args& a = *(const lr_step_args*)a3;
     const double* br_lds = (const double*)br3;
@@ -197,8 +198,8 @@
     else if (PRE) {
         lr_rj_draws pre;
         lr_draws_load(draws, pre, lane);
-        lr_chain_step_core<true, PB, HAND>(st, a, 0, c, lane, (lr_seg_scratch*)scratch3, lik, reinterpret_cast<double2*>((double*)table3),
-                                           table_es, br_lds, br_lds + LR_H_WIDE, &pre, hand, hand_epoch);
+        lr_chain_step_core<true, PB, HAND, SKIP>(st, a, 0, c, lane, (lr_seg_scratch*)scratch3, lik, reinterpret_cast<double2*>((double*)table3),
+                                                 table_es, br_lds, br_lds + LR_H_WIDE, &pre, hand, hand_epoch, ctl);
     } else
         lr_chain_step_core<true, PB>(st, a, 0, c, lane, (lr_seg_scratch*)scratch3, lik, reinterpret_cast<double2*>((double*)table3),
                                      table_es, br_lds, br_lds + LR_H_WIDE);
@@ -236,6 +237,9 @@
     lr_persist_step_body<PB, ES>(a3, c, lane, scratch3, st_f64, st_i32, lik, table3, br3);
 }
 
+#define LR_P4_DONE 1u
+#define LR_P4_NEED 2u
+#define LR_P4_ALL_DONE 0x01010101u
 template <int PB, int ES, int NW, int SAMPLER, bool HELP>
 __device__ __attribute__((noinline)) void lr_persist4_steppers(const __attribute__((address_space(3))) lr_step_args* a3, int c0,
                                                                int n_chains, int wave, int lane,
@@ -243,8 +247,71 @@
                                                                lr_lds_f64* st_f64, lr_lds_i32* st_i32, lr_lds_f64* red,
                                                                lr_lds_f64* tab, int tab_doubles, lr_lds_f64* br3, long long n_iters,
                                                                const lr_draw_slot* draws ,
-                                                               lr_table_hand* hands ) {
+                                                               lr_table_hand* hands , lr_lds_i32* p4ctl = nullptr,
+                                                               int shortcut = 0) {
     static_assert(!HELP || (ES == 2 && SAMPLER == 0), "helper waves: RJ sampler at unit resolution");
+    if constexpr (HELP) {
+        c0 = __builtin_amdgcn_readfirstlane(c0), n_chains = __builtin_amdgcn_readfirstlane(n_chains), wave = __builtin_amdgcn_readfirstlane(wave);
+        tab_doubles = __builtin_amdgcn_readfirstlane(tab_doubles), shortcut = __builtin_amdgcn_readfirstlane(shortcut);
+        draws = (const lr_draw_slot*)lr_uniform_ptr(draws), hands = (lr_table_hand*)lr_uniform_ptr(hands);
+        uint64_t it_end[2];
+#pragma unroll
+        for (int k = 0; k < 2; ++k) {
+            const lr_lds_i32* I = st_i32 + (2 * k + wave) * (LR_ISTATE_ROWS * LR_ROW) + LR_IROW_SCALARS * LR_ROW;
+            const uint32_t lo = (uint32_t)__builtin_amdgcn_readfirstlane(I[LR_I_IT_LO]), hi = (uint32_t)__builtin_amdgcn_readfirstlane(I[LR_I_IT_HI]);
+            it_end[k] = ((uint64_t)hi << 32 | lo) + (uint64_t)n_iters;
+        }
+        unsigned int W = (unsigned int)__builtin_amdgcn_readfirstlane(p4ctl[1]);
+#pragma unroll 1
+        for (int p = 0;; ++p) {
+            const int ph = p & 1, mine = 2 * ph + wave, other = 2 * (1 - ph) + wave;
+#ifdef LR_DIAG
+            const unsigned long long dq0 = wall_clock64();
+#endif
+            unsigned int b = (W >> (8 * mine)) & 0xffu, o = (W >> (8 * other)) & 0xffu;
+            const int c = c0 + mine;
+            const int epoch = (p + 1) & 0x3fffffff;
+            if (c < n_chains) {
+                if (!(b & LR_P4_DONE)) {
+                    const double lik = red[(ph * NW + 2) * 2 + wave];
+                    lr_skip_ctl ctl{ph ? it_end[1] : it_end[0], shortcut, 0, 0, 0, 0};
+                    int decided = 0;
+#pragma unroll 1
+                    do {
+                        ctl.carried = ctl.skipped;
+                        lr_persist_step_body<PB, ES, true, SAMPLER, true, true>(
+                            a3, c, lane, scratch3, st_f64 + mine * (LR_STATE_ROWS * LR_ROW), st_i32 + mine * (LR_ISTATE_ROWS * LR_ROW), lik,
+                            tab + ph * tab_doubles + wave, br3, draws + mine, hands + wave, epoch, &ctl);
+                        decided += ctl.decided;
+                    } while (ctl.skipped);
+                    b = ctl.done ? (LR_P4_DONE | LR_P4_NEED) : LR_P4_NEED;
+                    if (lane == 0 && decided) p4ctl[2 + wave] += decided;
+                } else if (lane == 0) {
+                    hands[wave].noop = 1;
+                    LR_WAVE_LDS_ORDER();
+                    __hip_atomic_store(&hands[wave].epoch, epoch, __ATOMIC_RELAXED, __HIP_MEMORY_SCOPE_WORKGROUP);
+                }
+            }
+            if (o & LR_P4_DONE) o = LR_P4_DONE;
+            if (lane == 0) {
+                __attribute__((address_space(3))) unsigned char* wb = (__attribute__((address_space(3))) unsigned char*)(p4ctl + ph);
+                wb[mine] = (unsigned char)b, wb[other] = (unsigned char)o;
+            }
+#ifdef LR_DIAG
+            const unsigned long long dq1 = wall_clock64();
+#endif
+            __syncthreads();
+#ifdef LR_DIAG
+            if (lane == 0 && blockIdx.x < 64) {
+                atomicAdd(&lr_diag_step[16384 + (blockIdx.x * 16 + wave) * 4 + 0], dq1 - dq0);
+                atomicAdd(&lr_diag_step[16384 + (blockIdx.x * 16 + wave) * 4 + 1], wall_clock64() - dq1);
+            }
+#endif
+            W = (unsigned int)__builtin_amdgcn_readfirstlane(p4ctl[ph]);
+            if ((W & LR_P4_ALL_DONE) == LR_P4_ALL_DONE) break;
+        }
+        return;
+    }
     for (long long iter = 0; iter < n_iters; ++iter) {
 #pragma unroll 1
         for (int ph = 0; ph < 2; ++ph) {
@@ -421,7 +488,8 @@
           bool HELP = false>
 __global__ __launch_bounds__(LR_P4_THREADS, LR_P4_THREADS / 256) void lr_persist4_kernel(const lr_step_args* __restrict__ ap ,
                                                                        lr_packed_lineages pk, long long n8,
-                                                                       lr_p4_shares sh, long long n_iters, char* carry_all) {
+                                                                       lr_p4_shares sh, long long n_iters, char* carry_all,
+                                                                       int shortcut ) {
     static_assert(!HELP || (!GENERAL && !PARAM), "helper waves: RJ sampler at unit resolution");
     const lr_step_args& a = *ap;
     LR_PSTAMP(0);
@@ -444,6 +512,7 @@
     __shared__ double br_lds[2][LR_H_WIDE];
     __shared__ lr_draw_slot draws_s[4];
     lr_draw_slot* const draws = draws_s;
+    __shared__ int p4ctl[4];
     const int tid = threadIdx.x, lane = tid & (LR_WAVE - 1), wave = tid / LR_WAVE;
     if (tid < (int)(sizeof(lr_step_args) / 4)) reinterpret_cast<int*>(&a_lds)[tid] = reinterpret_cast<const int*>(ap)[tid];
     for (int b = tid; b < LR_H_WIDE; b += blockDim.x) {
@@ -452,9 +521,10 @@
         br_lds[1][b] = in ? ap->log_br[b] : 0.0;
     }
     constexpr bool draw_ahead = !GENERAL && !PARAM;
-    auto draw_duty = [&](int pr) {
+    auto draw_duty = [&](int pr, unsigned int status = 0u ) {
         const int q = wave - W0, k = q & 1, ch = 2 * pr + k;
         if (!draw_ahead || q < 0 || q >= (HELP ? 2 : 4) || (int)(blockIdx.x * 4) + ch >= ap->cfg.n_chains) return;
+        if ((status >> (8 * ch)) & LR_P4_DONE) return;
         const int* I = st_i32[ch] + LR_IROW_SCALARS * LR_ROW;
         const unsigned long long it = ((unsigned long long)(unsigned int)I[LR_I_IT_HI] << 32 | (unsigned int)I[LR_I_IT_LO]) + 1ull;
         lr_draw_slot* slot = &draws[ch];
@@ -474,6 +544,7 @@
 #ifdef LR_DIAG
         if (lane == 0 && blockIdx.x < 64) atomicAdd(&lr_diag_step[16384 + (blockIdx.x * 16 + wave) * 4 + 2], wall_clock64() - dh0);
 #endif
+        if (hand->noop) return;
         const lr_seg_scratch* sc = &scratch[k];
         const int eL = lane <= LR_KMAX ? sc->edge[0][lane] : 0, eM = lane <= LR_KMAX ? sc->edge[1][lane] : 0;
         double* tabd = reinterpret_cast<double*>(tab[ph]) + k;
@@ -486,6 +557,11 @@
     };
     if (tid == 0) arrived = 0;
     if (tid < 2) hands[tid].epoch = 0;
+    if (HELP && tid == 0) {
+        unsigned int w = 0u;
+        for (int ch = 0; ch < 4; ++ch) w |= ((int)(blockIdx.x * 4) + ch < ap->cfg.n_chains ? LR_P4_NEED : LR_P4_DONE) << (8 * ch);
+        p4ctl[0] = 0, p4ctl[1] = (int)w, p4ctl[2] = p4ctl[3] = 0;
+    }
     for (int i = tid; i < 2 * NW * 2; i += LR_P4_THREADS) (&red[0][0][0])[i] = 0.0;
     int scans_done = 0;
     constexpr int NA = NS + (HELP ? 2 : 0);
@@ -557,7 +633,56 @@
     if (helper && !carried) help_scan(0);
     __syncthreads();
     LR_PSTAMP(3);
-    if (helper) {
+    bool carry_ok = true;
+    if (HELP && (helper || scanner)) {
+        unsigned int W = (unsigned int)__builtin_amdgcn_readfirstlane(p4ctl[1]);
+        int n_phases = 0, n_scans = carried ? 0 : 1;
+        bool all_done = false;
+#pragma unroll 1
+        for (int p = 0; !all_done; p += 2) {
+#pragma unroll
+        for (int ph = 0; ph < 2 && !all_done; ++ph) {
+            const bool scan = ((W >> (16 * (1 - ph))) & (LR_P4_NEED | LR_P4_NEED << 8)) != 0u;
+            if (ph == 0 && (W & 0x0101u) != 0x0101u) carry_ok = false;
+            if (ph == 1 && scan) carry_ok = true;
+            ++n_phases, n_scans += scan ? 1 : 0;
+#ifdef LR_DIAG
+            const unsigned long long dq0 = wall_clock64();
+#endif
+            if (helper) {
+                if (scan) help_scan(1 - ph);
+                help_duty(ph, (p + ph + 1) & 0x3fffffff);
+            } else {
+                if (scan) {
+                    double s0 = 0.0, s1 = 0.0;
+                    lr_scan_tail tail;
+                    lr_persist_scan<H, GENERAL, 1, false, true>(reinterpret_cast<const char*>(tab[1 - ph]), pk, nh, n8w, sid, LR_P4_SCANNERS, &s0, &s1, nullptr, &tail);
+                    leave_sums(1 - ph, s0, s1);
+                    lr_scan_drain(tail);
+                }
+                draw_duty(1 - ph, W);
+            }
+#ifdef LR_DIAG
+            const unsigned long long dq1 = wall_clock64();
+#endif
+            __syncthreads();
+#ifdef LR_DIAG
+            if (lane == 0 && blockIdx.x < 64) {
+                atomicAdd(&lr_diag_step[16384 + (blockIdx.x * 16 + wave) * 4 + 0], dq1 - dq0);
+                atomicAdd(&lr_diag_step[16384 + (blockIdx.x * 16 + wave) * 4 + 1], wall_clock64() - dq1);
+            }
+#endif
+            W = (unsigned int)__builtin_amdgcn_readfirstlane(p4ctl[ph]);
+            all_done = (W & LR_P4_ALL_DONE) == LR_P4_ALL_DONE;
+        }
+        }
+        if (tid == W0 * LR_WAVE) {
+            unsigned long long* cnt = reinterpret_cast<unsigned long long*>(reinterpret_cast<char*>(a.warn - 1) + LR_COUNTERS_OFFSET);
+            atomicAdd(cnt + LR_COUNTER_PHASES, (unsigned long long)n_phases);
+            atomicAdd(cnt + LR_COUNTER_SHORTCUTS, (unsigned long long)(p4ctl[2] + p4ctl[3]));
+            atomicAdd(cnt + LR_COUNTER_SCANS, (unsigned long long)n_scans);
+        }
+    } else if (helper) {
         for (long long iter = 0; iter < n_iters; ++iter) {
 #pragma unroll 1
             for (int ph = 0; ph < 2; ++ph) {
@@ -583,7 +708,7 @@
             (const __attribute__((address_space(3))) lr_step_args*)&a_lds, c0, C, wave, lane,
             (__attribute__((address_space(3))) lr_seg_scratch*)&scratch[wave], (lr_lds_f64*)&st_f64[0][0], (lr_lds_i32*)&st_i32[0][0],
             (lr_lds_f64*)&red[0][0][0], (lr_lds_f64*)reinterpret_cast<double*>(tab[0]), 2 * LR_UNIT_PLANES * H,
-            (lr_lds_f64*)&br_lds[0][0], n_iters, &draws[0], &hands[0]);
+            (lr_lds_f64*)&br_lds[0][0], n_iters, &draws[0], &hands[0], (lr_lds_i32*)&p4ctl[0], shortcut);
     else
     for (long long iter = 0; iter < n_iters; ++iter) {
 #pragma unroll
@@ -624,8 +749,9 @@
         g0[i] = tab[0][e], g1[i] = tab[1][e];
     }
     if (carry) {
-        if (tid < 2 * NW) reinterpret_cast<double*>(carry)[tid] = (&red[0][0][0])[tid];
-        if (tid == 0) *reinterpret_cast<int*>(carry + 2 * NW * 8) = 1;
+        const int ct = HELP ? sid : tid;
+        if (ct >= 0 && ct < 2 * NW && carry_ok) reinterpret_cast<double*>(carry)[ct] = (&red[0][0][0])[ct];
+        if (ct == 0) *reinterpret_cast<int*>(carry + 2 * NW * 8) = carry_ok ? 1 : 0;
     }
     LR_PSTAMP(5);
 }
@@ -1081,6 +1207,7 @@
     for (int j = 0; j < 16; ++j) e->p4.delta[j] = 0;
     e->p4.n_slots = 8;
     e->p4_help = lr_p4_help_choice(e);
+    e->p4_shortcut = lr_p4_shortcut_choice();
     e->streaming = false;
     e->packed_scan = lay.packed_scan != 0;
     e->fork = nullptr;
@@ -1396,16 +1523,17 @@
         for (int64_t done = 0; done < n_iters;) {
             const int64_t n = (n_iters - done > 4096) ? 4096 : n_iters - done;
         static const int carry_env = lr_env_int("LR_P4_CARRY", 1);
+        const int shortcut_env = e->p4_shortcut ? 1 : 0;
         char* p4_carry = (p4 && carry_env) ? e->ws + e->lay.xchg : nullptr;
 #define LR_P_LAUNCH(HH)                                                                                                       \
     if (p4) {                                                                                                                 \
         const dim3 g4((e->cfg.n_chains + 3) / 4), b4(LR_P4_THREADS);                                                          \
-        if (general && param) hipLaunchKernelGGL((lr_persist4_kernel<HH, true, true>), g4, b4, 0, stream, ap, pk, e->n8, e->p4, (long long)n, p4_carry);   \
-        else if (general) hipLaunchKernelGGL((lr_persist4_kernel<HH, true, false>), g4, b4, 0, stream, ap, pk, e->n8, e->p4, (long long)n, p4_carry);      \
-        else if (param) hipLaunchKernelGGL((lr_persist4_kernel<HH, false, true>), g4, b4, 0, stream, ap, pk, e->n8, e->p4, (long long)n, p4_carry);        \
+        if (general && param) hipLaunchKernelGGL((lr_persist4_kernel<HH, true, true>), g4, b4, 0, stream, ap, pk, e->n8, e->p4, (long long)n, p4_carry, shortcut_env);   \
+        else if (general) hipLaunchKernelGGL((lr_persist4_kernel<HH, true, false>), g4, b4, 0, stream, ap, pk, e->n8, e->p4, (long long)n, p4_carry, shortcut_env);      \
+        else if (param) hipLaunchKernelGGL((lr_persist4_kernel<HH, false, true>), g4, b4, 0, stream, ap, pk, e->n8, e->p4, (long long)n, p4_carry, shortcut_env);        \
         else if (e->p4_help)                                                 \
-            hipLaunchKernelGGL((lr_persist4_kernel<(HH <= 264 ? HH : 264), false, false, true>), g4, b4, 0, stream, ap, pk, e->n8, e->p4, (long long)n, p4_carry); \
-        else hipLaunchKernelGGL((lr_persist4_kernel<HH, false, false>), g4, b4, 0, stream, ap, pk, e->n8, e->p4, (long long)n, p4_carry);                  \
+            hipLaunchKernelGGL((lr_persist4_kernel<(HH <= 264 ? HH : 264), false, false, true>), g4, b4, 0, stream, ap, pk, e->n8, e->p4, (long long)n, p4_carry, shortcut_env); \
+        else hipLaunchKernelGGL((lr_persist4_kernel<HH, false, false>), g4, b4, 0, stream, ap, pk, e->n8, e->p4, (long long)n, p4_carry, shortcut_env);                  \
     } else if (wide) {                                                                                                        \
         hipLaunchKernelGGL((lr_persist_kernel<HH, 1024>), dim3(blocks), dim3(1024), 0, stream, ap, idx8, e->n8, e->p4, (long long)n, 0); \
     } else {                                                                                                                  \
@@ -1487,6 +1615,15 @@
     hipError_t he = hipMemcpyAsync(&v, e->ws + e->lay.status + 4, sizeof(v), hipMemcpyDeviceToHost, (hipStream_t)stream_);
     if (he == hipSuccess) he = hipStreamSynchronize((hipStream_t)stream_);
     *warnings = (int32_t)v;
+    return (int)he;
+}
+
+extern "C" int lr_mcmc_counters(lr_engine* e, int64_t* counters, void* stream_) {
+    if (!e || !counters) return LR_ERR_NULL;
+    unsigned long long v[3] = {0, 0, 0};
+    hipError_t he = hipMemcpyAsync(v, e->ws + e->lay.status + LR_COUNTERS_OFFSET, sizeof(v), hipMemcpyDeviceToHost, (hipStream_t)stream_);
+    if (he == hipSuccess) he = hipStreamSynchronize((hipStream_t)stream_);
+    for (int i = 0; i < 3; ++i) counters[i] = (int64_t)v[i];
     return (int)he;
 }
 
diff --git a/literate_amd/csrc/lr_pack.hip b/literate_amd/csrc/lr_pack.hip
--- a/literate_amd/csrc/lr_pack.hip
+++ b/literate_amd/csrc/lr_pack.hip
@@ -157,6 +157,7 @@
     for (int j = 0; j < 16; ++j) e->p4.delta[j] = 0;
     e->p4.help_trips = 0;
     e->p4_help = lr_p4_help_choice(e);
+    e->p4_shortcut = lr_p4_shortcut_choice();
     if (e->lay.persistent == 2 && e->p4_help) {
         static const int env_t = lr_env_int_pack("LR_P4_HELP_TRIPS", -1);
         const double t = ((double)e->n8 + 512.0) / 896.0;
diff --git a/literate_amd/csrc/lr_step.h b/literate_amd/csrc/lr_step.h
--- a/literate_amd/csrc/lr_step.h
+++ b/literate_amd/csrc/lr_step.h
@@ -544,16 +544,20 @@
     double par[8];
 };
 
-template <bool LDS_CONSTS = false, int PB = 0, int CS = 2, bool PAIR_PLANES = true, bool HAND = false>
+template <bool LDS_CONSTS = false, int PB = 0, int CS = 2, bool PAIR_PLANES = true, bool HAND = false, bool SKIP = false>
 __device__ __forceinline__ void lr_propose_rj(const lr_step_args& a, int c, int lane, lr_seg_scratch* scratch_p,
                                               uint64_t it, lr_rj_state& s, lr_rj_prop& p, double2* table,
                                               int table_es, const lr_rj_draws* pre = nullptr,
                                               const double* br_lds = nullptr, const double* logbr_lds = nullptr,
                                               const double* base_col = nullptr, int col_doubles = 0, double base_const = 0.0,
-                                              lr_table_hand* hand = nullptr, int hand_epoch = 0) {
+                                              lr_table_hand* hand = nullptr, int hand_epoch = 0, bool may_skip = false,
+                                              int origin = 0, bool* skipped = nullptr,
+                                              bool pre_on = true ) {
     static_assert(CS == 2 || (PB > 0 && !PAIR_PLANES), "a column of its own: one-pass builder, no pair planes");
+    static_assert(!SKIP || HAND, "proposals are skipped where a helper wave builds the tables");
     static_assert(!HAND || PB > 0, "a helper wave runs the one-pass builder");
     lr_seg_scratch& scratch = *scratch_p;
+    const bool has_pre = pre != nullptr && pre_on;
     const lr_mcmc_config& cfg = a.cfg;
     const int n_bins = cfg.n_bins;
     const lr_stream rng{(uint32_t)cfg.seed, (uint32_t)(cfg.chain_offset + c)};
@@ -563,12 +567,12 @@
     const double priorPoiA = s.priorPoi;
 
     lr_u2 ud{0.0, 0.0};
-    if (!pre) {
+    if (!has_pre) {
         const int ul = lane - LR_UD_LANE;
         const uint32_t purpose = (ul < 0) ? LR_P_MULT : ((ul == 0) ? LR_P_ACCEPT : (ul == 1 ? LR_P_MOVE : LR_P_RJ));
         ud = lr_pair(rng, it, purpose, ul < 0 ? (uint32_t)lane : (ul == 3 ? 1u : 0u));
     }
-    const double u_next = pre ? 1.0 : lr_bcast(ud.a, LR_UD_LANE);
+    const double u_next = has_pre ? 1.0 : lr_bcast(ud.a, LR_UD_LANE);
     LR_SSTAMP(2);
 
     double pL = L, pM = M, ptL = tL, ptM = tM;
@@ -578,10 +582,10 @@
     const double sample_shift_mu = cfg.const_death_rate ? 0.0 : 0.5;
     const double b_freq = cfg.const_death_rate ? 0.7 : 0.4, d_freq = 0.8;
     const double fL = cfg.update_fraction, fM = cfg.const_death_rate ? 1.0 : cfg.update_fraction;
-    const lr_u2 r = pre ? lr_u2{pre->r_a, pre->r_b} : lr_u2{lr_bcast(ud.a, LR_UD_LANE + 1), lr_bcast(ud.b, LR_UD_LANE + 1)};
+    const lr_u2 r = has_pre ? lr_u2{pre->r_a, pre->r_b} : lr_u2{lr_bcast(ud.a, LR_UD_LANE + 1), lr_bcast(ud.b, LR_UD_LANE + 1)};
     if (r.a < b_freq) {
         if (r.b < .5 || KL == 1) {
-            if (pre) {
+            if (has_pre) {
                 hasting = lr_wave_multiplier_pre(pL, KL, pre->da < fL, pre->x, pre->m, lane);
             } else {
                 hasting = lr_wave_multiplier(pL, KL, ud.a < fL, ud.b, a.mult_l, lane);
@@ -593,7 +597,7 @@
         }
     } else if (r.a < d_freq) {
         if (r.b < .5 || KM == 1) {
-            if (pre) {
+            if (has_pre) {
                 hasting = lr_wave_multiplier_pre(pM, KM, pre->da < fM, pre->x, pre->m, lane);
             } else {
                 hasting = lr_wave_multiplier(pM, KM, ud.a < fM, ud.b, a.mult_l, lane);
@@ -605,12 +609,12 @@
         }
     } else if (r.a < 0.999 && cfg.const_rates == 0) {
         move_kind = 4;
-        const lr_u2 q = pre ? lr_u2{pre->q_a, pre->q_b} : lr_u2{lr_bcast(ud.a, LR_UD_LANE + 2), lr_bcast(ud.b, LR_UD_LANE + 2)};
+        const lr_u2 q = has_pre ? lr_u2{pre->q_a, pre->q_b} : lr_u2{lr_bcast(ud.a, LR_UD_LANE + 2), lr_bcast(ud.b, LR_UD_LANE + 2)};
         const bool sideL = q.a > sample_shift_mu;
         double R = sideL ? L : M, T = sideL ? tL : tM;
         int K = sideL ? KL : KM;
         double score = 0.0;
-        const lr_u2 q2 = pre ? lr_u2{pre->q2_a, pre->q2_b} : lr_u2{lr_bcast(ud.a, LR_UD_LANE + 3), lr_bcast(ud.b, LR_UD_LANE + 3)};
+        const lr_u2 q2 = has_pre ? lr_u2{pre->q2_a, pre->q2_b} : lr_u2{lr_bcast(ud.a, LR_UD_LANE + 3), lr_bcast(ud.b, LR_UD_LANE + 3)};
         if (q.b > 0.5) {
             if (K >= LR_KMAX) {
                 invalid = LR_INVALID_KCAP;
@@ -618,7 +622,7 @@
                 const int ind = min((int)(q2.a * K), K - 1);
                 const double delta = q2.b * (lr_bcast(T, ind + 1) - lr_bcast(T, ind));
                 double beta;
-                if (pre) {
+                if (has_pre) {
                     beta = pre->beta;
                 } else {
                     double ga, gb;
@@ -657,16 +661,27 @@
     }
 
     LR_SSTAMP(3);
+    bool skip = false;
+    if (SKIP) {
+        const double nL = lr_dpp_zero<0x130 , 0xf, 0xf>(ptL);
+        const double nM = lr_dpp_zero<0x130, 0xf, 0xf>(ptM);
+        const double dmin = fmin(lane < PKL ? fabs(nL - ptL) : 1e300, lane < PKM ? fabs(nM - ptM) : 1e300);
+        if (__ballot(dmin <= LR_MIN_ALLOWED_T)) invalid |= LR_INVALID_GUARD;
+        bool noop = gibbs != 0;
+        if (move_kind == 1 || move_kind == 3) noop = __ballot(lane <= LR_KMAX && (peL != eL || peM != eM)) == 0ull;
+        skip = may_skip && (invalid != 0 || (origin != 0 && noop));
+        *skipped = skip;
+    }
     double logpL, logpM, log_u_next;
     lr_stage_segments(&scratch, pL, pM, peL, peM, PKL, PKM, lane, &logpL, &logpM, u_next, &log_u_next);
-    if (pre) log_u_next = pre->log_u;
+    if (has_pre) log_u_next = pre->log_u;
 
     lr_seg_cache sg{s.sgL, s.sgM, false};
     bool edges_same = false;
-    if ((pre && s.sg_valid) || base_col) edges_same = PKL == KL && PKM == KM && __ballot(lane <= LR_KMAX && (peL != eL || peM != eM)) == 0ull;
-    if (pre && s.sg_valid) sg.reuse = edges_same;
+    if ((has_pre && s.sg_valid) || base_col) edges_same = PKL == KL && PKM == KM && __ballot(lane <= LR_KMAX && (peL != eL || peM != eM)) == 0ull;
+    if (has_pre && s.sg_valid) sg.reuse = edges_same;
     const bool same_table = base_col && edges_same && (move_kind == 1 || move_kind == 3 || move_kind == 5);
-    if (HAND) {
+    if (HAND && !skip) {
         if (lane == 0) hand->KL = PKL, hand->KM = PKM, hand->reuse = sg.reuse ? 1 : 0, hand->noop = same_table ? 1 : 0;
         LR_WAVE_LDS_ORDER();
         if (lane == 0) __hip_atomic_store(&hand->epoch, hand_epoch, __ATOMIC_RELAXED, __HIP_MEMORY_SCOPE_WORKGROUP);
@@ -674,7 +689,7 @@
 
     LR_SSTAMP(4);
     double priorP = -INFINITY;
-    {
+    if (!SKIP) {
         const double nL = lr_dpp_zero<0x130 , 0xf, 0xf>(ptL);
         const double nM = lr_dpp_zero<0x130, 0xf, 0xf>(ptM);
         const double dmin = fmin(lane < PKL ? fabs(nL - ptL) : 1e300, lane < PKM ? fabs(nM - ptM) : 1e300);
@@ -697,14 +712,14 @@
         for (int i = lane; i < col_doubles; i += LR_WAVE) col[CS * i] = base_col[CS * i];
         constP = base_const;
     } else if (HAND) {
-        p.table_by_helper = 1;
+        p.table_by_helper = skip ? 0 : 1;
     } else {
         constP = lr_build_tables_segments<PB, CS>(&scratch, peL, peM, PKL, PKM, LDS_CONSTS ? br_lds : a.br_length,
                                                   LDS_CONSTS ? logbr_lds : a.log_br, cfg.model,
                                                   n_bins, a.n_cls, a.H, table, lane,
                                                   lr_tab_mode<LDS_CONSTS>(a, table_es), cfg.frac_birth, cfg.frac_death,
-                                                  table_es, pre ? &sg : nullptr);
-        s.sgL = sg.packL, s.sgM = sg.packM, s.sg_valid = (pre && sg.packL != -1) ? 1 : 0;
+                                                  table_es, has_pre ? &sg : nullptr);
+        s.sgL = sg.packL, s.sgM = sg.packM, s.sg_valid = (has_pre && sg.packL != -1) ? 1 : 0;
     }
     if (LDS_CONSTS && PAIR_PLANES && !HAND && !same_table) {
         LR_WAVE_LDS_ORDER();
@@ -718,12 +733,22 @@
     p.gibbs = gibbs, p.invalid = invalid, p.move = move_kind;
 }
 
-template <bool LDS_CONSTS = false, int PB = 0, bool HAND = false>
+struct lr_skip_ctl {
+    uint64_t it_end;
+    int on;
+    int carried;
+    int skipped;
+    int decided;
+    int done;
+};
+template <bool LDS_CONSTS = false, int PB = 0, bool HAND = false, bool SKIP = false>
 __device__ __forceinline__ void lr_chain_step_core(lr_chain_regs& st, const lr_step_args& a, int mode, int c, int lane,
                                                    lr_seg_scratch* scratch_p, double lik_sum, double2* table,
                                                    int table_es = 2, const double* br_lds = nullptr,
                                                    const double* logbr_lds = nullptr, const lr_rj_draws* pre = nullptr,
-                                                   lr_table_hand* hand = nullptr, int hand_epoch = 0) {
+                                                   lr_table_hand* hand = nullptr, int hand_epoch = 0,
+                                                   lr_skip_ctl* ctl = nullptr) {
+    static_assert(!SKIP || HAND, "");
     const lr_mcmc_config& cfg = a.cfg;
     const double sc = st.sc;
     const int isc = st.isc;
@@ -741,6 +766,8 @@
     int n_acc = lr_bcast_i(isc, LR_I_ACCEPTED);
     uint64_t next_sample = (uint64_t)(uint32_t)lr_bcast_i(isc, LR_I_NEXT_LO) | ((uint64_t)(uint32_t)lr_bcast_i(isc, LR_I_NEXT_HI) << 32);
     int trace_slot = lr_bcast_i(isc, LR_I_SLOT);
+    int origin = SKIP ? lr_bcast_i(isc, LR_I_ORIGIN) : 0;
+    const bool carried = SKIP && ctl->carried != 0;
     LR_SSTAMP(1);
 
     if (mode == 1) {
@@ -753,15 +780,18 @@
         const int gibbs = lr_bcast_i(isc, LR_I_GIBBS), invalid = lr_bcast_i(isc, LR_I_INVALID);
         const double priorP = lr_bcast(sc, LR_S_PRIOR_P), constP = lr_bcast(sc, LR_S_CONST_P);
         double lik;
-        const bool ok = lr_mh_accept(gibbs, invalid, lik_sum, constP, likA, priorP, priorA, lr_bcast(sc, LR_S_HASTING),
-                                     lr_bcast(sc, LR_S_LOG_U), &lik) && mode != 2;
+        const bool ok = lr_mh_accept(gibbs, invalid, carried ? likA : lik_sum, carried ? 0.0 : constP, likA, priorP, priorA,
+                                     lr_bcast(sc, LR_S_HASTING), lr_bcast(sc, LR_S_LOG_U), &lik) && mode != 2;
+        if (SKIP) ctl->decided = (carried && !invalid) ? 1 : 0;
         lik_p = invalid ? -INFINITY : lik;
         lr_warn_kcap(a.warn, invalid, lane);
         if (ok) {
             s.L = st.pL, s.M = st.pM, s.tL = st.ptL, s.tM = st.ptM, s.eL = st.peL, s.eM = st.peM;
             s.KL = lr_bcast_i(isc, LR_I_PKL), s.KM = lr_bcast_i(isc, LR_I_PKM);
-            likA = lik, priorA = priorP, s.priorPoi = lr_bcast(sc, LR_S_PRIORPOI_P), constA = constP;
+            likA = lik, priorA = priorP, s.priorPoi = lr_bcast(sc, LR_S_PRIORPOI_P);
+            if (!carried) constA = constP;
             n_acc += 1;
+            if (SKIP && !carried && !gibbs) origin = 1;
         }
         if (it == next_sample) {
             const int slot = trace_slot;
@@ -776,7 +806,12 @@
     const int KL = s.KL, KM = s.KM;
 
     lr_rj_prop p;
-    if (HAND) lr_propose_rj<LDS_CONSTS, (PB > 0 ? PB : 1), 2, true, HAND>(a, c, lane, scratch_p, it, s, p, table, table_es, pre, br_lds, logbr_lds, nullptr, 0, 0.0, hand, hand_epoch);
+    if (SKIP) {
+        bool skipped = false;
+        lr_propose_rj<LDS_CONSTS, (PB > 0 ? PB : 1), 2, true, HAND, SKIP>(a, c, lane, scratch_p, it, s, p, table, table_es, pre, br_lds, logbr_lds, nullptr, 0, 0.0,
+                                                                          hand, hand_epoch, ctl->on != 0 && it < ctl->it_end, origin, &skipped, !carried);
+        ctl->skipped = skipped ? 1 : 0, ctl->done = it >= ctl->it_end ? 1 : 0;
+    } else if (HAND) lr_propose_rj<LDS_CONSTS, (PB > 0 ? PB : 1), 2, true, HAND>(a, c, lane, scratch_p, it, s, p, table, table_es, pre, br_lds, logbr_lds, nullptr, 0, 0.0, hand, hand_epoch);
     else lr_propose_rj<LDS_CONSTS, PB>(a, c, lane, scratch_p, it, s, p, table, table_es, pre, br_lds, logbr_lds);
 
     st.pL = s.L, st.pM = s.M, st.ptL = s.tL, st.ptM = s.tM, st.peL = s.eL, st.peM = s.eM;
@@ -813,6 +848,7 @@
         io = (lane == LR_I_NEXT_LO) ? (int)(uint32_t)next_sample : io;
         io = (lane == LR_I_NEXT_HI) ? (int)(uint32_t)(next_sample >> 32) : io;
         io = (lane == LR_I_SLOT) ? trace_slot : io;
+        if (SKIP) io = (lane == LR_I_ORIGIN) ? origin : io;
         st.isc = io;
     }
     LR_SSTAMP(7);
diff --git a/literate_amd/engine.py b/literate_amd/engine.py
--- a/literate_amd/engine.py
+++ b/literate_amd/engine.py
@@ -202,6 +202,11 @@
         _hip.check(_hip.launch(self.lib.lr_mcmc_warnings, self.device, self.handle, C.byref(w)), "lr_mcmc_warnings")
         return int(w.value)
 
+    def counters(self):
+        v = (C.c_int64 * 3)()
+        _hip.check(_hip.launch(self.lib.lr_mcmc_counters, self.device, self.handle, v), "lr_mcmc_counters")
+        return dict(phases=int(v[0]), shortcuts=int(v[1]), scans=int(v[2]))
+
     def warning_text(self):
         w = self.warnings()
         if w & _hip.LR_WARN_KCAP:
```

Result: no change. 16250 billion, median of 6 (+0.5%).
